# speechbrain/speechbrain

Hardware: NVIDIA B200
Metric: audio-sec/sec (RTFx) Conformer-L ASR, batch=32x10s@16kHz (higher is better)
Workload: dtype fp16 operands, fp32 accumulate/residual/softmax

## Files before the change

### include/sbk.h

```cpp
#ifndef SBK_H_
#define SBK_H_
#include <stdint.h>
#ifdef __cplusplus
extern "C" {
#endif

typedef struct sbk_fbank sbk_fbank;
typedef struct sbk_asr sbk_asr;

enum { SBK_ATT_ROPE = 0, SBK_ATT_RELPOS = 1 };
enum { SBK_ACT_RELU = 0, SBK_ACT_GELU = 1 };
enum { SBK_PART_FBANK = 1, SBK_PART_CNN = 2, SBK_PART_ENCODER = 4, SBK_PART_DECODER = 8, SBK_PART_ALL = 15, SBK_PART_LM = 16 };

typedef struct {
    const char* name;
    const float* data;
    int64_t numel;
} sbk_tensor;

typedef struct {
    int n_fft, hop, n_mels;
    int cnn_c1, cnn_c2;
    int input_size, d_model, nhead, num_encoder_layers, num_decoder_layers, d_ffn, vocab, kernel_size;
    int attention_type;
    int decoder_activation;
    int max_len;
    int parts;
    int lm_d_model, lm_nhead, lm_layers, lm_d_ffn, lm_activation;
    float fbank_amin, fbank_top_db, norm_eps;
} sbk_asr_config;

typedef struct {
    int beam_size, max_steps, min_steps, bos, eos;
    float temperature;
    int using_eos_threshold;
    float eos_threshold;
    int length_normalization;
    float minus_inf;
    float lm_weight, lm_temperature;
    float ctc_weight;
    int blank_index;
    float length_weight;
    float coverage_weight, coverage_threshold;
} sbk_beam_params;

const char* sbk_last_error(void);
int sbk_version(void);
long long sbk_launch_count(void);
void sbk_gemm_profile_enable(int on);
int sbk_gemm_profile_read(int* n_launches, double* total_ms, double* total_flops);

int sbk_fbank_create(int n_fft, int hop, int n_mels, const float* window_host, const float* mel_matrix_host,
                     float amin, float top_db, sbk_fbank** out);
void sbk_fbank_destroy(sbk_fbank* fb);
int sbk_fbank_num_frames(const sbk_fbank* fb, int n_samples);
int sbk_fbank_forward(const sbk_fbank* fb, const float* wav_dev, int B, int L, float* out_dev,
                      int* utt_max_scratch_dev, void* stream);

int sbk_input_norm_global(const float* x_dev, float* out_dev, int B, int T, int F, const float* mean_dev,
                          const float* std_dev, float eps, void* stream);
int sbk_input_norm_sentence(const float* x_dev, float* out_dev, const float* rel_len_dev, int B, int T, int F,
                            int std_norm, int avoid_padding_norm, float eps, void* stream);

int sbk_gemm_f16_test(const void* A_dev, const void* W_dev, const float* bias_dev, void* out_dev, int out_is_f32,
                      int act, int M, int N, int K, void* stream);
int sbk_gemm_f16_resid_test(const void* A_dev, const void* W_dev, const float* bias_dev, float* x_dev, float alpha,
                            int M, int N, int K, void* stream);

int sbk_asr_create(const sbk_asr_config* cfg, const sbk_tensor* weights, int n_weights, sbk_asr** out);
void sbk_asr_destroy(sbk_asr* m);
int sbk_asr_clone(sbk_asr* src, sbk_asr** out);
int sbk_asr_set_dynchunk(sbk_asr* m, int chunk_size, int left_context_chunks);
int sbk_asr_set_poll_interval(sbk_asr* m, int every_n_steps);
int sbk_asr_set_decoder_ln_fusion(sbk_asr* m, int on);
int sbk_asr_set_decoder_tc_min_rows(sbk_asr* m, int rows);
int sbk_asr_lm_rescore(sbk_asr* m, const int* tokens_dev, const int* lens_dev, int n, int L, float temperature, int pad_index,
                       float* scores_dev, void* stream);
int sbk_asr_num_frames(const sbk_asr* m, int n_samples, int* T_feat, int* T_enc);

int sbk_asr_cnn_forward(sbk_asr* m, const float* feats_dev, int B, int T0, float* out_dev, void* stream);
int sbk_asr_encode_from_cnn(sbk_asr* m, const float* src_dev, const float* rel_len_dev, int B, int T,
                            float* enc_out_dev, void* stream);
int sbk_asr_encode_feats(sbk_asr* m, const float* feats_dev, const float* rel_len_dev, int B, int T0,
                         float* cnn_out_dev, float* enc_out_dev, void* stream);
int sbk_asr_greedy_from_enc(sbk_asr* m, const float* enc_dev, const float* rel_len_dev, int B, int T, int max_steps,
                            int bos, int eos, int* pred_dev, float* score_dev, float* log_probs_dev, int* steps_done,
                            void* stream);
int sbk_rows_argmax_f32(const float* x_dev, int rows, int V, int* idx_dev, void* stream);
int sbk_asr_ctc_head(sbk_asr* m, const float* enc_dev, int B, int T, float* log_probs_dev, int* argmax_dev, void* stream);
int sbk_asr_decode_teacher_forced(sbk_asr* m, const int* tgt_dev, const float* enc_dev, const int* enc_len_dev, int n, int S,
                                  int T, float* out_dev, void* stream);
int sbk_asr_beam_from_enc(sbk_asr* m, const float* enc_dev, const float* rel_len_dev, int B, int T,
                          const sbk_beam_params* params, int* hist_tok_dev, int* hist_pred_dev, float* hist_score_dev,
                          float* hist_lp_dev, int* steps_done, void* stream);
int sbk_asr_transcribe_greedy_dev(sbk_asr* m, const float* wav_dev, const float* rel_len_dev, int B, int L,
                                  int max_steps, int bos, int eos, float* enc_out_dev, int* pred_dev,
                                  float* score_dev, float* log_probs_dev, int* steps_done, void* stream);
int sbk_asr_transcribe_greedy_group_dev(sbk_asr* m, int G, const float* const* wav_dev, const float* const* rel_len_dev,
                                        int B, int L, int max_steps, int bos, int eos, int* const* pred_dev,
                                        int* steps_done, void* stream);
int sbk_asr_transcribe_greedy_host(sbk_asr* m, const float* wav_host, const float* rel_len_host, int B, int L,
                                   int max_steps, int bos, int eos, int* pred_host, float* score_host,
                                   int* steps_done, void* stream);

int sbk_asr_transcribe_greedy_group_host_async(sbk_asr* m, int G, const float* const* wav_host,
                                               const float* const* rel_len_host, int B, int L, int max_steps, int bos, int eos,
                                               int* const* pred_host, int* const* pred_dev, int* steps_done, void* stream);

int sbk_asr_transcribe_greedy_host_async(sbk_asr* m, const float* wav_host, const float* rel_len_host, int B, int L,
                                         int max_steps, int bos, int eos, int* pred_host, float* score_host,
                                         int* steps_done, void* stream);

#ifdef __cplusplus
}
#endif
#endif
```

### speechbrain_b200/_lib.py

```python
import ctypes
import os

import torch

_HERE = os.path.dirname(os.path.abspath(__file__))
LIB_PATH = os.path.join(_HERE, "libsbk.so")

_lib = None


class sbk_tensor(ctypes.Structure):
    _fields_ = [("name", ctypes.c_char_p), ("data", ctypes.c_void_p), ("numel", ctypes.c_int64)]


class sbk_asr_config(ctypes.Structure):
    _fields_ = [(k, ctypes.c_int) for k in (
        "n_fft", "hop", "n_mels", "cnn_c1", "cnn_c2", "input_size", "d_model", "nhead", "num_encoder_layers",
        "num_decoder_layers", "d_ffn", "vocab", "kernel_size", "attention_type", "decoder_activation", "max_len",
        "parts", "lm_d_model", "lm_nhead", "lm_layers", "lm_d_ffn", "lm_activation")] + [
        (k, ctypes.c_float) for k in ("fbank_amin", "fbank_top_db", "norm_eps")]


class sbk_beam_params(ctypes.Structure):
    _fields_ = [("beam_size", ctypes.c_int), ("max_steps", ctypes.c_int), ("min_steps", ctypes.c_int),
                ("bos", ctypes.c_int), ("eos", ctypes.c_int), ("temperature", ctypes.c_float),
                ("using_eos_threshold", ctypes.c_int), ("eos_threshold", ctypes.c_float),
                ("length_normalization", ctypes.c_int), ("minus_inf", ctypes.c_float),
                ("lm_weight", ctypes.c_float), ("lm_temperature", ctypes.c_float),
                ("ctc_weight", ctypes.c_float), ("blank_index", ctypes.c_int), ("length_weight", ctypes.c_float),
                ("coverage_weight", ctypes.c_float), ("coverage_threshold", ctypes.c_float)]


SBK_ATT_ROPE, SBK_ATT_RELPOS = 0, 1
SBK_ACT_RELU, SBK_ACT_GELU = 0, 1
SBK_PARTS = {"fbank": 1, "cnn": 2, "encoder": 4, "decoder": 8, "lm": 16}

EXPORTS = [
    "sbk_last_error", "sbk_version", "sbk_launch_count", "sbk_gemm_profile_enable", "sbk_gemm_profile_read", "sbk_fbank_create", "sbk_fbank_destroy", "sbk_fbank_num_frames",
    "sbk_fbank_forward", "sbk_input_norm_global", "sbk_input_norm_sentence", "sbk_gemm_f16_test", "sbk_gemm_f16_resid_test",
    "sbk_asr_create", "sbk_asr_destroy", "sbk_asr_num_frames", "sbk_asr_cnn_forward", "sbk_asr_encode_from_cnn",
    "sbk_asr_encode_feats", "sbk_asr_greedy_from_enc", "sbk_asr_transcribe_greedy_dev",
    "sbk_asr_transcribe_greedy_host", "sbk_asr_transcribe_greedy_host_async", "sbk_asr_clone",
    "sbk_asr_set_poll_interval", "sbk_asr_beam_from_enc", "sbk_asr_set_decoder_ln_fusion", "sbk_asr_transcribe_greedy_group_dev",
    "sbk_asr_set_decoder_tc_min_rows", "sbk_asr_lm_rescore", "sbk_asr_transcribe_greedy_group_host_async", "sbk_asr_decode_teacher_forced", "sbk_asr_ctc_head", "sbk_rows_argmax_f32", "sbk_asr_set_dynchunk",
]


def lib():
    global _lib
    if _lib is None:
        if not os.path.exists(LIB_PATH):
            raise RuntimeError(
                f"{LIB_PATH} not found: the sm_100a CUDA library is required (no CPU fallback). "
                "Build it with `make -C speechbrain_b200/csrc` or `__graft_entry__.build()`.")
        L = ctypes.CDLL(LIB_PATH)
        L.sbk_last_error.restype = ctypes.c_char_p
        for name in EXPORTS:
            getattr(L, name)
        for name in EXPORTS:
            if name not in ("sbk_last_error", "sbk_fbank_destroy", "sbk_asr_destroy", "sbk_launch_count",
                            "sbk_gemm_profile_enable"):
                getattr(L, name).restype = ctypes.c_int
        L.sbk_launch_count.restype = ctypes.c_longlong
        L.sbk_gemm_profile_enable.restype = None
        _lib = L
    return _lib


def check(rc, what):
    if rc != 0:
        raise RuntimeError(f"libsbk: {what} failed ({rc}): {lib().sbk_last_error().decode()}")


def ptr(t):
    if t is None:
        return ctypes.c_void_p(0)
    assert t.is_contiguous(), "libsbk needs contiguous tensors"
    return ctypes.c_void_p(t.data_ptr())


def stream_ptr(device=None):
    return ctypes.c_void_p(torch.cuda.current_stream(device).cuda_stream)


def require_cuda(t, what):
    if not t.is_cuda:
        raise RuntimeError(f"{what}: expected a CUDA tensor (speechbrain_b200 has no CPU path)")
```

### speechbrain_b200/csrc/common.cuh

```cuda
#pragma once
#include <cuda.h>
#include <cuda_fp16.h>
#include <cuda_runtime.h>
#include <stdint.h>

#define SBK_OK 0
#define SBK_ERR_CUDA -1
#define SBK_ERR_ARG -2
#define SBK_ERR_UNSUPPORTED -3
#define SBK_ERR_NOMEM -4

namespace sbk {

void set_error(const char* fmt, ...);

#define SBK_CUDA_CHECK(expr)                                                              \
    do {                                                                                  \
        cudaError_t _e = (expr);                                                          \
        if (_e != cudaSuccess) {                                                          \
            sbk::set_error("%s:%d: %s -> %s", __FILE__, __LINE__, #expr, cudaGetErrorString(_e)); \
            return SBK_ERR_CUDA;                                                          \
        }                                                                                 \
    } while (0)

void count_launch();
#define SBK_LAUNCH_CHECK()                   \
    do {                                     \
        sbk::count_launch();                 \
        SBK_CUDA_CHECK(cudaGetLastError());  \
    } while (0)

#define SBK_REQUIRE(cond, ...)            \
    do {                                  \
        if (!(cond)) {                    \
            sbk::set_error(__VA_ARGS__);  \
            return SBK_ERR_ARG;           \
        }                                 \
    } while (0)

__host__ __device__ inline int ceil_div(int a, int b) { return (a + b - 1) / b; }

__device__ __forceinline__ float warp_sum(float v) {
#pragma unroll
    for (int o = 16; o > 0; o >>= 1) v += __shfl_xor_sync(0xffffffffu, v, o);
    return v;
}
__device__ __forceinline__ float warp_max(float v) {
#pragma unroll
    for (int o = 16; o > 0; o >>= 1) v = fmaxf(v, __shfl_xor_sync(0xffffffffu, v, o));
    return v;
}

__device__ __forceinline__ uint32_t smem_u32(const void* p) {
    return static_cast<uint32_t>(__cvta_generic_to_shared(p));
}

__device__ __forceinline__ void mbar_init(uint64_t* bar, uint32_t count) {
    asm volatile("mbarrier.init.shared::cta.b64 [%0], %1;" ::"r"(smem_u32(bar)), "r"(count));
}
__device__ __forceinline__ void mbar_fence_init() {
    asm volatile("fence.mbarrier_init.release.cluster;" ::: "memory");
}
__device__ __forceinline__ void mbar_arrive_expect_tx(uint64_t* bar, uint32_t bytes) {
    asm volatile("mbarrier.arrive.expect_tx.shared::cta.b64 _, [%0], %1;" ::"r"(smem_u32(bar)), "r"(bytes)
                 : "memory");
}
__device__ __forceinline__ void mbar_arrive(uint64_t* bar) {
    asm volatile("mbarrier.arrive.shared::cta.b64 _, [%0];" ::"r"(smem_u32(bar)) : "memory");
}
__device__ __forceinline__ bool mbar_try_wait(uint64_t* bar, uint32_t parity) {
    uint32_t ok;
    asm volatile(
        "{\n\t.reg .pred p;\n\t"
        "mbarrier.try_wait.parity.shared::cta.b64 p, [%1], %2;\n\t"
        "selp.u32 %0, 1, 0, p;\n\t}"
        : "=r"(ok)
        : "r"(smem_u32(bar)), "r"(parity)
        : "memory");
    return ok != 0;
}
__device__ __forceinline__ void mbar_wait(uint64_t* bar, uint32_t parity) {
    while (!mbar_try_wait(bar, parity)) {
    }
}

__device__ __forceinline__ void tma_prefetch_desc(const CUtensorMap* m) {
    asm volatile("prefetch.tensormap [%0];" ::"l"(reinterpret_cast<uint64_t>(m)) : "memory");
}
__device__ __forceinline__ void tma_load_2d(void* smem_dst, const CUtensorMap* m, uint64_t* bar, int c0, int c1) {
    asm volatile(
        "cp.async.bulk.tensor.2d.shared::cluster.global.mbarrier::complete_tx::bytes [%0], [%1, {%3, %4}], [%2];"
        ::"r"(smem_u32(smem_dst)), "l"(reinterpret_cast<uint64_t>(m)), "r"(smem_u32(bar)), "r"(c0), "r"(c1)
        : "memory");
}
__device__ __forceinline__ void tma_load_4d(void* smem_dst, const CUtensorMap* m, uint64_t* bar, int c0, int c1, int c2, int c3) {
    asm volatile(
        "cp.async.bulk.tensor.4d.shared::cluster.global.mbarrier::complete_tx::bytes [%0], [%1, {%3, %4, %5, %6}], [%2];"
        ::"r"(smem_u32(smem_dst)), "l"(reinterpret_cast<uint64_t>(m)), "r"(smem_u32(bar)), "r"(c0), "r"(c1), "r"(c2), "r"(c3)
        : "memory");
}
__device__ __forceinline__ void bulk_load_1d(void* smem_dst, const void* gsrc, uint32_t bytes, uint64_t* bar) {
    asm volatile(
        "cp.async.bulk.shared::cluster.global.mbarrier::complete_tx::bytes [%0], [%1], %2, [%3];"
        ::"r"(smem_u32(smem_dst)), "l"(reinterpret_cast<uint64_t>(gsrc)), "r"(bytes), "r"(smem_u32(bar))
        : "memory");
}

__device__ __forceinline__ void tmem_alloc(uint32_t* smem_result, uint32_t ncols) {
    asm volatile("tcgen05.alloc.cta_group::1.sync.aligned.shared::cta.b32 [%0], %1;" ::"r"(smem_u32(smem_result)),
                 "r"(ncols)
                 : "memory");
    asm volatile("tcgen05.relinquish_alloc_permit.cta_group::1.sync.aligned;" ::: "memory");
}
__device__ __forceinline__ void tmem_dealloc(uint32_t taddr, uint32_t ncols) {
    asm volatile("tcgen05.dealloc.cta_group::1.sync.aligned.b32 %0, %1;" ::"r"(taddr), "r"(ncols) : "memory");
}
__device__ __forceinline__ void tc_fence_before() { asm volatile("tcgen05.fence::before_thread_sync;" ::: "memory"); }
__device__ __forceinline__ void tc_fence_after() { asm volatile("tcgen05.fence::after_thread_sync;" ::: "memory"); }

__device__ __forceinline__ void umma_f16(uint32_t tmem_d, uint64_t desc_a, uint64_t desc_b, uint32_t idesc,
                                         uint32_t accumulate) {
    asm volatile(
        "{\n\t.reg .pred p;\n\t"
        "setp.ne.b32 p, %4, 0;\n\t"
        "tcgen05.mma.cta_group::1.kind::f16 [%0], %1, %2, %3, p;\n\t}"
        ::"r"(tmem_d), "l"(desc_a), "l"(desc_b), "r"(idesc), "r"(accumulate)
        : "memory");
}
__device__ __forceinline__ void umma_commit(uint64_t* bar) {
    asm volatile("tcgen05.commit.cta_group::1.mbarrier::arrive::one.shared::cluster.b64 [%0];" ::"r"(smem_u32(bar))
                 : "memory");
}
__device__ __forceinline__ void tmem_ld_32x32(uint32_t taddr, uint32_t (&r)[32]) {
    asm volatile(
        "tcgen05.ld.sync.aligned.32x32b.x32.b32 "
        "{%0, %1, %2, %3, %4, %5, %6, %7, %8, %9, %10, %11, %12, %13, %14, %15, "
        "%16, %17, %18, %19, %20, %21, %22, %23, %24, %25, %26, %27, %28, %29, %30, %31}, [%32];"
        : "=r"(r[0]), "=r"(r[1]), "=r"(r[2]), "=r"(r[3]), "=r"(r[4]), "=r"(r[5]), "=r"(r[6]), "=r"(r[7]), "=r"(r[8]),
          "=r"(r[9]), "=r"(r[10]), "=r"(r[11]), "=r"(r[12]), "=r"(r[13]), "=r"(r[14]), "=r"(r[15]), "=r"(r[16]),
          "=r"(r[17]), "=r"(r[18]), "=r"(r[19]), "=r"(r[20]), "=r"(r[21]), "=r"(r[22]), "=r"(r[23]), "=r"(r[24]),
          "=r"(r[25]), "=r"(r[26]), "=r"(r[27]), "=r"(r[28]), "=r"(r[29]), "=r"(r[30]), "=r"(r[31])
        : "r"(taddr)
        : "memory");
}
__device__ __forceinline__ void tmem_ld_wait() { asm volatile("tcgen05.wait::ld.sync.aligned;" ::: "memory"); }

__device__ __forceinline__ uint64_t make_kmajor_sw128_desc(uint32_t smem_addr) {
    uint64_t d = 0;
    d |= static_cast<uint64_t>((smem_addr & 0x3FFFFu) >> 4);
    d |= static_cast<uint64_t>(1) << 16;
    d |= static_cast<uint64_t>(1024 >> 4) << 32;
    d |= static_cast<uint64_t>(1) << 46;
    d |= static_cast<uint64_t>(2) << 61;
    return d;
}
__host__ __device__ constexpr uint32_t make_idesc_f16(int M, int N, int ab_format) {
    return (1u << 4) | (static_cast<uint32_t>(ab_format) << 7) | (static_cast<uint32_t>(ab_format) << 10) |
           (static_cast<uint32_t>(N >> 3) << 17) | (static_cast<uint32_t>(M >> 4) << 24);
}

__device__ __forceinline__ __half2 floats2half2_sat(float lo, float hi) {
    uint32_t r;
    asm("cvt.rn.satfinite.f16x2.f32 %0, %1, %2;" : "=r"(r) : "f"(hi), "f"(lo));
    return *reinterpret_cast<__half2*>(&r);
}
__device__ __forceinline__ __half float2half_sat(float x) {
    const __half2 h = floats2half2_sat(x, 0.0f);
    return __low2half(h);
}

__device__ __forceinline__ float rcp_approx(float x) {
    float y;
    asm("rcp.approx.ftz.f32 %0, %1;" : "=f"(y) : "f"(x));
    return y;
}
__device__ __forceinline__ float exp_ftz(float x) {
    float y;
    asm("ex2.approx.ftz.f32 %0, %1;" : "=f"(y) : "f"(x * 1.4426950408889634f));
    return y;
}
__device__ __forceinline__ float sigmoid_f(float x) { return rcp_approx(1.0f + exp_ftz(-x)); }
__device__ __forceinline__ float tanh_approx(float x) {
    float y;
    asm("tanh.approx.f32 %0, %1;" : "=f"(y) : "f"(x));
    return y;
}
__device__ __forceinline__ float sigmoid_fast(float x) { return fmaf(0.5f, tanh_approx(0.5f * x), 0.5f); }
__device__ __forceinline__ float silu_fast(float x) {
    const float h = 0.5f * x;
    return fmaf(h, tanh_approx(h), h);
}
__device__ __forceinline__ void sts128(uint32_t addr, uint4 v) {
    asm volatile("st.shared.v4.b32 [%0], {%1, %2, %3, %4};" ::"r"(addr), "r"(v.x), "r"(v.y), "r"(v.z), "r"(v.w) : "memory");
}
__device__ __forceinline__ uint4 lds128(uint32_t addr) {
    uint4 v;
    asm volatile("ld.shared.v4.b32 {%0, %1, %2, %3}, [%4];" : "=r"(v.x), "=r"(v.y), "=r"(v.z), "=r"(v.w) : "r"(addr) : "memory");
    return v;
}
__device__ __forceinline__ uint4 f4_as_u4(float4 f) {
    return make_uint4(__float_as_uint(f.x), __float_as_uint(f.y), __float_as_uint(f.z), __float_as_uint(f.w));
}
__device__ __forceinline__ float4 u4_as_f4(uint4 u) {
    return make_float4(__uint_as_float(u.x), __uint_as_float(u.y), __uint_as_float(u.z), __uint_as_float(u.w));
}
__device__ __forceinline__ float silu_f(float x) { return x * sigmoid_f(x); }
__device__ __forceinline__ float gelu_erf_f(float x) { return 0.5f * x * (1.0f + erff(x * 0.70710678118654752f)); }

__device__ __forceinline__ int float_to_ordered(float f) {
    int i = __float_as_int(f);
    return i >= 0 ? i : i ^ 0x7FFFFFFF;
}
__device__ __forceinline__ float ordered_to_float(int i) { return __int_as_float(i >= 0 ? i : i ^ 0x7FFFFFFF); }

int make_tmap_2d_f16(CUtensorMap* out, const void* base, uint64_t rows, uint64_t cols, uint64_t row_stride_elems,
                     uint32_t box_rows, uint32_t box_cols);

}
```

### speechbrain_b200/csrc/engine.cu

```cuda
#include <math.h>
#include <stdio.h>
#include <stdlib.h>
#include <string.h>

#include <algorithm>
#include <map>
#include <string>
#include <vector>

#include "common.cuh"
#include "sbk_internal.h"
#include "../../include/sbk.h"

namespace sbk {

struct EncLayerW {
    const float *ffn1_ln_g, *ffn1_ln_b, *ffn1_b1, *ffn1_b2;
    const __half *ffn1_w1, *ffn1_w2;
    const float *norm1_g, *norm1_b;
    const __half *wqkv, *wo;
    const float* bo;
    const __half* wpos;
    const float *pos_u, *pos_v;
    const float *conv_ln_g, *conv_ln_b;
// ... 276 lines not shown
    }
    if (!p.ok) { rc = SBK_ERR_ARG; goto fail; }
    m->enc_norm_g = p.f32("Transformer.encoder.norm.norm.weight", d);
    m->enc_norm_b = p.f32("Transformer.encoder.norm.norm.bias", d);
    m->pos_len = c.max_len;
    if (c.attention_type == SBK_ATT_ROPE) {
        std::vector<float> cs((size_t)c.max_len * dh / 2), sn(cs.size());
        for (int i = 0; i < dh / 2; ++i) {
            const float ang = expf((float)(2 * i) * -(logf(10000.0f) / (float)dh));
            for (int t = 0; t < c.max_len; ++t) {
                const float ta = (float)t * ang;
                cs[(size_t)t * (dh / 2) + i] = cosf(ta);
                sn[(size_t)t * (dh / 2) + i] = sinf(ta);
            }
        }
        m->rope_cos = p.f32_raw(cs.data(), cs.size());
        m->rope_sin = p.f32_raw(sn.data(), sn.size());
    } else {
        std::vector<float> pe((size_t)c.max_len * d);
        for (int i = 0; i < d / 2; ++i) {
            const float fr = expf((float)(2 * i) * -(logf(10000.0f) / (float)d));
            for (int t = 0; t < c.max_len; ++t) {
                pe[(size_t)t * d + 2 * i] = sinf((float)t * fr);
                pe[(size_t)t * d + 2 * i + 1] = cosf((float)t * fr);
            }
        }
        m->relpos_pe = p.f16_raw(pe.data(), pe.size());
    }
    }
    if (has_dec) {
        m->emb = p.f32("Transformer.custom_tgt_module.layers.0.emb.Embedding.weight", (int64_t)c.vocab * d);
        {
            std::vector<float> pe((size_t)c.max_len * d);
            for (int i = 0; i < d / 2; ++i) {
                const float den = expf((float)(2 * i) * -(logf(10000.0f) / (float)d));
                for (int t = 0; t < c.max_len; ++t) {
                    pe[(size_t)t * d + 2 * i] = sinf((float)t * den);
                    pe[(size_t)t * d + 2 * i + 1] = cosf((float)t * den);
                }
            }
            m->dec_pe = p.f32_raw(pe.data(), pe.size());
        }
        const int L = c.num_decoder_layers;
        m->dec.resize(L);
        std::vector<float> wckv((size_t)L * 2 * d * d), bckv((size_t)L * 2 * d);
        const float qs = 1.0f / sqrtf((float)dh);
        for (int l = 0; l < L && p.ok; ++l) {
            const std::string q = "Transformer.decoder.layers." + std::to_string(l) + ".";
            DecLayerW& e = m->dec[l];
            e.n1g = p.f32(q + "norm1.norm.weight", d); e.n1b = p.f32(q + "norm1.norm.bias", d);
            e.n2g = p.f32(q + "norm2.norm.weight", d); e.n2b = p.f32(q + "norm2.norm.bias", d);
            e.n3g = p.f32(q + "norm3.norm.weight", d); e.n3b = p.f32(q + "norm3.norm.bias", d);
            const float* wi = find(w, q + "self_attn.att.in_proj_weight", (int64_t)3 * d * d);
            const float* bi = find(w, q + "self_attn.att.in_proj_bias", 3 * d);
            const float* wc = find(w, q + "multihead_attn.att.in_proj_weight", (int64_t)3 * d * d);
            const float* bc = find(w, q + "multihead_attn.att.in_proj_bias", 3 * d);
            if (!wi || !bi || !wc || !bc) { p.ok = false; break; }
            {
                std::vector<float> ws(wi, wi + (size_t)3 * d * d), bs(bi, bi + 3 * d);
                for (size_t i = 0; i < (size_t)d * d; ++i) ws[i] *= qs;
                for (int i = 0; i < d; ++i) bs[i] *= qs;
                e.w_self_in = p.f16_raw(ws.data(), ws.size());
                e.b_self_in = p.f32_raw(bs.data(), bs.size());
                std::vector<float> wq(wc, wc + (size_t)d * d), bq(bc, bc + d);
                for (auto& v : wq) v *= qs;
                for (auto& v : bq) v *= qs;
                e.w_cross_q = p.f16_raw(wq.data(), wq.size());
                e.b_cross_q = p.f32_raw(bq.data(), bq.size());
            }
            memcpy(&wckv[(size_t)l * 2 * d * d], wc + (size_t)d * d, (size_t)2 * d * d * 4);
            memcpy(&bckv[(size_t)l * 2 * d], bc + d, (size_t)2 * d * 4);
            e.w_self_out = p.f16(q + "self_attn.att.out_proj.weight", (int64_t)d * d); e.b_self_out = p.f32(q + "self_attn.att.out_proj.bias", d);
            e.w_cross_out = p.f16(q + "multihead_attn.att.out_proj.weight", (int64_t)d * d); e.b_cross_out = p.f32(q + "multihead_attn.att.out_proj.bias", d);
            e.w_ffn1 = p.f16(q + "pos_ffn.ffn.0.weight", (int64_t)F * d); e.b_ffn1 = p.f32(q + "pos_ffn.ffn.0.bias", F);
            e.w_ffn2 = p.f16(q + "pos_ffn.ffn.3.weight", (int64_t)d * F); e.b_ffn2 = p.f32(q + "pos_ffn.ffn.3.bias", d);
        }
        if (!p.ok) { rc = SBK_ERR_ARG; goto fail; }
        m->w_ckv = p.f16_raw(wckv.data(), wckv.size());
        m->b_ckv = p.f32_raw(bckv.data(), bckv.size());
        m->dec_norm_g = p.f32("Transformer.decoder.norm.norm.weight", d);
        m->dec_norm_b = p.f32("Transformer.decoder.norm.norm.bias", d);
        m->w_lin = nullptr; m->b_lin = nullptr;
        if (w.count("seq_lin.w.weight")) {
            m->w_lin = p.f16("seq_lin.w.weight", (int64_t)c.vocab * d);
            m->b_lin = p.f32("seq_lin.w.bias", c.vocab);
        }
    }
    if ((c.parts & SBK_PART_LM) && c.lm_layers > 0) {
        const int dl = c.lm_d_model, Fl = c.lm_d_ffn, dhl = dl / c.lm_nhead;
        if (dhl != 64 || dl % 128 != 0) { set_error("asr_create: LM head_dim must be 64 and d_model %% 128 == 0"); rc = SBK_ERR_UNSUPPORTED; goto fail; }
        m->has_lm = true;
        m->lm_emb = p.f32("lm.custom_src_module.emb.Embedding.weight", (int64_t)c.vocab * dl);
        {
            std::vector<float> pe((size_t)c.max_len * dl);
            for (int i = 0; i < dl / 2; ++i) {
                const float den = expf((float)(2 * i) * -(logf(10000.0f) / (float)dl));
                for (int t = 0; t < c.max_len; ++t) {
                    pe[(size_t)t * dl + 2 * i] = sinf((float)t * den);
                    pe[(size_t)t * dl + 2 * i + 1] = cosf((float)t * den);
                }
            }
            m->lm_pe = p.f32_raw(pe.data(), pe.size());
        }
        m->lm.resize(c.lm_layers);
        const float qs = 1.0f / sqrtf((float)dhl);
        for (int l = 0; l < c.lm_layers && p.ok; ++l) {
            const std::string q = "lm.encoder.layers." + std::to_string(l) + ".";
            LmLayerW& e = m->lm[l];
            const float* wi = find(w, q + "self_att.att.in_proj_weight", (int64_t)3 * dl * dl);
            const float* bi = find(w, q + "self_att.att.in_proj_bias", 3 * dl);
            if (!wi || !bi) { p.ok = false; break; }
            std::vector<float> ws(wi, wi + (size_t)3 * dl * dl), bs(bi, bi + 3 * dl);
            for (size_t i = 0; i < (size_t)dl * dl; ++i) ws[i] *= qs;
            for (int i = 0; i < dl; ++i) bs[i] *= qs;
            e.w_in = p.f16_raw(ws.data(), ws.size());
            e.b_in = p.f32_raw(bs.data(), bs.size());
            e.w_out = p.f16(q + "self_att.att.out_proj.weight", (int64_t)dl * dl); e.b_out = p.f32(q + "self_att.att.out_proj.bias", dl);
            e.w1 = p.f16(q + "pos_ffn.ffn.0.weight", (int64_t)Fl * dl); e.b1 = p.f32(q + "pos_ffn.ffn.0.bias", Fl);
            e.w2 = p.f16(q + "pos_ffn.ffn.3.weight", (int64_t)dl * Fl); e.b2 = p.f32(q + "pos_ffn.ffn.3.bias", dl);
            e.n1g = p.f32(q + "norm1.norm.weight", dl); e.n1b = p.f32(q + "norm1.norm.bias", dl);
            e.n2g = p.f32(q + "norm2.norm.weight", dl); e.n2b = p.f32(q + "norm2.norm.bias", dl);
        }
        m->lm_norm_g = p.f32("lm.encoder.norm.norm.weight", dl); m->lm_norm_b = p.f32("lm.encoder.norm.norm.bias", dl);
        m->lm_wp0 = p.f16("lm.output_proj.layers.0.w.weight", (int64_t)dl * dl); m->lm_bp0 = p.f32("lm.output_proj.layers.0.w.bias", dl);
        m->lm_lnp_g = p.f32("lm.output_proj.layers.1.norm.weight", dl); m->lm_lnp_b = p.f32("lm.output_proj.layers.1.norm.bias", dl);
        m->lm_wp2 = p.f16("lm.output_proj.layers.2.w.weight", (int64_t)c.vocab * dl); m->lm_bp2 = p.f32("lm.output_proj.layers.2.w.bias", c.vocab);
        if (!p.ok) { rc = SBK_ERR_ARG; goto fail; }
    }
    if (w.count("ctc_lin.w.weight")) {
        m->w_ctc = p.f16("ctc_lin.w.weight", (int64_t)c.vocab * d);
        m->b_ctc = p.f32("ctc_lin.w.bias", c.vocab);
    }
    if (!p.ok) { rc = SBK_ERR_ARG; goto fail; }
    if (cudaMallocHost(&m->host_flag, 64) != cudaSuccess) { set_error("cudaMallocHost failed"); rc = SBK_ERR_NOMEM; goto fail; }
    m->weight_refs = new int(1);
    if (cudaDeviceSynchronize() != cudaSuccess) { set_error("asr_create: device error after upload"); rc = SBK_ERR_CUDA; goto fail; }
    *out = m;
    return SBK_OK;
fail:
    if (m->fbank) fbank_destroy(m->fbank);
    cudaFree(m->warena.base);
    delete m;
    return rc;
}

int asr_clone(AsrModel* src, AsrModel** out) {
    SBK_REQUIRE(src && out, "asr_clone: null argument");
    AsrModel* m = new AsrModel(*src);
    m->ws = Arena();
    m->wsB = m->wsL = m->ws_rows = m->ws_steps = 0;
    m->b = AsrModel::Buf();
    m->ctc = AsrModel::CtcBuf();
    m->cov = AsrModel::CovBuf();
    m->step_graph = nullptr;
    m->pipe_graph = nullptr;
    m->group_graph = nullptr;
    m->hgroup_graph = nullptr;
    m->beam_graph = nullptr;
    m->gwav = m->grel = nullptr; m->gwav_cap = 0;
    m->copy_stream = nullptr; m->ev_fork = nullptr;
    for (auto& e : m->ev_ready) e = nullptr;
    m->graph_rows = m->graph_T = m->graph_B = -1;
    m->cap_stream = nullptr;
    m->host_flag = nullptr;
    if (cudaMallocHost(&m->host_flag, 64) != cudaSuccess) {
        delete m;
        set_error("asr_clone: cudaMallocHost failed");
        return SBK_ERR_NOMEM;
    }
    ++*m->weight_refs;
    *out = m;
    return SBK_OK;
}

void asr_destroy(AsrModel* m) {
    if (!m) return;
    if (m->step_graph) cudaGraphExecDestroy(m->step_graph);
    if (m->pipe_graph) cudaGraphExecDestroy(m->pipe_graph);
    if (m->group_graph) cudaGraphExecDestroy(m->group_graph);
    if (m->hgroup_graph) cudaGraphExecDestroy(m->hgroup_graph);
    if (m->beam_graph) cudaGraphExecDestroy(m->beam_graph);
    cudaFree(m->gwav);
    if (m->copy_stream) cudaStreamDestroy(m->copy_stream);
    if (m->ev_fork) cudaEventDestroy(m->ev_fork);
    for (auto e : m->ev_ready) if (e) cudaEventDestroy(e);
    if (m->weight_refs && --*m->weight_refs == 0) {
        if (m->fbank) fbank_destroy(m->fbank);
        cudaFree(m->warena.base);
        delete m->weight_refs;
    }
    cudaFree(m->ws.base);
    cudaFree(m->ctc.base);
    cudaFree(m->cov.base);
    if (m->host_flag) cudaFreeHost(m->host_flag);
    if (m->cap_stream) cudaStreamDestroy(m->cap_stream);
    if (m->side_stream) cudaStreamDestroy(m->side_stream);
    if (m->dec_stream) cudaStreamDestroy(m->dec_stream);
    if (m->ev_dfork) cudaEventDestroy(m->ev_dfork);
    if (m->ev_djoin) cudaEventDestroy(m->ev_djoin);
    if (m->ev_bfork) cudaEventDestroy(m->ev_bfork);
    if (m->ev_bjoin) cudaEventDestroy(m->ev_bjoin);
    delete m;
}

static void drop_graphs(AsrModel* m) {
    if (m->step_graph) { cudaGraphExecDestroy(m->step_graph); m->step_graph = nullptr; m->graph_rows = -1; }
    if (m->pipe_graph) { cudaGraphExecDestroy(m->pipe_graph); m->pipe_graph = nullptr; }
    if (m->group_graph) { cudaGraphExecDestroy(m->group_graph); m->group_graph = nullptr; }
    if (m->hgroup_graph) { cudaGraphExecDestroy(m->hgroup_graph); m->hgroup_graph = nullptr; }
    if (m->beam_graph) { cudaGraphExecDestroy(m->beam_graph); m->beam_graph = nullptr; }
}

static void frames(const sbk_asr_config& c, int L, int* T0, int* T1, int* T2) {
    *T0 = 1 + L / c.hop;
    *T1 = (*T0 - 1) / 2 + 1;
    *T2 = (*T1 - 1) / 2 + 1;
}

static int ensure_workspace(AsrModel* m, int B, int L, int rows, int steps) {
    if (m->ws.base && B <= m->wsB && L <= m->wsL && rows <= m->ws_rows && steps <= m->ws_steps) return SBK_OK;
    B = std::max(B, m->wsB); L = std::max(L, m->wsL); rows = std::max(rows, m->ws_rows); steps = std::max(steps, m->ws_steps);
    const sbk_asr_config& c = m->cfg;
    int T0, T1, T2;
    frames(c, L, &T0, &T1, &T2);
    const int F1 = (c.n_mels - 1) / 2 + 1;
    const size_t M = (size_t)B * T2, d = c.d_model, F = c.d_ffn, Ld = c.num_decoder_layers, S = steps + 1;
    const size_t Md = (size_t)std::max(B, rows) * T2;
    size_t need = 0;
    auto sz = [&](size_t bytes) { need += (bytes + 255) & ~size_t(255); };
    sz((size_t)B * L * 4); sz((size_t)B * T0 * c.n_mels * 4); sz(M * d * 4); sz(M * d * 4); sz(Md * d * 4);
    sz((size_t)B * T1 * F1 * c.cnn_c1 * 4); sz(M * c.input_size * 4); sz((size_t)rows * d * 4);
    sz((size_t)rows * c.vocab * 4); sz((size_t)rows * S * 4);
    sz(B * 4); sz((size_t)std::max(B, rows) * 4); sz((size_t)rows * (S + 1) * 4); sz(rows * 4 + 64); sz(rows * 4); sz(64); sz((size_t)rows * S * 4); sz(B * 4);
    sz((size_t)B * T1 * F1 * c.cnn_c1 * 2); sz(M * c.input_size * 2); sz(M * d * 2); sz(M * F * 2); sz(M * 3 * d * 2);
    sz(M * d * 2); sz((size_t)T2 * d * 2); sz(Md * d * 2); sz(Md * Ld * 2 * d * 2);
    sz((size_t)Ld * rows * S * d * 2); sz((size_t)Ld * rows * S * d * 2);
    sz((size_t)rows * d * 2); sz((size_t)rows * d * 2); sz((size_t)rows * d * 2); sz((size_t)rows * F * 2);
    sz((size_t)2 * rows * S * 4); sz(B * 4 + 64); sz((size_t)2 * rows * 4); sz((size_t)rows * d * 4); sz((size_t)rows * 33 * 4);
    sz((size_t)rows * S * 4); sz((size_t)rows * S * 4); sz((size_t)rows * S * 4); sz((size_t)rows * S * 4);
    const size_t dl = m->has_lm ? c.lm_d_model : 0, Fl = m->has_lm ? c.lm_d_ffn : 0, Ll = m->has_lm ? c.lm_layers : 0;
    if (m->has_lm) {
        sz(rows * dl * 4); sz(rows * dl * 4); sz((size_t)rows * c.vocab * 4); sz((size_t)rows * c.vocab * 4);
        sz(rows * dl * 2); sz(rows * dl * 2); sz(rows * dl * 2); sz(rows * Fl * 2); sz(rows * dl * 2);
        sz(Ll * rows * S * dl * 2); sz(Ll * rows * S * dl * 2); sz((size_t)rows * S * 4);
    }
    need += 1 << 20;
    if (need > m->ws.cap) {
        if (m->ws.base) { cudaDeviceSynchronize(); cudaFree(m->ws.base); m->ws.base = nullptr; }
        if (cudaMalloc(&m->ws.base, need) != cudaSuccess) {
            m->ws.cap = 0;
            set_error("workspace cudaMalloc(%zu) failed", need);
            return SBK_ERR_NOMEM;
        }
        m->ws.cap = need;
    }
    drop_graphs(m);
    m->ws.used = 0;
    AsrModel::Buf& b = m->b;
#define TAKE(field, type, bytes) b.field = reinterpret_cast<type*>(m->ws.take(bytes))
    TAKE(wav, float, (size_t)B * L * 4); TAKE(feats, float, (size_t)B * T0 * c.n_mels * 4); TAKE(x, float, M * d * 4);
    TAKE(glu, float, M * d * 4); TAKE(enc_out, float, Md * d * 4); TAKE(act1_f, float, (size_t)B * T1 * F1 * c.cnn_c1 * 4);
    TAKE(cnn_f, float, M * c.input_size * 4); TAKE(dx, float, (size_t)rows * d * 4); TAKE(logits, float, (size_t)rows * c.vocab * 4);
    TAKE(score, float, (size_t)rows * S * 4);
    TAKE(utt_max, int, B * 4); TAKE(enc_len, int, (size_t)std::max(B, rows) * 4); TAKE(tokens, int, (size_t)rows * (S + 1) * 4); TAKE(step, int, rows * 4 + 64);
    TAKE(has_ended, int, rows * 4); TAKE(ended_count, int, 64); TAKE(pred, int, (size_t)rows * S * 4); TAKE(rel_len, float, B * 4);
    TAKE(act1, __half, (size_t)B * T1 * F1 * c.cnn_c1 * 2); TAKE(a_in, __half, M * c.input_size * 2); TAKE(h16, __half, M * d * 2);
    TAKE(f16, __half, M * F * 2); TAKE(qkv16, __half, M * 3 * d * 2); TAKE(att16, __half, M * d * 2);
    TAKE(P16, __half, (size_t)T2 * d * 2); TAKE(enc16, __half, Md * d * 2); TAKE(ckv16, __half, Md * Ld * 2 * d * 2);
    TAKE(kcache, __half, (size_t)Ld * rows * S * d * 2); TAKE(vcache, __half, (size_t)Ld * rows * S * d * 2);
    TAKE(dh16, __half, (size_t)rows * d * 2); TAKE(dq16, __half, (size_t)rows * d * 2); TAKE(datt16, __half, (size_t)rows * d * 2);
    TAKE(df16, __half, (size_t)rows * F * 2);
    TAKE(lineage, int, (size_t)2 * rows * S * 4); TAKE(finished, int, B * 4 + 64); TAKE(seq_scores, float, (size_t)2 * rows * 4);
    TAKE(lnout, float, (size_t)rows * d * 4); TAKE(beam_scr, float, (size_t)rows * 33 * 4);
    TAKE(hist_tok, int, (size_t)rows * S * 4); TAKE(hist_pred, int, (size_t)rows * S * 4);
    TAKE(hist_score, float, (size_t)rows * S * 4); TAKE(hist_lp, float, (size_t)rows * S * 4);
    if (m->has_lm) {
        TAKE(lx, float, rows * dl * 4); TAKE(lh32, float, rows * dl * 4); TAKE(lm_logits, float, (size_t)rows * c.vocab * 4);
        TAKE(lm_extra, float, (size_t)rows * c.vocab * 4);
        TAKE(lx16, __half, rows * dl * 2); TAKE(lq16, __half, rows * dl * 2); TAKE(latt16, __half, rows * dl * 2);
        TAKE(lf16, __half, rows * Fl * 2); TAKE(lh16, __half, rows * dl * 2);
        TAKE(lkc, __half, Ll * rows * S * dl * 2); TAKE(lvc, __half, Ll * rows * S * dl * 2); TAKE(tok_cache, int, (size_t)rows * S * 4);
        if (!b.tok_cache) { set_error("workspace carve failed (LM)"); return SBK_ERR_NOMEM; }
    }
    if (!b.df16 || !b.seq_scores || !b.lnout || !b.hist_lp) { set_error("workspace carve failed"); return SBK_ERR_NOMEM; }
#undef TAKE
    m->wsB = B; m->wsL = L; m->ws_rows = rows; m->ws_steps = steps;
    return SBK_OK;
}

#define RC(expr) do { int _rc = (expr); if (_rc) return _rc; } while (0)

static int run_encoder(AsrModel* m, const float* feats, int B, int T0, const int* enc_len, float* cnn_out_f,
                       float* enc_out, cudaStream_t st) {
    const sbk_asr_config& c = m->cfg;
    AsrModel::Buf& b = m->b;
    const int T1 = (T0 - 1) / 2 + 1, T = feats ? (T1 - 1) / 2 + 1 : T0;
    const int M = B * T, d = c.d_model, F = c.d_ffn, H = c.nhead, dh = d / H;
    SBK_REQUIRE(m->has_enc, "encode: this handle was created without encoder weights");
    SBK_REQUIRE(feats == nullptr || m->has_cnn, "encode: this handle was created without CNN weights");
    SBK_REQUIRE(T <= m->pos_len, "encode: %d frames exceed max_len=%d", T, m->pos_len);
    if (feats != nullptr)
        RC(cnn_frontend_forward(feats, B, T0, c.n_mels, m->c1_w, m->c1_b, m->c1_g, m->c1_be, c.cnn_c1, m->c2_w, m->c2_b,
                                m->c2_g, m->c2_be, c.cnn_c2, b.act1, nullptr, b.a_in, cnn_out_f, st));
    GemmEpilogue e;
    e.mode = EPI_F32; e.bias = m->b_in; e.out = b.x; e.ldo = d;
    RC(gemm_f16(b.a_in, c.input_size, m->w_in, c.input_size, e, M, d, c.input_size, st));
    const float att_scale = 1.0f / sqrtf((float)d);
    for (int l = 0; l < c.num_encoder_layers; ++l) {
        const EncLayerW& w = m->enc[l];
        if (l == 0) RC(layernorm_rows(b.x, b.h16, true, w.ffn1_ln_g, w.ffn1_ln_b, M, d, 1e-5f, false, st));
        e = GemmEpilogue(); e.mode = EPI_F16; e.act = ACT_SILU; e.bias = w.ffn1_b1; e.out = b.f16; e.ldo = F;
        RC(gemm_f16(b.h16, d, w.ffn1_w1, d, e, M, F, d, st));
        e = GemmEpilogue(); e.mode = EPI_RESID; e.bias = w.ffn1_b2; e.out = b.x; e.resid = b.x; e.ldo = d; e.alpha = 0.5f;
        RC(gemm_f16(b.f16, F, w.ffn1_w2, F, e, M, d, F, st));
        RC(layernorm_rows(b.x, b.h16, true, w.norm1_g, w.norm1_b, M, d, 1e-5f, false, st));
        e = GemmEpilogue(); e.out = b.qkv16; e.ldo = 3 * d;
        if (c.attention_type == SBK_ATT_ROPE) {
            e.mode = EPI_ROPE; e.alpha = att_scale; e.T = T; e.rope_cos = m->rope_cos; e.rope_sin = m->rope_sin; e.head_dim = dh;
        } else {
            e.mode = EPI_F16;
        }
        RC(gemm_f16(b.h16, d, w.wqkv, d, e, M, 3 * d, d, st));
        if (c.attention_type == SBK_ATT_RELPOS) {
            e = GemmEpilogue(); e.mode = EPI_F16; e.out = b.P16; e.ldo = d;
            RC(gemm_f16(m->relpos_pe, d, w.wpos, d, e, T, d, d, st));
        }
        RC(encoder_attention(b.qkv16, 3 * d, B, T, H, dh, enc_len, c.attention_type == SBK_ATT_RELPOS, w.pos_u, w.pos_v,
                             b.P16, d, att_scale, b.att16, d, st, m->dyn_chunk, m->dyn_left));
        e = GemmEpilogue(); e.mode = EPI_RESID; e.bias = w.bo; e.out = b.x; e.resid = b.x; e.ldo = d; e.alpha = 1.0f;
        RC(gemm_f16(b.att16, d, w.wo, d, e, M, d, d, st));
        RC(layernorm_rows(b.x, b.h16, true, w.conv_ln_g, w.conv_ln_b, M, d, 1e-5f, false, st));
        e = GemmEpilogue(); e.mode = EPI_GLU; e.bias = w.bpw1; e.out = b.glu; e.ldo = d;
        RC(gemm_f16(b.h16, d, w.wpw1, d, e, M, 2 * d, d, st));
        RC(dwconv_ln_swish(b.glu, B, T, d, c.kernel_size, w.wdw, w.bdw, w.aconv_ln_g, w.aconv_ln_b, 1e-5f, b.h16, st, m->dyn_chunk));
        e = GemmEpilogue(); e.mode = EPI_RESID; e.bias = w.bpw2; e.out = b.x; e.resid = b.x; e.ldo = d; e.alpha = 1.0f;
        e.row_lens = enc_len; e.T = T;
        RC(gemm_f16(b.h16, d, w.wpw2, d, e, M, d, d, st));
        RC(layernorm_rows(b.x, b.h16, true, w.ffn2_ln_g, w.ffn2_ln_b, M, d, 1e-5f, false, st));
        e = GemmEpilogue(); e.mode = EPI_F16; e.act = ACT_SILU; e.bias = w.ffn2_b1; e.out = b.f16; e.ldo = F;
        RC(gemm_f16(b.h16, d, w.ffn2_w1, d, e, M, F, d, st));
        e = GemmEpilogue(); e.mode = EPI_RESID; e.bias = w.ffn2_b2; e.out = b.x; e.resid = b.x; e.ldo = d; e.alpha = 0.5f;
        RC(gemm_f16(b.f16, F, w.ffn2_w2, F, e, M, d, F, st));
        if (l + 1 < c.num_encoder_layers) {
            const EncLayerW& nx = m->enc[l + 1];
            RC(layernorm2_rows(b.x, b.x, b.h16, true, w.norm2_g, w.norm2_b, 1e-5f, nx.ffn1_ln_g, nx.ffn1_ln_b, 1e-5f, M, d, st));
        } else {
            RC(layernorm2_rows(b.x, nullptr, enc_out, false, w.norm2_g, w.norm2_b, 1e-5f, m->enc_norm_g, m->enc_norm_b, 1e-6f, M,
                               d, st));
        }
    }
    if (c.num_encoder_layers == 0)
        RC(layernorm_rows(b.x, enc_out, false, m->enc_norm_g, m->enc_norm_b, M, d, 1e-6f, false, st));
    return SBK_OK;
}

__global__ void abs_len_kernel(const float* rel, int B, int T, int* out) {
    const int i = blockIdx.x * blockDim.x + threadIdx.x;
    if (i < B) out[i] = min(T, max(0, __float2int_rn(rel[i] * static_cast<float>(T))));
}

static int dec_ln(AsrModel* m, SkinnyArgs& a, const float* g, const float* bta, int rows, cudaStream_t st) {
    AsrModel::Buf& b = m->b;
    const int d = m->cfg.d_model;
    if (m->fuse_dec_ln && (d == 256 || d == 512 || d == 768 || d == 1024)) {
        a.X = b.dx; a.ln_g = g; a.ln_b = bta; a.ln_eps = 1e-6f;
        return SBK_OK;
    }
    a.A = b.dh16; a.lda = d;
    return layernorm_rows(b.dx, b.dh16, true, g, bta, rows, d, 1e-6f, false, st);
}

static bool xatt_headmajor(const AsrModel* m) {
    static const bool legacy = getenv("SBK_XATT_ROWMAJOR") != nullptr || getenv("SBK_GEMM_V1") != nullptr;
    return !legacy && m->cfg.d_model / m->cfg.nhead == 64 && m->cfg.d_model % 256 == 0;
}
static int project_cross_kv(AsrModel* m, int M, int T, cudaStream_t st) {
    const sbk_asr_config& c = m->cfg;
    AsrModel::Buf& b = m->b;
    const int d = c.d_model, Ld = c.num_decoder_layers;
    RC(cast_f32_f16(b.enc_out, b.enc16, (size_t)M * d, st));
    for (int l = 0; l < Ld; ++l) {
        GemmEpilogue e;
        e.mode = EPI_F16; e.bias = m->b_ckv + (size_t)l * 2 * d; e.out = b.ckv16 + (size_t)l * M * 2 * d; e.ldo = 2 * d;
        if (xatt_headmajor(m)) { e.kv_heads = c.nhead; e.kv_part_stride = (size_t)M * d; e.T = T; }
        RC(gemm_f16(b.enc16, d, m->w_ckv + (size_t)l * 2 * d * d, d, e, M, 2 * d, d, st));
    }
    return SBK_OK;
}
static void cross_kv_args(const AsrModel* m, DecAttnArgs& t, int l, int n_utt, int T) {
    const int d = m->cfg.d_model;
    const size_t M = (size_t)n_utt * T;
    t.kbase = m->b.ckv16 + (size_t)l * M * 2 * d;
    if (xatt_headmajor(m)) {
        t.vbase = t.kbase + M * d; t.row_stride = (size_t)T * d; t.head_stride = T * 64; t.key_stride = 64;
    } else {
        t.vbase = t.kbase + d; t.row_stride = (size_t)T * 2 * d; t.head_stride = 0; t.key_stride = 2 * d;
    }
}

static int enqueue_decode_layers_tc(AsrModel* m, int rows, int rows_per_utt, int T, int S_max, const int* lineage,
                                    cudaStream_t st, bool with_head) {
    const sbk_asr_config& c = m->cfg;
    AsrModel::Buf& b = m->b;
    const int d = c.d_model, F = c.d_ffn, H = c.nhead, dh = d / H, Ld = c.num_decoder_layers;
    const int n_utt = rows / rows_per_utt;
    for (int l = 0; l < Ld; ++l) {
        const DecLayerW& w = m->dec[l];
        __half* kc = b.kcache + (size_t)l * rows * S_max * d;
        __half* vc = b.vcache + (size_t)l * rows * S_max * d;
        RC(layernorm_rows(b.dx, b.dh16, true, w.n1g, w.n1b, rows, d, 1e-6f, false, st));
        GemmEpilogue e;
        e.mode = EPI_QKV_CACHE; e.bias = w.b_self_in; e.out = b.dq16; e.ldo = d; e.kcache = kc; e.vcache = vc;
        e.step_ptr = b.step; e.S_max = S_max; e.qkv_d = d;
        RC(gemm_f16_small(b.dh16, d, w.w_self_in, d, e, rows, 3 * d, d, st));
        DecAttnArgs t{};
        t.q = b.dq16; t.ldq = d; t.kbase = kc; t.vbase = vc; t.row_stride = (size_t)S_max * d; t.key_stride = d;
        t.rows_per_block = 1; t.n_keys_ptr = b.step; t.enc_len = nullptr; t.H = H; t.dh = dh; t.out = b.datt16; t.ldo = d;
        t.lineage = lineage; t.lin_stride = S_max;
        RC(dec_attention(t, rows, S_max, st));
        e = GemmEpilogue(); e.mode = EPI_RESID; e.bias = w.b_self_out; e.out = b.dx; e.resid = b.dx; e.ldo = d;
        RC(gemm_f16_small(b.datt16, d, w.w_self_out, d, e, rows, d, d, st));
        RC(layernorm_rows(b.dx, b.dh16, true, w.n2g, w.n2b, rows, d, 1e-6f, false, st));
        e = GemmEpilogue(); e.mode = EPI_F16; e.bias = w.b_cross_q; e.out = b.dq16; e.ldo = d;
        RC(gemm_f16_small(b.dh16, d, w.w_cross_q, d, e, rows, d, d, st));
        t = DecAttnArgs{};
        t.q = b.dq16; t.ldq = d; cross_kv_args(m, t, l, n_utt, T); t.rows_per_block = rows_per_utt;
        t.n_keys_ptr = nullptr; t.enc_len = b.enc_len; t.H = H; t.dh = dh; t.out = b.datt16; t.ldo = d;
        RC(dec_attention(t, rows, T, st));
        e = GemmEpilogue(); e.mode = EPI_RESID; e.bias = w.b_cross_out; e.out = b.dx; e.resid = b.dx; e.ldo = d;
        RC(gemm_f16_small(b.datt16, d, w.w_cross_out, d, e, rows, d, d, st));
        RC(layernorm_rows(b.dx, b.dh16, true, w.n3g, w.n3b, rows, d, 1e-6f, false, st));
        e = GemmEpilogue(); e.mode = EPI_F16; e.act = c.decoder_activation == SBK_ACT_GELU ? ACT_GELU : ACT_RELU;
        e.bias = w.b_ffn1; e.out = b.df16; e.ldo = F;
        RC(gemm_f16_small(b.dh16, d, w.w_ffn1, d, e, rows, F, d, st));
        e = GemmEpilogue(); e.mode = EPI_RESID; e.bias = w.b_ffn2; e.out = b.dx; e.resid = b.dx; e.ldo = d;
        RC(gemm_f16_small(b.df16, F, w.w_ffn2, F, e, rows, d, F, st));
    }
    if (!with_head) return SBK_OK;
    SBK_REQUIRE(m->w_lin != nullptr, "decode step: this handle was created without the output head (seq_lin.w.*)");
    RC(layernorm_rows(b.dx, b.dh16, true, m->dec_norm_g, m->dec_norm_b, rows, d, 1e-6f, false, st));
    GemmEpilogue e;
    e.mode = EPI_F32; e.bias = m->b_lin; e.out = b.logits; e.ldo = c.vocab;
    RC(gemm_f16_small(b.dh16, d, m->w_lin, d, e, rows, c.vocab, d, st));
    return SBK_OK;
}

static int enqueue_decode_layers(AsrModel* m, int rows, int rows_per_utt, int T, int S_max, const int* lineage,
                                 cudaStream_t st, bool with_head = true) {
    if (rows >= m->dec_tc_rows && m->cfg.d_model % 32 == 0)
        return enqueue_decode_layers_tc(m, rows, rows_per_utt, T, S_max, lineage, st, with_head);
    const sbk_asr_config& c = m->cfg;
    AsrModel::Buf& b = m->b;
    const int d = c.d_model, F = c.d_ffn, H = c.nhead, dh = d / H, Ld = c.num_decoder_layers;
    const int ffn_epi = c.decoder_activation == SBK_ACT_GELU ? SK_F16_GELU : SK_F16_RELU;
    const int n_utt = rows / rows_per_utt;
    for (int l = 0; l < Ld; ++l) {
        const DecLayerW& w = m->dec[l];
        __half* kc = b.kcache + (size_t)l * rows * S_max * d;
        __half* vc = b.vcache + (size_t)l * rows * S_max * d;
        SkinnyArgs a{};
        RC(dec_ln(m, a, w.n1g, w.n1b, rows, st));
        a.W = w.w_self_in; a.ldw = d; a.bias = w.b_self_in; a.n_rows = rows; a.N = 3 * d; a.K = d;
        a.epi = SK_QKV_CACHE; a.out = b.dq16; a.ldo = d; a.kcache = kc; a.vcache = vc; a.step_ptr = b.step; a.S_max = S_max;
        a.d = d; a.q_scale = 1.0f;
        RC(skinny_gemm(a, st));
        DecAttnArgs t{};
        t.q = b.dq16; t.ldq = d; t.kbase = kc; t.vbase = vc; t.row_stride = (size_t)S_max * d; t.key_stride = d;
        t.rows_per_block = 1; t.n_keys_ptr = b.step; t.enc_len = nullptr; t.H = H; t.dh = dh; t.out = b.datt16; t.ldo = d;
        t.lineage = lineage; t.lin_stride = S_max;
        RC(dec_attention(t, rows, S_max, st));
        a = SkinnyArgs{}; a.A = b.datt16; a.lda = d; a.W = w.w_self_out; a.ldw = d; a.bias = w.b_self_out; a.n_rows = rows;
        a.N = d; a.K = d; a.epi = SK_RESID; a.out = b.dx; a.ldo = d;
        RC(skinny_gemm(a, st));
        a = SkinnyArgs{};
        RC(dec_ln(m, a, w.n2g, w.n2b, rows, st));
        a.W = w.w_cross_q; a.ldw = d; a.bias = w.b_cross_q; a.n_rows = rows;
        a.N = d; a.K = d; a.epi = SK_F16; a.out = b.dq16; a.ldo = d;
        RC(skinny_gemm(a, st));
        t = DecAttnArgs{};
        t.q = b.dq16; t.ldq = d; cross_kv_args(m, t, l, n_utt, T); t.rows_per_block = rows_per_utt;
        t.n_keys_ptr = nullptr; t.enc_len = b.enc_len; t.H = H; t.dh = dh; t.out = b.datt16; t.ldo = d;
        RC(dec_attention(t, rows, T, st));
        a = SkinnyArgs{}; a.A = b.datt16; a.lda = d; a.W = w.w_cross_out; a.ldw = d; a.bias = w.b_cross_out; a.n_rows = rows;
        a.N = d; a.K = d; a.epi = SK_RESID; a.out = b.dx; a.ldo = d;
        RC(skinny_gemm(a, st));
        a = SkinnyArgs{};
        RC(dec_ln(m, a, w.n3g, w.n3b, rows, st));
        a.W = w.w_ffn1; a.ldw = d; a.bias = w.b_ffn1; a.n_rows = rows;
        a.N = F; a.K = d; a.epi = ffn_epi; a.out = b.df16; a.ldo = F;
        RC(skinny_gemm(a, st));
        a = SkinnyArgs{}; a.A = b.df16; a.lda = F; a.W = w.w_ffn2; a.ldw = F; a.bias = w.b_ffn2; a.n_rows = rows;
        a.N = d; a.K = F; a.epi = SK_RESID; a.out = b.dx; a.ldo = d;
        RC(skinny_gemm(a, st));
    }
    if (!with_head) return SBK_OK;
    SBK_REQUIRE(m->w_lin != nullptr, "decode step: this handle was created without the output head (seq_lin.w.*)");
    SkinnyArgs a{};
    RC(dec_ln(m, a, m->dec_norm_g, m->dec_norm_b, rows, st));
    a.W = m->w_lin; a.ldw = d; a.bias = m->b_lin; a.n_rows = rows; a.N = c.vocab; a.K = d;
    a.epi = SK_F32; a.out = b.logits; a.ldo = c.vocab;
    RC(skinny_gemm(a, st));
    return SBK_OK;
}

static int enqueue_decode_step(AsrModel* m, int rows, int rows_per_utt, int T, int S_max, int eos, float* log_probs,
                               int L_lp, cudaStream_t st) {
    AsrModel::Buf& b = m->b;
    RC(enqueue_decode_layers(m, rows, rows_per_utt, T, S_max, nullptr, st));
    RC(greedy_select(b.logits, rows, m->cfg.vocab, b.step, eos, b.tokens, S_max + 1, b.has_ended, b.ended_count, b.pred,
                     b.score, S_max, log_probs, L_lp, m->emb, m->dec_pe, m->cfg.d_model, b.dx, st));
    return SBK_OK;
}

static int enqueue_lm_step_tc(AsrModel* m, int rows, int S_max, float temperature, float weight, cudaStream_t st) {
    const sbk_asr_config& c = m->cfg;
    AsrModel::Buf& b = m->b;
    const int dl = c.lm_d_model, Fl = c.lm_d_ffn, H = c.lm_nhead;
    for (int l = 0; l < c.lm_layers; ++l) {
        const LmLayerW& w = m->lm[l];
        __half* kc = b.lkc + (size_t)l * rows * S_max * dl;
        __half* vc = b.lvc + (size_t)l * rows * S_max * dl;
        GemmEpilogue e;
        e.mode = EPI_QKV_CACHE; e.bias = w.b_in; e.out = b.lq16; e.ldo = dl; e.kcache = kc; e.vcache = vc;
        e.step_ptr = b.step; e.S_max = S_max; e.qkv_d = dl;
        RC(gemm_f16_small(b.lx16, dl, w.w_in, dl, e, rows, 3 * dl, dl, st));
        DecAttnArgs t{};
        t.q = b.lq16; t.ldq = dl; t.kbase = kc; t.vbase = vc; t.row_stride = (size_t)S_max * dl; t.key_stride = dl;
        t.rows_per_block = 1; t.n_keys_ptr = b.step; t.H = H; t.dh = 64; t.out = b.latt16; t.ldo = dl;
        t.lineage = b.lineage; t.lin_stride = S_max; t.tok_cache = b.tok_cache; t.pad_tok = 0;
        RC(dec_attention(t, rows, S_max, st));
        e = GemmEpilogue(); e.mode = EPI_RESID; e.bias = w.b_out; e.out = b.lx; e.resid = b.lx; e.ldo = dl;
        RC(gemm_f16_small(b.latt16, dl, w.w_out, dl, e, rows, dl, dl, st));
        RC(layernorm_dual(b.lx, b.lx16, w.n1g, w.n1b, rows, dl, 1e-6f, true, st));
        e = GemmEpilogue(); e.mode = EPI_F16; e.act = c.lm_activation == SBK_ACT_GELU ? ACT_GELU : ACT_RELU;
        e.bias = w.b1; e.out = b.lf16; e.ldo = Fl;
        RC(gemm_f16_small(b.lx16, dl, w.w1, dl, e, rows, Fl, dl, st));
        e = GemmEpilogue(); e.mode = EPI_RESID; e.bias = w.b2; e.out = b.lx; e.resid = b.lx; e.ldo = dl;
        RC(gemm_f16_small(b.lf16, Fl, w.w2, Fl, e, rows, dl, Fl, st));
        RC(layernorm_dual(b.lx, b.lx16, w.n2g, w.n2b, rows, dl, 1e-6f, true, st));
    }
    RC(layernorm_dual(b.lx, b.lx16, m->lm_norm_g, m->lm_norm_b, rows, dl, 1e-6f, false, st));
    GemmEpilogue e;
    e.mode = EPI_F32; e.bias = m->lm_bp0; e.out = b.lh32; e.ldo = dl;
    RC(gemm_f16_small(b.lx16, dl, m->lm_wp0, dl, e, rows, dl, dl, st));
    RC(layernorm_dual(b.lh32, b.lh16, m->lm_lnp_g, m->lm_lnp_b, rows, dl, 1e-6f, false, st));
    e = GemmEpilogue(); e.mode = EPI_F32; e.bias = m->lm_bp2; e.out = b.lm_logits; e.ldo = c.vocab;
    RC(gemm_f16_small(b.lh16, dl, m->lm_wp2, dl, e, rows, c.vocab, dl, st));
    RC(weighted_log_softmax(b.lm_logits, b.lm_extra, rows, c.vocab, temperature, weight, st));
    return SBK_OK;
}

static int enqueue_lm_step(AsrModel* m, int rows, int S_max, float temperature, float weight, cudaStream_t st) {
    if (rows >= m->dec_tc_rows) return enqueue_lm_step_tc(m, rows, S_max, temperature, weight, st);
    const sbk_asr_config& c = m->cfg;
    AsrModel::Buf& b = m->b;
    const int dl = c.lm_d_model, Fl = c.lm_d_ffn, H = c.lm_nhead;
    for (int l = 0; l < c.lm_layers; ++l) {
        const LmLayerW& w = m->lm[l];
        __half* kc = b.lkc + (size_t)l * rows * S_max * dl;
        __half* vc = b.lvc + (size_t)l * rows * S_max * dl;
        SkinnyArgs a{};
        a.A = b.lx16; a.lda = dl; a.W = w.w_in; a.ldw = dl; a.bias = w.b_in; a.n_rows = rows; a.N = 3 * dl; a.K = dl;
        a.epi = SK_QKV_CACHE; a.out = b.lq16; a.ldo = dl; a.kcache = kc; a.vcache = vc; a.step_ptr = b.step; a.S_max = S_max;
        a.d = dl; a.q_scale = 1.0f;
        RC(skinny_gemm(a, st));
        DecAttnArgs t{};
        t.q = b.lq16; t.ldq = dl; t.kbase = kc; t.vbase = vc; t.row_stride = (size_t)S_max * dl; t.key_stride = dl;
        t.rows_per_block = 1; t.n_keys_ptr = b.step; t.H = H; t.dh = 64; t.out = b.latt16; t.ldo = dl;
        t.lineage = b.lineage; t.lin_stride = S_max; t.tok_cache = b.tok_cache; t.pad_tok = 0;
        RC(dec_attention(t, rows, S_max, st));
        a = SkinnyArgs{}; a.A = b.latt16; a.lda = dl; a.W = w.w_out; a.ldw = dl; a.bias = w.b_out; a.n_rows = rows;
        a.N = dl; a.K = dl; a.epi = SK_RESID; a.out = b.lx; a.ldo = dl;
        RC(skinny_gemm(a, st));
        RC(layernorm_dual(b.lx, b.lx16, w.n1g, w.n1b, rows, dl, 1e-6f, true, st));
        a = SkinnyArgs{}; a.A = b.lx16; a.lda = dl; a.W = w.w1; a.ldw = dl; a.bias = w.b1; a.n_rows = rows;
        a.N = Fl; a.K = dl; a.epi = c.lm_activation == SBK_ACT_GELU ? SK_F16_GELU : SK_F16_RELU; a.out = b.lf16; a.ldo = Fl;
        RC(skinny_gemm(a, st));
        a = SkinnyArgs{}; a.A = b.lf16; a.lda = Fl; a.W = w.w2; a.ldw = Fl; a.bias = w.b2; a.n_rows = rows;
        a.N = dl; a.K = Fl; a.epi = SK_RESID; a.out = b.lx; a.ldo = dl;
        RC(skinny_gemm(a, st));
        RC(layernorm_dual(b.lx, b.lx16, w.n2g, w.n2b, rows, dl, 1e-6f, true, st));
    }
    RC(layernorm_dual(b.lx, b.lx16, m->lm_norm_g, m->lm_norm_b, rows, dl, 1e-6f, false, st));
    SkinnyArgs a{};
    a.A = b.lx16; a.lda = dl; a.W = m->lm_wp0; a.ldw = dl; a.bias = m->lm_bp0; a.n_rows = rows; a.N = dl; a.K = dl;
    a.epi = SK_F32; a.out = b.lh32; a.ldo = dl;
    RC(skinny_gemm(a, st));
    RC(layernorm_dual(b.lh32, b.lh16, m->lm_lnp_g, m->lm_lnp_b, rows, dl, 1e-6f, false, st));
    a = SkinnyArgs{}; a.A = b.lh16; a.lda = dl; a.W = m->lm_wp2; a.ldw = dl; a.bias = m->lm_bp2; a.n_rows = rows;
    a.N = c.vocab; a.K = dl; a.epi = SK_F32; a.out = b.lm_logits; a.ldo = c.vocab;
    RC(skinny_gemm(a, st));
    RC(weighted_log_softmax(b.lm_logits, b.lm_extra, rows, c.vocab, temperature, weight, st));
    return SBK_OK;
}

static int run_beam(AsrModel* m, int B, int T, const sbk_beam_params& p, int* hist_tok_out, int* hist_pred_out,
                    float* hist_score_out, float* hist_lp_out, int* steps_done, cudaStream_t st) {
    const sbk_asr_config& c = m->cfg;
    AsrModel::Buf& b = m->b;
    const int d = c.d_model, Ld = c.num_decoder_layers, M = B * T, beam = p.beam_size, rows = B * beam, S_max = m->ws_steps + 1;
    SBK_REQUIRE(m->has_dec, "beam: this handle was created without decoder weights");
    SBK_REQUIRE(p.max_steps <= m->ws_steps && p.max_steps + 1 <= c.max_len, "beam: max_steps=%d too large", p.max_steps);
    *steps_done = 0;
    if (p.max_steps <= 0) return SBK_OK;
    RC(project_cross_kv(m, M, T, st));
    set_pdl(getenv("SBK_PDL") != nullptr);
    const bool use_lm = p.lm_weight != 0.0f;
    SBK_REQUIRE(!use_lm || m->has_lm, "beam: lm_weight != 0 but this handle has no TransformerLM weights");
    const bool use_ctc = p.ctc_weight != 0.0f;
    int* hist_tok = b.hist_tok; int* hist_pred = b.hist_pred; float* hist_score = b.hist_score; float* hist_lp = b.hist_lp;
    CtcStep cs{};
    if (use_ctc) {
        SBK_REQUIRE(m->w_ctc, "beam: ctc_weight != 0 but this handle has no ctc_lin weights");
        SBK_REQUIRE(p.blank_index >= 0 && p.blank_index < c.vocab && p.blank_index != p.bos && p.blank_index != p.eos &&
                    p.bos != p.eos, "Set blank, eos and bos to different indexes for joint ATT/CTC or CTC decoding");
        const size_t V = c.vocab;
        auto al = [](size_t n) { return (n * 4 + 255) & ~size_t(255); };
        const size_t need = 2 * al((size_t)M * V) + al(M) + 2 * al((size_t)2 * rows * T) + al(2 * rows) + (use_lm ? 0 : al(rows * V)) +
                            al((size_t)2 * rows * (T + 4)) + al(2 * rows);
        AsrModel::CtcBuf& cb = m->ctc;
        if (need > cb.cap) {
            if (cb.base) { SBK_CUDA_CHECK(cudaStreamSynchronize(st)); cudaFree(cb.base); cb.base = nullptr; cb.cap = 0; }
            if (m->beam_graph) { cudaGraphExecDestroy(m->beam_graph); m->beam_graph = nullptr; }
            if (cudaMalloc(&cb.base, need) != cudaSuccess) { set_error("beam: CTC scorer cudaMalloc(%zu) failed", need); return SBK_ERR_NOMEM; }
            cb.cap = need;
        }
        char* q = reinterpret_cast<char*>(cb.base);
        cb.x = reinterpret_cast<float*>(q); q += al((size_t)M * V);
        cb.xlin = reinterpret_cast<float*>(q); q += al((size_t)M * V);
        cb.xb = reinterpret_cast<float*>(q); q += al(M);
        cb.rsum = reinterpret_cast<float*>(q); q += al((size_t)2 * rows * T);
        cb.rb = reinterpret_cast<float*>(q); q += al((size_t)2 * rows * T);
        cb.psi = reinterpret_cast<float*>(q); q += al(2 * rows);
        cb.tab = reinterpret_cast<float*>(q); q += al((size_t)2 * rows * (T + 4));
        cb.tabM = reinterpret_cast<float*>(q); q += al(2 * rows);
        cb.add = use_lm ? b.lm_extra : reinterpret_cast<float*>(q);
        GemmEpilogue e;
        e.mode = EPI_F32; e.bias = m->b_ctc; e.out = cb.x; e.ldo = c.vocab;
        RC(gemm_f16(b.enc16, d, m->w_ctc, d, e, M, c.vocab, d, st));
        RC(ctc_prefix_reset(cb.x, cb.xlin, cb.xb, b.enc_len, B, T, c.vocab, p.blank_index, beam, cb.rsum, cb.rb, cb.psi, cb.tab, cb.tabM, st));
        cs.x = cb.x; cs.xlin = cb.xlin; cs.xb = cb.xb; cs.enc_len = b.enc_len; cs.hist_tok = hist_tok; cs.hist_pred = hist_pred; cs.n_bh = rows;
        cs.rsum_base = cb.rsum; cs.rb_base = cb.rb; cs.psi_base = cb.psi; cs.step_ptr = b.step; cs.tab = cb.tab; cs.tabM = cb.tabM;
        cs.bos = p.bos; cs.T = T; cs.V = c.vocab; cs.beam = beam; cs.blank = p.blank_index; cs.eos = p.eos;
        cs.weight = p.ctc_weight; cs.out = cb.add; cs.accumulate = use_lm ? 1 : 0;
// ... 17 lines not shown
        cv.threshold = p.coverage_threshold; cv.weight = p.coverage_weight; cv.out = m->cov.base + (size_t)2 * rows * T;
    }
    BeamLm lm;
    if (use_lm) { lm.emb = m->lm_emb; lm.pe = m->lm_pe; lm.d = c.lm_d_model; lm.x = b.lx; lm.x16 = b.lx16; lm.tok_cache = b.tok_cache; }
    RC(beam_reset(rows, beam, S_max, p.bos, b.step, b.seq_scores, b.lineage, b.finished, b.ended_count, m->emb, m->dec_pe, d,
                  b.dx, use_lm ? &lm : nullptr, st));
    BeamStepArgs a{};
    a.add_scores = use_lm ? b.lm_extra : (use_ctc ? m->ctc.add : nullptr);
    a.lm = lm;
    if (use_ctc) { a.attn_weight = 1.0f - p.ctc_weight; a.blank = p.blank_index; }
    a.add_const = p.length_weight;
    a.add_row = use_cov ? cv.out : nullptr;
    a.logits = b.logits; a.V = c.vocab; a.beam = beam; a.S_max = S_max; a.seq_scores = b.seq_scores; a.lineage = b.lineage;
    a.step_arr = b.step; a.finished = b.finished; a.n_full = b.ended_count;
    a.hist_tok = hist_tok; a.hist_pred = hist_pred; a.hist_score = hist_score; a.hist_lp = hist_lp;
    a.temperature = p.temperature; a.eos_threshold = p.eos_threshold; a.minus_inf = p.minus_inf; a.min_steps = p.min_steps;
    a.eos = p.eos; a.use_eos_threshold = p.using_eos_threshold; a.length_norm = p.length_normalization;
    a.emb = m->emb; a.pe = m->dec_pe; a.d = d; a.x_next = b.dx; a.scratch = b.beam_scr;
    const bool fork = (use_lm || use_ctc) && getenv("SBK_BEAM_SERIAL") == nullptr;
    if (fork && !m->side_stream) {
        SBK_CUDA_CHECK(cudaStreamCreateWithFlags(&m->side_stream, cudaStreamNonBlocking));
        SBK_CUDA_CHECK(cudaEventCreateWithFlags(&m->ev_bfork, cudaEventDisableTiming));
        SBK_CUDA_CHECK(cudaEventCreateWithFlags(&m->ev_bjoin, cudaEventDisableTiming));
    }
    auto enqueue_step = [&](cudaStream_t s_) -> int {
        cudaStream_t s2 = s_;
        if (fork) {
            s2 = m->side_stream;
            SBK_CUDA_CHECK(cudaEventRecord(m->ev_bfork, s_));
            SBK_CUDA_CHECK(cudaStreamWaitEvent(s2, m->ev_bfork, 0));
        }
        if (use_ctc) RC(ctc_prefix_update(cs, s2));
        if (use_lm) RC(enqueue_lm_step(m, rows, S_max, p.lm_temperature, p.lm_weight, s2));
        RC(enqueue_decode_layers(m, rows, beam, T, S_max, b.lineage, s_));
        if (use_cov) RC(coverage_score(cv, s_));
        if (fork) {
            SBK_CUDA_CHECK(cudaEventRecord(m->ev_bjoin, s2));
            SBK_CUDA_CHECK(cudaStreamWaitEvent(s_, m->ev_bjoin, 0));
        }
        if (use_ctc) RC(ctc_prefix_score(cs, s_));
        RC(beam_step(a, B, s_));
        return SBK_OK;
    };
    const bool use_graph = getenv("SBK_NO_GRAPH") == nullptr;
    if (use_graph) {
        AsrModel::BeamKey key;
        memset(&key, 0, sizeof(key));
        key.p = p; key.B = B; key.T = T; key.rows = rows; key.S_max = S_max; key.fuse_ln = m->fuse_dec_ln; key.tc_rows = m->dec_tc_rows; key.fork = fork ? 1 : 0;
        if (m->beam_graph == nullptr || memcmp(&key, &m->beam_key, sizeof(key)) != 0) {
            if (m->beam_graph) { cudaGraphExecDestroy(m->beam_graph); m->beam_graph = nullptr; }
            if (!m->cap_stream) SBK_CUDA_CHECK(cudaStreamCreateWithFlags(&m->cap_stream, cudaStreamNonBlocking));
            cudaGraph_t g;
            SBK_CUDA_CHECK(cudaStreamBeginCapture(m->cap_stream, cudaStreamCaptureModeThreadLocal));
            launch_count_begin_capture();
            int rc = enqueue_step(m->cap_stream);
            m->beam_nodes = launch_count_end_capture();
            cudaError_t ce = cudaStreamEndCapture(m->cap_stream, &g);
            if (rc) return rc;
            SBK_CUDA_CHECK(ce);
            SBK_CUDA_CHECK(cudaGraphInstantiate(&m->beam_graph, g, 0));
            cudaGraphDestroy(g);
            m->beam_key = key;
        }
    }
    const int check_every = m->poll_every > 0 ? m->poll_every : p.max_steps;
    int s = 0;
    while (s < p.max_steps) {
        const int chunk = std::min(check_every, p.max_steps - s);
        for (int i = 0; i < chunk; ++i) {
            if (use_graph) { SBK_CUDA_CHECK(cudaGraphLaunch(m->beam_graph, st)); launch_count_add(m->beam_nodes); }
            else RC(enqueue_step(st));
        }
        s += chunk;
        if (s < p.max_steps && m->poll_every > 0) {
            SBK_CUDA_CHECK(cudaMemcpyAsync(m->host_flag, b.ended_count, 4, cudaMemcpyDeviceToHost, st));
            SBK_CUDA_CHECK(cudaStreamSynchronize(st));
            if (*m->host_flag >= B) break;
        }
    }
    const size_t hb = (size_t)s * rows * 4;
    if (hist_tok_out) SBK_CUDA_CHECK(cudaMemcpyAsync(hist_tok_out, hist_tok, hb, cudaMemcpyDeviceToDevice, st));
    if (hist_pred_out) SBK_CUDA_CHECK(cudaMemcpyAsync(hist_pred_out, hist_pred, hb, cudaMemcpyDeviceToDevice, st));
    if (hist_score_out) SBK_CUDA_CHECK(cudaMemcpyAsync(hist_score_out, hist_score, hb, cudaMemcpyDeviceToDevice, st));
    if (hist_lp_out) SBK_CUDA_CHECK(cudaMemcpyAsync(hist_lp_out, hist_lp, hb, cudaMemcpyDeviceToDevice, st));
    *steps_done = s;
    return SBK_OK;
}

static int run_greedy(AsrModel* m, int B, int T, int max_steps, int bos, int eos, float* log_probs, int* steps_done,
                      cudaStream_t st, bool in_capture = false) {
    const sbk_asr_config& c = m->cfg;
    AsrModel::Buf& b = m->b;
    const int d = c.d_model, M = B * T, rows = B, S_max = m->ws_steps + 1;
    SBK_REQUIRE(m->has_dec, "greedy: this handle was created without decoder weights");
    SBK_REQUIRE(max_steps <= m->ws_steps && max_steps + 1 <= c.max_len, "greedy: max_steps=%d too large", max_steps);
    *steps_done = 0;
    if (max_steps <= 0) return SBK_OK;
    RC(project_cross_kv(m, M, T, st));
    RC(greedy_reset(b.tokens, S_max + 1, rows, bos, b.step, b.has_ended, b.ended_count, m->emb, m->dec_pe, d, b.dx, st));
    set_pdl(getenv("SBK_PDL") != nullptr);
    const bool use_graph = !in_capture && getenv("SBK_NO_GRAPH") == nullptr && log_probs == nullptr;
    if (in_capture) {
        for (int i = 0; i < max_steps; ++i) RC(enqueue_decode_step(m, rows, 1, T, S_max, eos, log_probs, max_steps, st));
        *steps_done = max_steps;
        return SBK_OK;
    }
    if (use_graph && (m->step_graph == nullptr || m->graph_rows != rows || m->graph_T != T || m->graph_B != B ||
                      m->graph_eos != eos || m->graph_S != S_max)) {
        if (m->step_graph) { cudaGraphExecDestroy(m->step_graph); m->step_graph = nullptr; }
        cudaGraph_t g;
        if (!m->cap_stream) SBK_CUDA_CHECK(cudaStreamCreateWithFlags(&m->cap_stream, cudaStreamNonBlocking));
        SBK_CUDA_CHECK(cudaStreamBeginCapture(m->cap_stream, cudaStreamCaptureModeThreadLocal));
        launch_count_begin_capture();
        int rc = enqueue_decode_step(m, rows, 1, T, S_max, eos, nullptr, 0, m->cap_stream);
        m->graph_nodes = launch_count_end_capture();
        cudaError_t ce = cudaStreamEndCapture(m->cap_stream, &g);
        if (rc) return rc;
        SBK_CUDA_CHECK(ce);
        SBK_CUDA_CHECK(cudaGraphInstantiate(&m->step_graph, g, 0));
        cudaGraphDestroy(g);
        m->graph_rows = rows; m->graph_T = T; m->graph_B = B; m->graph_eos = eos; m->graph_S = S_max;
    }
    const int check_every = m->poll_every > 0 ? m->poll_every : max_steps;
    int s = 0;
    while (s < max_steps) {
        const int chunk = std::min(check_every, max_steps - s);
        for (int i = 0; i < chunk; ++i) {
            if (use_graph) { SBK_CUDA_CHECK(cudaGraphLaunch(m->step_graph, st)); launch_count_add(m->graph_nodes); }
            else RC(enqueue_decode_step(m, rows, 1, T, S_max, eos, log_probs, max_steps, st));
        }
        s += chunk;
        if (s < max_steps && m->poll_every > 0) {
            SBK_CUDA_CHECK(cudaMemcpyAsync(m->host_flag, b.ended_count, 4, cudaMemcpyDeviceToHost, st));
            SBK_CUDA_CHECK(cudaStreamSynchronize(st));
            if (*m->host_flag >= rows) break;
        }
    }
    *steps_done = s;
    return SBK_OK;
}

__global__ void lm_teacher_reset_kernel(const int* __restrict__ tokens, int n, int L, int S_max, int pad, int* __restrict__ lineage,
                                        int* __restrict__ tok_cache, float* __restrict__ scores) {
    const int r = blockIdx.x;
    for (int p = threadIdx.x; p < S_max; p += blockDim.x) {
        lineage[static_cast<size_t>(r) * S_max + p] = r;
        lineage[static_cast<size_t>(n) * S_max + static_cast<size_t>(r) * S_max + p] = r;
        tok_cache[static_cast<size_t>(r) * S_max + p] = p < L ? tokens[static_cast<size_t>(r) * L + p] : pad;
    }
    if (threadIdx.x == 0) scores[r] = 0.0f;
}
__global__ void lm_teacher_embed_kernel(const int* __restrict__ tokens, int L, int s, const float* __restrict__ emb,
                                        const float* __restrict__ pe, int d, float sqrt_d, float* __restrict__ x,
                                        __half* __restrict__ x16, int* __restrict__ step_arr) {
    const int r = blockIdx.x;
    const int tok = tokens[static_cast<size_t>(r) * L + s];
    for (int i = threadIdx.x; i < d; i += blockDim.x) {
        const float v = emb[static_cast<size_t>(tok) * d + i] * sqrt_d + pe[static_cast<size_t>(s) * d + i];
        x[static_cast<size_t>(r) * d + i] = v;
        x16[static_cast<size_t>(r) * d + i] = float2half_sat(v);
    }
    if (threadIdx.x == 0) step_arr[r] = s;
}
__global__ void lm_teacher_score_kernel(const float* __restrict__ log_probs, int V, const int* __restrict__ tokens, int L, int s,
                                        const int* __restrict__ lens, int pad, float* __restrict__ scores, int n) {
    const int r = blockIdx.x * blockDim.x + threadIdx.x;
    if (r >= n || s + 1 >= lens[r]) return;
    const float* lp = log_probs + static_cast<size_t>(r) * V;
    const int tgt = tokens[static_cast<size_t>(r) * L + s + 1];
    const float v = (tgt == pad ? -INFINITY : lp[tgt]) - log1pf(-expf(lp[pad]));
    if (v == v) scores[r] += v;
}

__global__ void dec_teacher_embed_kernel(const int* __restrict__ tokens, int S, int s, const float* __restrict__ emb,
                                         const float* __restrict__ pe, int d, float sqrt_d, float* __restrict__ x,
                                         int* __restrict__ step_arr) {
    const int r = blockIdx.x;
    const int tok = tokens[static_cast<size_t>(r) * S + s];
    for (int i = threadIdx.x; i < d; i += blockDim.x)
        x[static_cast<size_t>(r) * d + i] = emb[static_cast<size_t>(tok) * d + i] * sqrt_d + pe[static_cast<size_t>(s) * d + i];
    if (threadIdx.x == 0) step_arr[r] = s;
}

static int run_decode_teacher(AsrModel* m, const int* tokens, int n, int S, int T, float* out, cudaStream_t st) {
    const sbk_asr_config& c = m->cfg;
    AsrModel::Buf& b = m->b;
    const int d = c.d_model, M = n * T, S_max = m->ws_steps + 1;
    SBK_REQUIRE(m->has_dec, "decode: this handle was created without decoder weights");
    SBK_REQUIRE(S <= m->ws_steps && S <= c.max_len, "decode: %d target positions exceed the workspace / max_len", S);
    RC(project_cross_kv(m, M, T, st));
    for (int s = 0; s < S; ++s) {
        dec_teacher_embed_kernel<<<n, 128, 0, st>>>(tokens, S, s, m->emb, m->dec_pe, d, sqrtf((float)d), b.dx, b.step);
        SBK_LAUNCH_CHECK();
        RC(enqueue_decode_layers(m, n, 1, T, S_max, nullptr, st, false));
        RC(layernorm_rows(b.dx, b.lnout, false, m->dec_norm_g, m->dec_norm_b, n, d, 1e-6f, false, st));
        SBK_CUDA_CHECK(cudaMemcpy2DAsync(out + (size_t)s * d, (size_t)S * d * 4, b.lnout, (size_t)d * 4, (size_t)d * 4, n,
                                         cudaMemcpyDeviceToDevice, st));
    }
    return SBK_OK;
}

static int run_lm_rescore(AsrModel* m, const int* tokens, const int* lens, int n, int L, float temperature, int pad,
                          float* scores, cudaStream_t st) {
    const sbk_asr_config& c = m->cfg;
    AsrModel::Buf& b = m->b;
    const int S_max = m->ws_steps + 1, dl = c.lm_d_model;
    lm_teacher_reset_kernel<<<n, 128, 0, st>>>(tokens, n, L, S_max, pad, b.lineage, b.tok_cache, scores);
    SBK_LAUNCH_CHECK();
    for (int s = 0; s + 1 < L; ++s) {
        lm_teacher_embed_kernel<<<n, 128, 0, st>>>(tokens, L, s, m->lm_emb, m->lm_pe, dl, sqrtf((float)dl), b.lx, b.lx16, b.step);
        SBK_LAUNCH_CHECK();
        RC(enqueue_lm_step(m, n, S_max, temperature, 1.0f, st));
        lm_teacher_score_kernel<<<ceil_div(n, 128), 128, 0, st>>>(b.lm_extra, c.vocab, tokens, L, s, lens, pad, scores, n);
        SBK_LAUNCH_CHECK();
    }
    return SBK_OK;
}

}

using namespace sbk;

extern "C" {

const char* sbk_last_error(void) { return sbk::last_error(); }

int sbk_version(void) { return 100; }

long long sbk_launch_count(void) { return sbk::launch_count(); }

void sbk_gemm_profile_enable(int on) {
    GemmProfile* p = gemm_profile();
    for (cudaEvent_t e : p->ev) cudaEventDestroy(e);
    p->ev.clear();
    p->flops.clear();
    p->shape.clear();
    p->enabled = on != 0;
}
int sbk_gemm_profile_read(int* n_launches, double* total_ms, double* total_flops) {
    GemmProfile* p = gemm_profile();
    double ms = 0.0, fl = 0.0;
    for (size_t i = 0; i < p->flops.size(); ++i) {
        float t = 0.0f;
        if (cudaEventElapsedTime(&t, p->ev[2 * i], p->ev[2 * i + 1]) != cudaSuccess) {
            set_error("sbk_gemm_profile_read: events not complete (synchronize first)");
            return SBK_ERR_CUDA;
        }
        ms += t;
        fl += p->flops[i];
        if (getenv("SBK_GEMM_TRACE"))
            fprintf(stderr, "gemm M=%d N=%d K=%d epi=%d : %.1f us  %.0f TFLOP/s\n", p->shape[4 * i], p->shape[4 * i + 1],
                    p->shape[4 * i + 2], p->shape[4 * i + 3], t * 1e3, p->flops[i] / (t * 1e-3) / 1e12);
    }
    if (n_launches) *n_launches = (int)p->flops.size();
    if (total_ms) *total_ms = ms;
    if (total_flops) *total_flops = fl;
    return SBK_OK;
}

int sbk_fbank_create(int n_fft, int hop, int n_mels, const float* window_host, const float* mel_matrix_host, float amin,
                     float top_db, sbk_fbank** out) {
    return fbank_create(reinterpret_cast<Fbank**>(out), n_fft, hop, n_mels, window_host, mel_matrix_host, amin, top_db);
}
void sbk_fbank_destroy(sbk_fbank* fb) { fbank_destroy(reinterpret_cast<Fbank*>(fb)); }
int sbk_fbank_num_frames(const sbk_fbank* fb, int n_samples) { return fbank_num_frames(reinterpret_cast<const Fbank*>(fb), n_samples); }
int sbk_fbank_forward(const sbk_fbank* fb, const float* wav_dev, int B, int L, float* out_dev, int* utt_max_scratch_dev,
                      void* stream) {
    return fbank_forward(reinterpret_cast<const Fbank*>(fb), wav_dev, B, L, out_dev, utt_max_scratch_dev, nullptr, nullptr,
                         0.0f, static_cast<cudaStream_t>(stream));
}
int sbk_input_norm_global(const float* x_dev, float* out_dev, int B, int T, int F, const float* mean_dev,
                          const float* std_dev, float eps, void* stream) {
    return global_norm_forward(x_dev, out_dev, B, T, F, mean_dev, std_dev, eps, static_cast<cudaStream_t>(stream));
}
int sbk_input_norm_sentence(const float* x_dev, float* out_dev, const float* rel_len_dev, int B, int T, int F,
                            int std_norm, int avoid_padding_norm, float eps, void* stream) {
    return sentence_norm_forward(x_dev, out_dev, rel_len_dev, B, T, F, std_norm, avoid_padding_norm, eps,
                                 static_cast<cudaStream_t>(stream));
}

int sbk_gemm_f16_test(const void* A_dev, const void* W_dev, const float* bias_dev, void* out_dev, int out_is_f32, int act,
                      int M, int N, int K, void* stream) {
    GemmEpilogue e;
    e.mode = out_is_f32 ? EPI_F32 : EPI_F16;
    e.act = act;
    e.bias = bias_dev;
    e.out = out_dev;
    e.ldo = N;
    return gemm_f16(A_dev, K, W_dev, K, e, M, N, K, static_cast<cudaStream_t>(stream));
}

int sbk_gemm_f16_resid_test(const void* A_dev, const void* W_dev, const float* bias_dev, float* x_dev, float alpha, int M,
                            int N, int K, void* stream) {
    GemmEpilogue e;
    e.mode = EPI_RESID;
    e.bias = bias_dev;
    e.out = x_dev;
    e.resid = x_dev;
    e.alpha = alpha;
    e.ldo = N;
    return gemm_f16(A_dev, K, W_dev, K, e, M, N, K, static_cast<cudaStream_t>(stream));
}

int sbk_asr_create(const sbk_asr_config* cfg, const sbk_tensor* weights, int n_weights, sbk_asr** out) {
    return asr_create(cfg, weights, n_weights, reinterpret_cast<AsrModel**>(out));
}
void sbk_asr_destroy(sbk_asr* m) { asr_destroy(reinterpret_cast<AsrModel*>(m)); }
int sbk_asr_clone(sbk_asr* src, sbk_asr** out) {
    return asr_clone(reinterpret_cast<AsrModel*>(src), reinterpret_cast<AsrModel**>(out));
}
int sbk_asr_set_decoder_ln_fusion(sbk_asr* m, int on) {
    AsrModel* mm = reinterpret_cast<AsrModel*>(m);
    if (mm->fuse_dec_ln != (on != 0)) drop_graphs(mm);
    mm->fuse_dec_ln = on != 0;
    return SBK_OK;
}
int sbk_asr_set_decoder_tc_min_rows(sbk_asr* m, int rows) {
    AsrModel* mm = reinterpret_cast<AsrModel*>(m);
    if (mm->dec_tc_rows != rows) drop_graphs(mm);
    mm->dec_tc_rows = rows;
    return SBK_OK;
}
int sbk_asr_set_dynchunk(sbk_asr* m, int chunk_size, int left_context_chunks) {
    AsrModel* mm = reinterpret_cast<AsrModel*>(m);
    SBK_REQUIRE(chunk_size >= 0, "set_dynchunk: chunk_size must be >= 0 (0 = full-context attention)");
    const int left = left_context_chunks < 0 ? -1 : left_context_chunks;
    if (mm->dyn_chunk != chunk_size || mm->dyn_left != left) drop_graphs(mm);
    mm->dyn_chunk = chunk_size;
    mm->dyn_left = left;
    return SBK_OK;
}
int sbk_asr_set_poll_interval(sbk_asr* m, int every_n_steps) {
    reinterpret_cast<AsrModel*>(m)->poll_every = every_n_steps;
    return SBK_OK;
}

int sbk_asr_num_frames(const sbk_asr* mm, int n_samples, int* T_feat, int* T_enc) {
    const AsrModel* m = reinterpret_cast<const AsrModel*>(mm);
    int T0, T1, T2;
    frames(m->cfg, n_samples, &T0, &T1, &T2);
    if (T_feat) *T_feat = T0;
    if (T_enc) *T_enc = T2;
    return SBK_OK;
}

int sbk_asr_cnn_forward(sbk_asr* mm, const float* feats_dev, int B, int T0, float* out_dev, void* stream) {
    AsrModel* m = reinterpret_cast<AsrModel*>(mm);
    const sbk_asr_config& c = m->cfg;
    SBK_REQUIRE(m->has_cnn, "cnn_forward: this handle was created without CNN weights");
    const int L = (T0 - 1) * c.hop;
    RC(ensure_workspace(m, B, L, std::max(B, m->ws_rows), std::max(1, m->ws_steps)));
    return cnn_frontend_forward(feats_dev, B, T0, c.n_mels, m->c1_w, m->c1_b, m->c1_g, m->c1_be, c.cnn_c1, m->c2_w, m->c2_b,
                                m->c2_g, m->c2_be, c.cnn_c2, m->b.act1, nullptr, m->b.a_in, out_dev,
                                static_cast<cudaStream_t>(stream));
}

int sbk_asr_encode_feats(sbk_asr* mm, const float* feats_dev, const float* rel_len_dev, int B, int T0,
                         float* cnn_out_dev, float* enc_out_dev, void* stream) {
    AsrModel* m = reinterpret_cast<AsrModel*>(mm);
    cudaStream_t st = static_cast<cudaStream_t>(stream);
    const sbk_asr_config& c = m->cfg;
    const int L = (T0 - 1) * c.hop;
    RC(ensure_workspace(m, B, L, std::max(B, m->ws_rows), std::max(1, m->ws_steps)));
    const int T1 = (T0 - 1) / 2 + 1, T = (T1 - 1) / 2 + 1;
    const int* enc_len = nullptr;
    if (rel_len_dev) {
        abs_len_kernel<<<ceil_div(B, 128), 128, 0, st>>>(rel_len_dev, B, T, m->b.enc_len);
        SBK_LAUNCH_CHECK();
        enc_len = m->b.enc_len;
    }
    return run_encoder(m, feats_dev, B, T0, enc_len, cnn_out_dev, enc_out_dev ? enc_out_dev : m->b.enc_out, st);
}

int sbk_asr_encode_from_cnn(sbk_asr* mm, const float* src_dev, const float* rel_len_dev, int B, int T,
                            float* enc_out_dev, void* stream) {
    AsrModel* m = reinterpret_cast<AsrModel*>(mm);
    cudaStream_t st = static_cast<cudaStream_t>(stream);
    const sbk_asr_config& c = m->cfg;
    const int L = ((T - 1) * 4) * c.hop;
    RC(ensure_workspace(m, B, L, std::max(B, m->ws_rows), std::max(1, m->ws_steps)));
    RC(cast_f32_f16(src_dev, m->b.a_in, (size_t)B * T * c.input_size, st));
    const int* enc_len = nullptr;
    if (rel_len_dev) {
        abs_len_kernel<<<ceil_div(B, 128), 128, 0, st>>>(rel_len_dev, B, T, m->b.enc_len);
        SBK_LAUNCH_CHECK();
        enc_len = m->b.enc_len;
    }
    return run_encoder(m, nullptr, B, T, enc_len, nullptr, enc_out_dev ? enc_out_dev : m->b.enc_out, st);
}

static int transcribe_enqueue(AsrModel* m, const float* wav_dev, const float* rel_len_dev, int B, int L, int max_steps,
                              int bos, int eos, float* enc_out_dev, int* pred_dev, float* score_dev, float* log_probs_dev,
                              int* steps_done, cudaStream_t st, bool in_capture) {
    const sbk_asr_config& c = m->cfg;
    int T0, T1, T;
    frames(c, L, &T0, &T1, &T);
    AsrModel::Buf& b = m->b;
    RC(fbank_forward(m->fbank, wav_dev, B, L, b.feats, b.utt_max, m->glob_mean, m->glob_std, c.norm_eps > 0.0f ? c.norm_eps : 1e-10f, st));
    const int* enc_len = nullptr;
    if (rel_len_dev) {
        abs_len_kernel<<<ceil_div(B, 128), 128, 0, st>>>(rel_len_dev, B, T, b.enc_len);
        SBK_LAUNCH_CHECK();
        enc_len = b.enc_len;
    } else {
        std::vector<int> full(B, T);
        SBK_CUDA_CHECK(cudaMemcpyAsync(b.enc_len, full.data(), B * 4, cudaMemcpyHostToDevice, st));
        SBK_CUDA_CHECK(cudaStreamSynchronize(st));
        enc_len = b.enc_len;
    }
    RC(run_encoder(m, b.feats, B, T0, enc_len, nullptr, b.enc_out, st));
    if (enc_out_dev)
        SBK_CUDA_CHECK(cudaMemcpyAsync(enc_out_dev, b.enc_out, (size_t)B * T * c.d_model * 4, cudaMemcpyDeviceToDevice, st));
    int done = 0;
    if (max_steps > 0 && m->has_dec) {
        RC(run_greedy(m, B, T, max_steps, bos, eos, log_probs_dev, &done, st, in_capture));
        const int S_max = m->ws_steps + 1;
        if (pred_dev)
            SBK_CUDA_CHECK(cudaMemcpy2DAsync(pred_dev, (size_t)max_steps * 4, b.pred, (size_t)S_max * 4, (size_t)done * 4, B,
                                             cudaMemcpyDeviceToDevice, st));
        if (score_dev)
            SBK_CUDA_CHECK(cudaMemcpy2DAsync(score_dev, (size_t)max_steps * 4, b.score, (size_t)S_max * 4, (size_t)done * 4, B,
                                             cudaMemcpyDeviceToDevice, st));
    }
    if (steps_done) *steps_done = done;
    return SBK_OK;
}

static int transcribe_group_enqueue(AsrModel* m, int G, const float* const* wav_dev, const float* const* rel_dev, int B, int L,
                                    int max_steps, int bos, int eos, int* const* pred_dev, int* steps_done, cudaStream_t st,
                                    bool in_capture, const cudaEvent_t* ready = nullptr, int* const* pred_host = nullptr) {
    const sbk_asr_config& c = m->cfg;
    int T0, T1, T;
    frames(c, L, &T0, &T1, &T);
    AsrModel::Buf& b = m->b;
    for (int g = 0; g < G; ++g) {
        if (ready) SBK_CUDA_CHECK(cudaStreamWaitEvent(st, ready[g], 0));
        RC(fbank_forward(m->fbank, wav_dev[g], B, L, b.feats, b.utt_max, m->glob_mean, m->glob_std, c.norm_eps > 0.0f ? c.norm_eps : 1e-10f, st));
        int* enc_len = b.enc_len + (size_t)g * B;
        abs_len_kernel<<<ceil_div(B, 128), 128, 0, st>>>(rel_dev[g], B, T, enc_len);
        SBK_LAUNCH_CHECK();
        RC(run_encoder(m, b.feats, B, T0, enc_len, nullptr, b.enc_out + (size_t)g * B * T * c.d_model, st));
    }
    static const bool prio = getenv("SBK_DEC_PRIORITY") == nullptr || atoi(getenv("SBK_DEC_PRIORITY")) != 0;
    cudaStream_t ds = st;
    if (prio) {
        if (!m->dec_stream) {
            int lo = 0, hi = 0;
            SBK_CUDA_CHECK(cudaDeviceGetStreamPriorityRange(&lo, &hi));
            SBK_CUDA_CHECK(cudaStreamCreateWithPriority(&m->dec_stream, cudaStreamNonBlocking, hi));
            SBK_CUDA_CHECK(cudaEventCreateWithFlags(&m->ev_dfork, cudaEventDisableTiming));
            SBK_CUDA_CHECK(cudaEventCreateWithFlags(&m->ev_djoin, cudaEventDisableTiming));
        }
        ds = m->dec_stream;
        SBK_CUDA_CHECK(cudaEventRecord(m->ev_dfork, st));
        SBK_CUDA_CHECK(cudaStreamWaitEvent(ds, m->ev_dfork, 0));
    }
    int done = 0;
    RC(run_greedy(m, G * B, T, max_steps, bos, eos, nullptr, &done, ds, in_capture));
    const int S_max = m->ws_steps + 1;
    for (int g = 0; g < G; ++g) {
        if (pred_dev && pred_dev[g])
            SBK_CUDA_CHECK(cudaMemcpy2DAsync(pred_dev[g], (size_t)max_steps * 4, b.pred + (size_t)g * B * S_max, (size_t)S_max * 4,
                                             (size_t)done * 4, B, cudaMemcpyDeviceToDevice, ds));
        if (pred_host && pred_host[g])
            SBK_CUDA_CHECK(cudaMemcpy2DAsync(pred_host[g], (size_t)max_steps * 4, b.pred + (size_t)g * B * S_max, (size_t)S_max * 4,
                                             (size_t)done * 4, B, cudaMemcpyDeviceToHost, ds));
    }
    if (prio) {
        SBK_CUDA_CHECK(cudaEventRecord(m->ev_djoin, ds));
        SBK_CUDA_CHECK(cudaStreamWaitEvent(st, m->ev_djoin, 0));
    }
    if (steps_done) *steps_done = done;
    return SBK_OK;
}

static int transcribe_group_host_enqueue(AsrModel* m, int G, const float* const* wav_host, const float* const* rel_host, int B,
                                         int L, int max_steps, int bos, int eos, int* const* pred_host, int* const* pred_dev,
                                         int* steps_done, cudaStream_t st, bool in_capture) {
    SBK_CUDA_CHECK(cudaEventRecord(m->ev_fork, st));
    SBK_CUDA_CHECK(cudaStreamWaitEvent(m->copy_stream, m->ev_fork, 0));
    const float* wav_dev[16];
    const float* rel_dev[16];
    for (int g = 0; g < G; ++g) {
        float* w = m->gwav + (size_t)g * B * L;
        float* r = m->grel + (size_t)g * B;
        SBK_CUDA_CHECK(cudaMemcpyAsync(w, wav_host[g], (size_t)B * L * 4, cudaMemcpyHostToDevice, m->copy_stream));
        SBK_CUDA_CHECK(cudaMemcpyAsync(r, rel_host[g], (size_t)B * 4, cudaMemcpyHostToDevice, m->copy_stream));
        SBK_CUDA_CHECK(cudaEventRecord(m->ev_ready[g], m->copy_stream));
        wav_dev[g] = w; rel_dev[g] = r;
    }
    return transcribe_group_enqueue(m, G, wav_dev, rel_dev, B, L, max_steps, bos, eos, pred_dev, steps_done, st, in_capture,
                                    m->ev_ready, pred_host);
}

int sbk_asr_transcribe_greedy_group_dev(sbk_asr* mm, int G, const float* const* wav_dev, const float* const* rel_len_dev,
                                        int B, int L, int max_steps, int bos, int eos, int* const* pred_dev, int* steps_done,
                                        void* stream) {
    AsrModel* m = reinterpret_cast<AsrModel*>(mm);
    cudaStream_t st = static_cast<cudaStream_t>(stream);
    SBK_REQUIRE(G >= 1 && G <= 16, "transcribe_group: G=%d not in [1, 16]", G);
    SBK_REQUIRE(m->has_fbank && m->has_cnn && m->has_enc && m->has_dec, "transcribe_group: handle lacks model parts");
    SBK_REQUIRE(m->glob_mean != nullptr, "transcribe_group: model has no normalize.glob_mean/std weights");
    for (int g = 0; g < G; ++g) SBK_REQUIRE(wav_dev[g] && rel_len_dev[g], "transcribe_group: null batch pointer");
    RC(ensure_workspace(m, B, L, std::max(G * B, m->ws_rows), std::max(max_steps, m->ws_steps)));
    const bool whole_graph = m->poll_every == 0 && getenv("SBK_NO_GRAPH") == nullptr && max_steps > 0;
    if (!whole_graph) return transcribe_group_enqueue(m, G, wav_dev, rel_len_dev, B, L, max_steps, bos, eos, pred_dev, steps_done, st, false);
    AsrModel::GroupKey key;
    memset(&key, 0, sizeof(key));
    key.G = G; key.B = B; key.L = L; key.steps = max_steps; key.bos = bos; key.eos = eos;
    for (int g = 0; g < G; ++g) { key.wav[g] = wav_dev[g]; key.rel[g] = rel_len_dev[g]; key.pred[g] = pred_dev[g]; }
    if (m->group_graph == nullptr || memcmp(&key, &m->group_key, sizeof(key)) != 0) {
        if (m->group_graph) { cudaGraphExecDestroy(m->group_graph); m->group_graph = nullptr; }
        if (!m->cap_stream) SBK_CUDA_CHECK(cudaStreamCreateWithFlags(&m->cap_stream, cudaStreamNonBlocking));
        cudaGraph_t gr;
        SBK_CUDA_CHECK(cudaStreamBeginCapture(m->cap_stream, cudaStreamCaptureModeThreadLocal));
        launch_count_begin_capture();
        int done = 0;
        int rc = transcribe_group_enqueue(m, G, wav_dev, rel_len_dev, B, L, max_steps, bos, eos, pred_dev, &done, m->cap_stream, true);
        m->group_nodes = launch_count_end_capture();
        cudaError_t ce = cudaStreamEndCapture(m->cap_stream, &gr);
        if (rc) return rc;
        SBK_CUDA_CHECK(ce);
        SBK_CUDA_CHECK(cudaGraphInstantiate(&m->group_graph, gr, 0));
        cudaGraphDestroy(gr);
        m->group_key = key;
    }
    SBK_CUDA_CHECK(cudaGraphLaunch(m->group_graph, st));
    launch_count_add(m->group_nodes);
    if (steps_done) *steps_done = max_steps;
    return SBK_OK;
}

int sbk_asr_transcribe_greedy_group_host_async(sbk_asr* mm, int G, const float* const* wav_host,
                                               const float* const* rel_len_host, int B, int L, int max_steps, int bos, int eos,
                                               int* const* pred_host, int* const* pred_dev, int* steps_done, void* stream) {
    AsrModel* m = reinterpret_cast<AsrModel*>(mm);
    cudaStream_t st = static_cast<cudaStream_t>(stream);
    SBK_REQUIRE(G >= 1 && G <= 16, "transcribe_group_host: G=%d not in [1, 16]", G);
    SBK_REQUIRE(m->has_fbank && m->has_cnn && m->has_enc && m->has_dec, "transcribe_group_host: handle lacks model parts");
    SBK_REQUIRE(m->glob_mean != nullptr, "transcribe_group_host: model has no normalize.glob_mean/std weights");
    SBK_REQUIRE(wav_host && rel_len_host && pred_host, "transcribe_group_host: null argument");
    for (int g = 0; g < G; ++g) SBK_REQUIRE(wav_host[g] && rel_len_host[g] && pred_host[g], "transcribe_group_host: null batch pointer");
    RC(ensure_workspace(m, B, L, std::max(G * B, m->ws_rows), std::max(max_steps, m->ws_steps)));
    const size_t need = (size_t)G * B * L * 4 + (size_t)G * B * 4 + 256;
    if (need > m->gwav_cap) {
        if (m->gwav) { SBK_CUDA_CHECK(cudaDeviceSynchronize()); cudaFree(m->gwav); m->gwav = nullptr; m->gwav_cap = 0; }
        if (m->hgroup_graph) { cudaGraphExecDestroy(m->hgroup_graph); m->hgroup_graph = nullptr; }
        if (cudaMalloc(&m->gwav, need) != cudaSuccess) { set_error("transcribe_group_host: cudaMalloc(%zu) failed", need); return SBK_ERR_NOMEM; }
        m->gwav_cap = need;
    }
    m->grel = m->gwav + (size_t)G * B * L;
    if (!m->copy_stream) {
        SBK_CUDA_CHECK(cudaStreamCreateWithFlags(&m->copy_stream, cudaStreamNonBlocking));
        SBK_CUDA_CHECK(cudaEventCreateWithFlags(&m->ev_fork, cudaEventDisableTiming));
        for (auto& e : m->ev_ready) SBK_CUDA_CHECK(cudaEventCreateWithFlags(&e, cudaEventDisableTiming));
    }
    const bool whole_graph = m->poll_every == 0 && getenv("SBK_NO_GRAPH") == nullptr && max_steps > 0;
    if (!whole_graph)
        return transcribe_group_host_enqueue(m, G, wav_host, rel_len_host, B, L, max_steps, bos, eos, pred_host, pred_dev,
                                             steps_done, st, false);
    AsrModel::HostGroupKey key;
    memset(&key, 0, sizeof(key));
    key.G = G; key.B = B; key.L = L; key.steps = max_steps; key.bos = bos; key.eos = eos;
    for (int g = 0; g < G; ++g) {
        key.wav[g] = wav_host[g]; key.rel[g] = rel_len_host[g]; key.pred[g] = pred_host[g];
        key.pred_dev[g] = pred_dev ? pred_dev[g] : nullptr;
    }
    if (m->hgroup_graph == nullptr || memcmp(&key, &m->hgroup_key, sizeof(key)) != 0) {
        if (m->hgroup_graph) { cudaGraphExecDestroy(m->hgroup_graph); m->hgroup_graph = nullptr; }
        if (!m->cap_stream) SBK_CUDA_CHECK(cudaStreamCreateWithFlags(&m->cap_stream, cudaStreamNonBlocking));
        cudaGraph_t gr;
        SBK_CUDA_CHECK(cudaStreamBeginCapture(m->cap_stream, cudaStreamCaptureModeThreadLocal));
        launch_count_begin_capture();
        int done = 0;
        int rc = transcribe_group_host_enqueue(m, G, wav_host, rel_len_host, B, L, max_steps, bos, eos, pred_host, pred_dev, &done,
                                               m->cap_stream, true);
        m->hgroup_nodes = launch_count_end_capture();
        cudaError_t ce = cudaStreamEndCapture(m->cap_stream, &gr);
        if (rc) return rc;
        SBK_CUDA_CHECK(ce);
        SBK_CUDA_CHECK(cudaGraphInstantiate(&m->hgroup_graph, gr, 0));
        cudaGraphDestroy(gr);
        m->hgroup_key = key;
    }
    SBK_CUDA_CHECK(cudaGraphLaunch(m->hgroup_graph, st));
    launch_count_add(m->hgroup_nodes);
    if (steps_done) *steps_done = max_steps;
    return SBK_OK;
}

int sbk_asr_transcribe_greedy_dev(sbk_asr* mm, const float* wav_dev, const float* rel_len_dev, int B, int L,
                                  int max_steps, int bos, int eos, float* enc_out_dev, int* pred_dev, float* score_dev,
                                  float* log_probs_dev, int* steps_done, void* stream) {
    AsrModel* m = reinterpret_cast<AsrModel*>(mm);
    cudaStream_t st = static_cast<cudaStream_t>(stream);
    SBK_REQUIRE(m->has_fbank && m->has_cnn && m->has_enc, "transcribe: handle lacks fbank/CNN/encoder weights");
    SBK_REQUIRE(m->glob_mean != nullptr, "transcribe: model has no normalize.glob_mean/std (global CMVN) weights");
    RC(ensure_workspace(m, B, L, std::max(B, m->ws_rows), std::max(max_steps, m->ws_steps)));
    const bool whole_graph = m->poll_every == 0 && rel_len_dev != nullptr && log_probs_dev == nullptr &&
                             getenv("SBK_NO_GRAPH") == nullptr && (max_steps == 0 || m->has_dec);
    if (!whole_graph)
        return transcribe_enqueue(m, wav_dev, rel_len_dev, B, L, max_steps, bos, eos, enc_out_dev, pred_dev, score_dev,
                                  log_probs_dev, steps_done, st, false);
    AsrModel::PipeKey key;
    memset(&key, 0, sizeof(key));
    key.wav = wav_dev; key.rel = rel_len_dev; key.enc = enc_out_dev; key.pred = pred_dev; key.score = score_dev;
// ... 192 lines not shown
```

### speechbrain_b200/csrc/gemm_epilogue.cuh

```cuda
#pragma once
#include "common.cuh"
#include "sbk_internal.h"

namespace sbk {

struct EpiPrefetch {
    float4 bias[8];
    float4 res[8];
    bool on = false;
};
__device__ __forceinline__ void epilogue_prefetch(const GemmEpilogue& e, EpiPrefetch& p, int row, int col0, int M, int N) {
    p.on = row < M && col0 + 32 <= N;
    if (!p.on) return;
#pragma unroll
    for (int j = 0; j < 8; ++j)
        p.bias[j] = e.bias != nullptr ? __ldg(reinterpret_cast<const float4*>(e.bias + col0) + j) : make_float4(0.f, 0.f, 0.f, 0.f);
    if (e.mode == EPI_RESID) {
        const float4* r = reinterpret_cast<const float4*>(e.resid + static_cast<size_t>(row) * e.ldo + col0);
#pragma unroll
        for (int j = 0; j < 8; ++j) p.res[j] = __ldcg(r + j);
    }
}

__device__ __forceinline__ void epilogue_chunk(const GemmEpilogue& e, const uint32_t (&acc)[32], int row, int col0,
                                               int M, int N, const EpiPrefetch& pre) {
    if (row >= M || col0 >= N) return;
    const bool full = (col0 + 32 <= N);
    float v[32];
#pragma unroll
    for (int j = 0; j < 32; ++j) v[j] = __uint_as_float(acc[j]);
    if (pre.on) {
#pragma unroll
        for (int j = 0; j < 32; j += 4) {
            const float4 b = pre.bias[j >> 2];
            v[j] += b.x; v[j + 1] += b.y; v[j + 2] += b.z; v[j + 3] += b.w;
        }
    } else if (e.bias != nullptr) {
        if (full) {
#pragma unroll
            for (int j = 0; j < 32; j += 4) {
                const float4 b = __ldg(reinterpret_cast<const float4*>(e.bias + col0 + j));
                v[j] += b.x; v[j + 1] += b.y; v[j + 2] += b.z; v[j + 3] += b.w;
            }
        } else {
#pragma unroll
            for (int j = 0; j < 32; ++j)
                if (col0 + j < N) v[j] += __ldg(e.bias + col0 + j);
        }
    }
    switch (e.mode) {
        case EPI_F16: {
            if (e.act == ACT_SILU) {
#pragma unroll
                for (int j = 0; j < 32; ++j) v[j] = silu_f(v[j]);
            } else if (e.act == ACT_GELU) {
#pragma unroll
                for (int j = 0; j < 32; ++j) v[j] = gelu_erf_f(v[j]);
            } else if (e.act == ACT_RELU) {
#pragma unroll
                for (int j = 0; j < 32; ++j) v[j] = fmaxf(v[j], 0.0f);
            }
            __half* o = reinterpret_cast<__half*>(e.out) + static_cast<size_t>(row) * e.ldo + col0;
            if (full) {
#pragma unroll
                for (int j = 0; j < 32; j += 8) {
                    __half2 h0 = floats2half2_sat(v[j], v[j + 1]), h1 = floats2half2_sat(v[j + 2], v[j + 3]);
                    __half2 h2 = floats2half2_sat(v[j + 4], v[j + 5]), h3 = floats2half2_sat(v[j + 6], v[j + 7]);
                    uint4 u;
                    u.x = *reinterpret_cast<uint32_t*>(&h0); u.y = *reinterpret_cast<uint32_t*>(&h1);
                    u.z = *reinterpret_cast<uint32_t*>(&h2); u.w = *reinterpret_cast<uint32_t*>(&h3);
                    *reinterpret_cast<uint4*>(o + j) = u;
                }
            } else {
#pragma unroll
                for (int j = 0; j < 32; ++j)
                    if (col0 + j < N) o[j] = float2half_sat(v[j]);
            }
            break;
        }
        case EPI_F32: {
            float* o = reinterpret_cast<float*>(e.out) + static_cast<size_t>(row) * e.ldo + col0;
            if (full) {
#pragma unroll
                for (int j = 0; j < 32; j += 4)
                    *reinterpret_cast<float4*>(o + j) = make_float4(v[j], v[j + 1], v[j + 2], v[j + 3]);
            } else {
#pragma unroll
                for (int j = 0; j < 32; ++j)
                    if (col0 + j < N) o[j] = v[j];
            }
            break;
        }
        case EPI_RESID: {
            float alpha = e.alpha;
            if (e.row_lens != nullptr) {
                const int b = row / e.T, t = row - b * e.T;
                if (t >= e.row_lens[b]) alpha = 0.0f;
            }
            const float* r = e.resid + static_cast<size_t>(row) * e.ldo + col0;
            float* o = reinterpret_cast<float*>(e.out) + static_cast<size_t>(row) * e.ldo + col0;
            if (full) {
#pragma unroll
                for (int j = 0; j < 32; j += 4) {
                    const float4 x = pre.on ? pre.res[j >> 2] : *reinterpret_cast<const float4*>(r + j);
                    *reinterpret_cast<float4*>(o + j) = make_float4(fmaf(alpha, v[j], x.x), fmaf(alpha, v[j + 1], x.y),
                                                                    fmaf(alpha, v[j + 2], x.z), fmaf(alpha, v[j + 3], x.w));
                }
            } else {
#pragma unroll
                for (int j = 0; j < 32; ++j)
                    if (col0 + j < N) o[j] = fmaf(alpha, v[j], r[j]);
            }
            break;
        }
        case EPI_QKV_CACHE: {
            const int sect = col0 / e.qkv_d, c = col0 - sect * e.qkv_d;
            __half* o;
            if (sect == 0) o = reinterpret_cast<__half*>(e.out) + static_cast<size_t>(row) * e.ldo + c;
            else o = (sect == 1 ? e.kcache : e.vcache) +
                     (static_cast<size_t>(row) * e.S_max + __ldg(e.step_ptr + row)) * e.qkv_d + c;
#pragma unroll
            for (int j = 0; j < 32; j += 8) {
                __half2 h0 = floats2half2_sat(v[j], v[j + 1]), h1 = floats2half2_sat(v[j + 2], v[j + 3]);
                __half2 h2 = floats2half2_sat(v[j + 4], v[j + 5]), h3 = floats2half2_sat(v[j + 6], v[j + 7]);
                uint4 u;
                u.x = *reinterpret_cast<uint32_t*>(&h0); u.y = *reinterpret_cast<uint32_t*>(&h1);
                u.z = *reinterpret_cast<uint32_t*>(&h2); u.w = *reinterpret_cast<uint32_t*>(&h3);
                *reinterpret_cast<uint4*>(o + j) = u;
            }
            break;
        }
        case EPI_GLU: {
            float* o = reinterpret_cast<float*>(e.out) + static_cast<size_t>(row) * e.ldo + (col0 >> 1);
#pragma unroll
            for (int j = 0; j < 16; j += 4)
                *reinterpret_cast<float4*>(o + j) =
                    make_float4(v[j] * sigmoid_f(v[j + 16]), v[j + 1] * sigmoid_f(v[j + 17]),
                                v[j + 2] * sigmoid_f(v[j + 18]), v[j + 3] * sigmoid_f(v[j + 19]));
            break;
        }
        case EPI_ROPE: {
            const int dh = e.head_dim;
            const int within = col0 % (3 * dh);
            const int sect = within / dh;
            if (sect < 2) {
                const int t = row % e.T;
                const int p0 = (within - sect * dh) >> 1;
                const float* cs = e.rope_cos + static_cast<size_t>(t) * (dh >> 1) + p0;
                const float* sn = e.rope_sin + static_cast<size_t>(t) * (dh >> 1) + p0;
                const float sc = sect == 0 ? e.alpha : 1.0f;
#pragma unroll
                for (int j = 0; j < 32; j += 2) {
                    const float c = __ldg(cs + (j >> 1)), s = __ldg(sn + (j >> 1));
                    const float x0 = v[j], x1 = v[j + 1];
                    v[j] = (x0 * c - x1 * s) * sc;
                    v[j + 1] = (x1 * c + x0 * s) * sc;
                }
            }
            __half* o = reinterpret_cast<__half*>(e.out) + static_cast<size_t>(row) * e.ldo + col0;
#pragma unroll
            for (int j = 0; j < 32; j += 8) {
                __half2 h0 = floats2half2_sat(v[j], v[j + 1]), h1 = floats2half2_sat(v[j + 2], v[j + 3]);
                __half2 h2 = floats2half2_sat(v[j + 4], v[j + 5]), h3 = floats2half2_sat(v[j + 6], v[j + 7]);
                uint4 u;
                u.x = *reinterpret_cast<uint32_t*>(&h0); u.y = *reinterpret_cast<uint32_t*>(&h1);
                u.z = *reinterpret_cast<uint32_t*>(&h2); u.w = *reinterpret_cast<uint32_t*>(&h3);
                *reinterpret_cast<uint4*>(o + j) = u;
            }
            break;
        }
    }
}


constexpr int EPI_STG_PITCH = 144;
constexpr int EPI_STG_BYTES = 32 * EPI_STG_PITCH;

template <int MODE>
__host__ __device__ constexpr int epi_stg_pitch() { return (MODE == EPI_F32 || MODE == EPI_RESID || MODE == EPI_ROPE) ? EPI_STG_PITCH : 80; }

__device__ __forceinline__ void epilogue_resid_prefetch(const GemmEpilogue& e, float4 (&res)[8], int row_base, int col0, int M,
                                                        int lane) {
    const int seg = lane & 7, rsub = lane >> 3;
#pragma unroll
    for (int i = 0; i < 8; ++i) {
        const int row = row_base + i * 4 + rsub;
        res[i] = row < M ? __ldcg(reinterpret_cast<const float4*>(e.resid + static_cast<size_t>(row) * e.ldo + col0 + seg * 4))
                         : make_float4(0.f, 0.f, 0.f, 0.f);
    }
}

__device__ __forceinline__ void epilogue_rope_prefetch(const GemmEpilogue& e, float4 (&rc)[4], float4 (&rs)[4], int row_base,
                                                       int col0, int lane) {
    const int dh = e.head_dim;
    const int within = col0 % (3 * dh);
    const int sect = within / dh;
    if (sect < 2) {
        const int p = ((within - sect * dh) >> 1) + (lane & 3) * 4;
#pragma unroll
        for (int i = 0; i < 4; ++i) {
            const int t = (row_base + i * 8 + (lane >> 2)) % e.T;
            rc[i] = __ldg(reinterpret_cast<const float4*>(e.rope_cos + static_cast<size_t>(t) * (dh >> 1) + p));
            rs[i] = __ldg(reinterpret_cast<const float4*>(e.rope_sin + static_cast<size_t>(t) * (dh >> 1) + p));
        }
    }
}

template <int MODE, int ACT, int PITCH = EPI_STG_PITCH>
__device__ __forceinline__ void epilogue_chunk_coalesced(const GemmEpilogue& e, const uint32_t (&acc)[32], uint8_t* stg,
                                                         int row_base, int col0, int M, int lane, float4 (&res)[8],
                                                         int next_col0, float4 (&rc)[4], float4 (&rs)[4],
                                                         const float* sbias = nullptr) {
    float v[32];
#pragma unroll
    for (int j = 0; j < 32; ++j) v[j] = __uint_as_float(acc[j]);
    if (sbias != nullptr) {
#pragma unroll
        for (int j = 0; j < 32; j += 4) {
            const float4 b = *reinterpret_cast<const float4*>(sbias + j);
            v[j] += b.x; v[j + 1] += b.y; v[j + 2] += b.z; v[j + 3] += b.w;
        }
    } else if (e.bias != nullptr) {
#pragma unroll
        for (int j = 0; j < 32; j += 4) {
            const float4 b = __ldg(reinterpret_cast<const float4*>(e.bias + col0 + j));
            v[j] += b.x; v[j + 1] += b.y; v[j + 2] += b.z; v[j + 3] += b.w;
        }
    }
    const int my_row = row_base + lane;
    const uint32_t stg_s = smem_u32(stg);
    const uint32_t my = stg_s + lane * PITCH;
    constexpr int out_bytes_per_row = (MODE == EPI_F32 || MODE == EPI_RESID) ? 128 : 64;
    {
        if constexpr (MODE == EPI_F32 || MODE == EPI_RESID || MODE == EPI_ROPE) {
            if constexpr (MODE == EPI_RESID) {
                float alpha = e.alpha;
                if (e.row_lens != nullptr && my_row < M) {
                    const int b = my_row / e.T, t = my_row - b * e.T;
                    if (t >= e.row_lens[b]) alpha = 0.0f;
                }
#pragma unroll
                for (int j = 0; j < 32; ++j) v[j] *= alpha;
            }
#pragma unroll
            for (int j = 0; j < 32; j += 4)
                sts128(my + j * 4, f4_as_u4(make_float4(v[j], v[j + 1], v[j + 2], v[j + 3])));
        } else if constexpr (MODE == EPI_GLU) {
            if constexpr (ACT == ACT_SILU_FAST) {
#pragma unroll
                for (int j = 0; j < 16; j += 4)
                    sts128(my + j * 4, f4_as_u4(make_float4(v[j] * sigmoid_fast(v[j + 16]), v[j + 1] * sigmoid_fast(v[j + 17]),
                                                            v[j + 2] * sigmoid_fast(v[j + 18]), v[j + 3] * sigmoid_fast(v[j + 19]))));
            } else {
#pragma unroll
                for (int j = 0; j < 16; j += 4)
                    sts128(my + j * 4, f4_as_u4(make_float4(v[j] * sigmoid_f(v[j + 16]), v[j + 1] * sigmoid_f(v[j + 17]),
                                                            v[j + 2] * sigmoid_f(v[j + 18]), v[j + 3] * sigmoid_f(v[j + 19]))));
            }
        } else {
            if constexpr (ACT == ACT_SILU) {
#pragma unroll
                for (int j = 0; j < 32; ++j) v[j] = silu_f(v[j]);
            } else if constexpr (ACT == ACT_SILU_FAST) {
#pragma unroll
                for (int j = 0; j < 32; ++j) v[j] = silu_fast(v[j]);
            } else if constexpr (ACT == ACT_GELU) {
#pragma unroll
                for (int j = 0; j < 32; ++j) v[j] = gelu_erf_f(v[j]);
            }
#pragma unroll
            for (int j = 0; j < 32; j += 8) {
                __half2 h0 = floats2half2_sat(v[j], v[j + 1]), h1 = floats2half2_sat(v[j + 2], v[j + 3]);
                __half2 h2 = floats2half2_sat(v[j + 4], v[j + 5]), h3 = floats2half2_sat(v[j + 6], v[j + 7]);
                uint4 u;
                u.x = *reinterpret_cast<uint32_t*>(&h0); u.y = *reinterpret_cast<uint32_t*>(&h1);
                u.z = *reinterpret_cast<uint32_t*>(&h2); u.w = *reinterpret_cast<uint32_t*>(&h3);
                sts128(my + j * 2, u);
            }
        }
    }
    __syncwarp();
    if constexpr (out_bytes_per_row == 128) {
        const int seg = lane & 7, rsub = lane >> 3;
        float* outp = reinterpret_cast<float*>(e.out);
#pragma unroll
        for (int i = 0; i < 8; ++i) {
            const int r = i * 4 + rsub;
            const int row = row_base + r;
            if (row < M) {
                float4 val = u4_as_f4(lds128(stg_s + r * PITCH + seg * 16));
                if constexpr (MODE == EPI_RESID) {
                    val.x += res[i].x; val.y += res[i].y; val.z += res[i].z; val.w += res[i].w;
                }
                *reinterpret_cast<float4*>(outp + static_cast<size_t>(row) * e.ldo + col0 + seg * 4) = val;
            }
        }
        if constexpr (MODE == EPI_RESID)
            if (next_col0 >= 0) epilogue_resid_prefetch(e, res, row_base, next_col0, M, lane);
    } else if constexpr (MODE == EPI_ROPE) {
        const int seg = lane & 3, rsub = lane >> 2;
        const int dh = e.head_dim;
        const int sect = (col0 % (3 * dh)) / dh;
        const float sc = sect == 0 ? e.alpha : 1.0f;
        __half* outp = reinterpret_cast<__half*>(e.out);
#pragma unroll
        for (int i = 0; i < 4; ++i) {
            const int r = i * 8 + rsub;
            const int row = row_base + r;
            float4 x0 = u4_as_f4(lds128(stg_s + r * PITCH + seg * 32));
            float4 x1 = u4_as_f4(lds128(stg_s + r * PITCH + seg * 32 + 16));
            if (sect < 2) {
                const float4 c = rc[i], s4 = rs[i];
                const float a0 = (x0.x * c.x - x0.y * s4.x) * sc, a1 = (x0.y * c.x + x0.x * s4.x) * sc;
                const float a2 = (x0.z * c.y - x0.w * s4.y) * sc, a3 = (x0.w * c.y + x0.z * s4.y) * sc;
                const float b0 = (x1.x * c.z - x1.y * s4.z) * sc, b1 = (x1.y * c.z + x1.x * s4.z) * sc;
                const float b2 = (x1.z * c.w - x1.w * s4.w) * sc, b3 = (x1.w * c.w + x1.z * s4.w) * sc;
                x0 = make_float4(a0, a1, a2, a3);
                x1 = make_float4(b0, b1, b2, b3);
            }
            if (row < M) {
                __half2 h0 = floats2half2_sat(x0.x, x0.y), h1 = floats2half2_sat(x0.z, x0.w);
                __half2 h2 = floats2half2_sat(x1.x, x1.y), h3 = floats2half2_sat(x1.z, x1.w);
                uint4 u;
                u.x = *reinterpret_cast<uint32_t*>(&h0); u.y = *reinterpret_cast<uint32_t*>(&h1);
                u.z = *reinterpret_cast<uint32_t*>(&h2); u.w = *reinterpret_cast<uint32_t*>(&h3);
                *reinterpret_cast<uint4*>(outp + static_cast<size_t>(row) * e.ldo + col0 + seg * 8) = u;
            }
        }
        if (next_col0 >= 0) epilogue_rope_prefetch(e, rc, rs, row_base, next_col0, lane);
    } else {
        const int seg = lane & 3, rsub = lane >> 2;
        uint8_t* outp = reinterpret_cast<uint8_t*>(e.out);
        const size_t row_pitch = MODE == EPI_GLU ? static_cast<size_t>(e.ldo) * 4 : static_cast<size_t>(e.ldo) * 2;
        const size_t col_off = static_cast<size_t>(col0) * 2;
        if (MODE == EPI_F16 && e.kv_heads > 0) {
            const int d = e.kv_heads * 64;
            const int part = col0 / d, cc = col0 - part * d, head = cc >> 6, dcol = cc & 63;
            __half* pbase = reinterpret_cast<__half*>(e.out) + static_cast<size_t>(part) * e.kv_part_stride;
#pragma unroll
            for (int i = 0; i < 4; ++i) {
                const int r = i * 8 + rsub;
                const int row = row_base + r;
                if (row < M) {
                    const int b = row / e.T, t = row - b * e.T;
                    __half* dst = pbase + ((static_cast<size_t>(b) * e.kv_heads + head) * e.T + t) * 64 + dcol + seg * 8;
                    *reinterpret_cast<uint4*>(dst) = lds128(stg_s + r * PITCH + seg * 16);
                }
            }
        } else {
#pragma unroll
            for (int i = 0; i < 4; ++i) {
                const int r = i * 8 + rsub;
                const int row = row_base + r;
                if (row < M)
                    *reinterpret_cast<uint4*>(outp + static_cast<size_t>(row) * row_pitch + col_off + seg * 16) =
                        lds128(stg_s + r * PITCH + seg * 16);
            }
        }
    }
    __syncwarp();
}

}
```

### speechbrain_b200/csrc/gemm_tc.cu

```cuda
#include <stdlib.h>

#include "common.cuh"
#include "gemm_epilogue.cuh"
#include "sbk_internal.h"

namespace sbk {

constexpr int GEMM_BM = 128;
constexpr int GEMM_BK = 64;
constexpr int GEMM_THREADS = 192;

template <int BN, int STAGES, int SPLIT = 1>
struct GemmSmem {
    static constexpr int A_BYTES = GEMM_BM * GEMM_BK * 2;
    static constexpr int B_BYTES = BN * GEMM_BK * 2;
    static constexpr int STAGE_BYTES = A_BYTES + B_BYTES;
    static constexpr int BAR_OFFSET = STAGES * STAGE_BYTES;
    static constexpr int PART_OFFSET = BAR_OFFSET + 256;
    static constexpr int PART_BYTES = (SPLIT - 1) * GEMM_BM * BN * 4;
    static constexpr int TOTAL = PART_OFFSET + PART_BYTES + 1024;
};

__device__ __forceinline__ uint32_t gemm_cluster_rank() {
    uint32_t r;
    asm volatile("mov.u32 %0, %%cluster_ctarank;" : "=r"(r));
    return r;
}
__device__ __forceinline__ void gemm_cluster_sync() {
    asm volatile("barrier.cluster.arrive.release.aligned;" ::: "memory");
    asm volatile("barrier.cluster.wait.acquire.aligned;" ::: "memory");
}
__device__ __forceinline__ void st_cluster_f4(const void* local_ptr, uint32_t cta, float a, float b, float c, float d) {
    uint32_t raddr;
    asm volatile("mapa.shared::cluster.u32 %0, %1, %2;" : "=r"(raddr) : "r"(smem_u32(local_ptr)), "r"(cta));
    asm volatile("st.shared::cluster.v4.f32 [%0], {%1, %2, %3, %4};" ::"r"(raddr), "f"(a), "f"(b), "f"(c), "f"(d) : "memory");
}

template <int BN, int STAGES, int SPLIT = 1>
__global__ void __launch_bounds__(GEMM_THREADS, (BN <= 128 ? 2 : 1))
gemm_tc_kernel(const __grid_constant__ CUtensorMap tmap_a, const __grid_constant__ CUtensorMap tmap_b,
               const GemmEpilogue epi, int M, int N, int K) {
    using S = GemmSmem<BN, STAGES, SPLIT>;
    extern __shared__ uint8_t smem_raw[];
    uint8_t* smem = reinterpret_cast<uint8_t*>((reinterpret_cast<uintptr_t>(smem_raw) + 1023) & ~uintptr_t(1023));
    uint64_t* full_bar = reinterpret_cast<uint64_t*>(smem + S::BAR_OFFSET);
    uint64_t* empty_bar = full_bar + STAGES;
    uint64_t* tmem_full_bar = empty_bar + STAGES;
    uint32_t* tmem_base_ptr = reinterpret_cast<uint32_t*>(tmem_full_bar + 1);

    const int warp = threadIdx.x >> 5, lane = threadIdx.x & 31;
    const int n0 = blockIdx.x * BN, m0 = blockIdx.y * GEMM_BM;
    const uint32_t rank = SPLIT > 1 ? gemm_cluster_rank() : 0u;
    const int num_kb = (K + GEMM_BK - 1) / GEMM_BK / SPLIT;
    const int kb0 = static_cast<int>(rank) * num_kb;

    if (warp == 0 && lane == 0) {
        tma_prefetch_desc(&tmap_a);
        tma_prefetch_desc(&tmap_b);
        for (int s = 0; s < STAGES; ++s) {
            mbar_init(&full_bar[s], 1);
            mbar_init(&empty_bar[s], 1);
        }
        mbar_init(tmem_full_bar, 1);
        mbar_fence_init();
    }
    if (warp == 1) tmem_alloc(tmem_base_ptr, BN);
    tc_fence_before();
    __syncthreads();
    if constexpr (SPLIT > 1) gemm_cluster_sync();
    tc_fence_after();
    const uint32_t tmem_base = *tmem_base_ptr;

    if (warp == 0) {
        if (lane == 0) {
            for (int kb = 0; kb < num_kb; ++kb) {
                const int s = kb % STAGES;
                const uint32_t ph = (kb / STAGES) & 1;
                mbar_wait(&empty_bar[s], ph ^ 1);
                mbar_arrive_expect_tx(&full_bar[s], S::STAGE_BYTES);
                uint8_t* a_dst = smem + s * S::STAGE_BYTES;
                tma_load_2d(a_dst, &tmap_a, &full_bar[s], (kb0 + kb) * GEMM_BK, m0);
                tma_load_2d(a_dst + S::A_BYTES, &tmap_b, &full_bar[s], (kb0 + kb) * GEMM_BK, n0);
            }
        }
    } else if (warp == 1) {
        if (lane == 0) {
            const uint32_t idesc = make_idesc_f16(GEMM_BM, BN, 0);
            for (int kb = 0; kb < num_kb; ++kb) {
                const int s = kb % STAGES;
                const uint32_t ph = (kb / STAGES) & 1;
                mbar_wait(&full_bar[s], ph);
                tc_fence_after();
                const uint32_t a_addr = smem_u32(smem + s * S::STAGE_BYTES);
                const uint64_t da = make_kmajor_sw128_desc(a_addr);
                const uint64_t db = make_kmajor_sw128_desc(a_addr + S::A_BYTES);
#pragma unroll
                for (int k = 0; k < GEMM_BK / 16; ++k)
                    umma_f16(tmem_base, da + 2 * k, db + 2 * k, idesc, (kb | k) != 0 ? 1u : 0u);
                umma_commit(&empty_bar[s]);
            }
            umma_commit(tmem_full_bar);
        }
    } else {
        const int q = warp & 3;
        const int row = m0 + q * 32 + lane;
        EpiPrefetch pre;
        if constexpr (BN == 32 && SPLIT == 1) epilogue_prefetch(epi, pre, row, n0, M, N);
        mbar_wait(tmem_full_bar, 0);
        tc_fence_after();
        if constexpr (SPLIT == 1) {
#pragma unroll 1
            for (int c = 0; c < BN / 32; ++c) {
                uint32_t acc[32];
                tmem_ld_32x32(tmem_base + (static_cast<uint32_t>(q * 32) << 16) + c * 32, acc);
                tmem_ld_wait();
                epilogue_chunk(epi, acc, row, n0 + c * 32, M, N, pre);
            }
        } else if (rank != 0) {
            float* part = reinterpret_cast<float*>(smem + S::PART_OFFSET) +
                          (static_cast<size_t>(rank - 1) * GEMM_BM + q * 32 + lane) * BN;
#pragma unroll 1
            for (int c = 0; c < BN / 32; ++c) {
                uint32_t acc[32];
                tmem_ld_32x32(tmem_base + (static_cast<uint32_t>(q * 32) << 16) + c * 32, acc);
                tmem_ld_wait();
#pragma unroll
                for (int j = 0; j < 32; j += 4)
                    st_cluster_f4(part + c * 32 + j, 0, __uint_as_float(acc[j]), __uint_as_float(acc[j + 1]),
                                  __uint_as_float(acc[j + 2]), __uint_as_float(acc[j + 3]));
            }
        }
    }
    if constexpr (SPLIT > 1) {
        tc_fence_before();
        gemm_cluster_sync();
        if (rank == 0 && warp >= 2) {
            tc_fence_after();
            const int q = warp & 3;
            const int row = m0 + q * 32 + lane;
#pragma unroll 1
            for (int c = 0; c < BN / 32; ++c) {
                uint32_t acc[32];
                tmem_ld_32x32(tmem_base + (static_cast<uint32_t>(q * 32) << 16) + c * 32, acc);
                tmem_ld_wait();
#pragma unroll 1
                for (int r = 0; r < SPLIT - 1; ++r) {
                    const float* part = reinterpret_cast<const float*>(smem + S::PART_OFFSET) +
                                        (static_cast<size_t>(r) * GEMM_BM + q * 32 + lane) * BN + c * 32;
#pragma unroll
                    for (int j = 0; j < 32; j += 4) {
                        const float4 p4 = *reinterpret_cast<const float4*>(part + j);
                        acc[j] = __float_as_uint(__uint_as_float(acc[j]) + p4.x);
                        acc[j + 1] = __float_as_uint(__uint_as_float(acc[j + 1]) + p4.y);
                        acc[j + 2] = __float_as_uint(__uint_as_float(acc[j + 2]) + p4.z);
                        acc[j + 3] = __float_as_uint(__uint_as_float(acc[j + 3]) + p4.w);
                    }
                }
                epilogue_chunk(epi, acc, row, n0 + c * 32, M, N, EpiPrefetch());
            }
        }
    }
    tc_fence_before();
    __syncthreads();
    if (warp == 1) tmem_dealloc(tmem_base, BN);
}

template <int BN, int STAGES, int SPLIT = 1>
static int launch_gemm(const void* A, int lda, const void* W, int ldw, const GemmEpilogue& epi, int M, int N, int K,
                       cudaStream_t stream) {
    using S = GemmSmem<BN, STAGES, SPLIT>;
    CUtensorMap ta, tb;
    int rc = make_tmap_2d_f16(&ta, A, M, K, lda, GEMM_BM, GEMM_BK);
    if (rc) return rc;
    rc = make_tmap_2d_f16(&tb, W, N, K, ldw, BN, GEMM_BK);
    if (rc) return rc;
    auto kern = gemm_tc_kernel<BN, STAGES, SPLIT>;
    SBK_CUDA_CHECK(cudaFuncSetAttribute(kern, cudaFuncAttributeMaxDynamicSharedMemorySize, S::TOTAL));
    dim3 grid(ceil_div(N, BN), ceil_div(M, GEMM_BM), SPLIT);
    GemmProfile* prof = gemm_profile();
    cudaEvent_t e0 = nullptr, e1 = nullptr;
    if (prof->enabled) {
        cudaEventCreate(&e0);
        cudaEventCreate(&e1);
        cudaEventRecord(e0, stream);
    }
    if constexpr (SPLIT == 1) {
        kern<<<grid, GEMM_THREADS, S::TOTAL, stream>>>(ta, tb, epi, M, N, K);
    } else {
        cudaLaunchConfig_t cfg = {};
        cfg.gridDim = grid;
        cfg.blockDim = dim3(GEMM_THREADS);
        cfg.dynamicSmemBytes = S::TOTAL;
        cfg.stream = stream;
        cudaLaunchAttribute attr[1];
        attr[0].id = cudaLaunchAttributeClusterDimension;
        attr[0].val.clusterDim.x = 1;
        attr[0].val.clusterDim.y = 1;
        attr[0].val.clusterDim.z = SPLIT;
        cfg.attrs = attr;
        cfg.numAttrs = 1;
        SBK_CUDA_CHECK(cudaLaunchKernelEx(&cfg, kern, ta, tb, epi, M, N, K));
    }
    if (prof->enabled) {
        cudaEventRecord(e1, stream);
        prof->ev.push_back(e0);
        prof->ev.push_back(e1);
        prof->flops.push_back(2.0 * M * N * K);
        prof->shape.insert(prof->shape.end(), {M, N, K, epi.mode});
    }
    SBK_LAUNCH_CHECK();
    return SBK_OK;
}

int gemm_f16_small(const void* A, int lda, const void* W, int ldw, const GemmEpilogue& epi, int M, int N, int K,
                   cudaStream_t stream) {
    SBK_REQUIRE(M > 0 && N > 0 && K > 0, "gemm_f16_small: empty problem M=%d N=%d K=%d", M, N, K);
    SBK_REQUIRE((K % 8) == 0 && (lda % 8) == 0 && (ldw % 8) == 0, "gemm_f16_small: K/lda/ldw must be multiples of 8");
    SBK_REQUIRE((reinterpret_cast<uintptr_t>(A) & 15) == 0 && (reinterpret_cast<uintptr_t>(W) & 15) == 0,
                "gemm_f16_small: operands must be 16-byte aligned");
    SBK_REQUIRE(epi.mode == EPI_F16 || epi.mode == EPI_F32 || epi.mode == EPI_RESID || epi.mode == EPI_QKV_CACHE,
                "gemm_f16_small: epilogue mode %d not supported", epi.mode);
    if (epi.mode == EPI_QKV_CACHE)
        SBK_REQUIRE(epi.qkv_d % 32 == 0 && N == 3 * epi.qkv_d && epi.kcache && epi.vcache && epi.step_ptr,
                    "gemm_f16_small: bad EPI_QKV_CACHE arguments");
    if (N > 2048) return launch_gemm<64, 6>(A, lda, W, ldw, epi, M, N, K, stream);
    static const bool split = getenv("SBK_DEC_SPLITK") != nullptr;
    if (K >= 2048 && K % (4 * GEMM_BK) == 0 && split)
        return launch_gemm<32, 8, 4>(A, lda, W, ldw, epi, M, N, K, stream);
    return launch_gemm<32, 8>(A, lda, W, ldw, epi, M, N, K, stream);
}

int gemm_f16(const void* A, int lda, const void* W, int ldw, const GemmEpilogue& epi, int M, int N, int K,
             cudaStream_t stream) {
    SBK_REQUIRE(M > 0 && N > 0 && K > 0, "gemm_f16: empty problem M=%d N=%d K=%d", M, N, K);
    SBK_REQUIRE((K % 8) == 0 && (lda % 8) == 0 && (ldw % 8) == 0, "gemm_f16: K/lda/ldw must be multiples of 8");
    SBK_REQUIRE((reinterpret_cast<uintptr_t>(A) & 15) == 0 && (reinterpret_cast<uintptr_t>(W) & 15) == 0,
                "gemm_f16: operands must be 16-byte aligned");
    if (epi.mode == EPI_GLU || epi.mode == EPI_ROPE)
        SBK_REQUIRE(N % 32 == 0, "gemm_f16: GLU/RoPE epilogues need N %% 32 == 0");
    if (epi.mode == EPI_ROPE) SBK_REQUIRE(epi.head_dim % 32 == 0, "gemm_f16: RoPE epilogue needs head_dim %% 32 == 0");
    if (N % 256 == 0 && getenv("SBK_GEMM_V1") == nullptr) return gemm_f16_2cta(A, lda, W, ldw, epi, M, N, K, stream);
    return launch_gemm<128, 3>(A, lda, W, ldw, epi, M, N, K, stream);
}

}
```

### speechbrain_b200/csrc/gemm_tc2.cu

```cuda
#include <stdio.h>
#include <stdlib.h>

#include <algorithm>

#include "common.cuh"
#include "gemm_epilogue.cuh"
#include "sbk_internal.h"

namespace sbk {

constexpr int G2_BM = 128;
constexpr int G2_BN = 256;
constexpr int G2_BK = 64;
constexpr int G2_STAGES = 5;
template <int MODE>
constexpr int g2_epi_warps() { return (MODE == EPI_F32 || MODE == EPI_RESID || MODE == EPI_ROPE) ? 8 : 16; }
constexpr int G2_A_BYTES = G2_BM * G2_BK * 2;
template <int BN, int ST>
struct G2Cfg {
    static constexpr int B_BYTES = (BN / 2) * G2_BK * 2;
    static constexpr int STAGE_BYTES = G2_A_BYTES + B_BYTES;
    static constexpr int BAR_OFFSET = ST * STAGE_BYTES;
    static constexpr int STG_OFFSET = BAR_OFFSET + 256;
    static_assert(STAGE_BYTES % 1024 == 0, "128B-swizzled stages must stay 1 KB aligned");
    static_assert((2 * ST + 4) * 8 + 4 <= 256, "barrier block");
};
template <int MODE, int EW, int BN, int ST>
constexpr int g2_bias_offset() { return G2Cfg<BN, ST>::STG_OFFSET + EW * 32 * epi_stg_pitch<MODE>(); }
template <int MODE, int EW, int BN, int ST>
constexpr int g2_smem() { return g2_bias_offset<MODE, EW, BN, ST>() + BN * 4 + 1024; }

__device__ __forceinline__ uint32_t cluster_ctarank() {
    uint32_t r;
    asm volatile("mov.u32 %0, %%cluster_ctarank;" : "=r"(r));
    return r;
}
__device__ __forceinline__ void cluster_sync_all() {
    asm volatile("barrier.cluster.arrive.release.aligned;" ::: "memory");
    asm volatile("barrier.cluster.wait.acquire.aligned;" ::: "memory");
}
__device__ __forceinline__ void mbar_wait_b(uint64_t* bar, uint32_t parity, int tag) {
    for (uint32_t spins = 0; !mbar_try_wait(bar, parity); ++spins) {
        if (spins > (1u << 26)) {
            printf("gemm2: barrier timeout tag=%d block=%d thread=%d\n", tag, blockIdx.x, threadIdx.x);
            __trap();
        }
    }
}
__device__ __forceinline__ void mbar_arrive_remote(uint64_t* bar, uint32_t cta) {
    uint32_t raddr;
    asm volatile("mapa.shared::cluster.u32 %0, %1, %2;" : "=r"(raddr) : "r"(smem_u32(bar)), "r"(cta));
    asm volatile("mbarrier.arrive.shared::cluster.b64 _, [%0];" ::"r"(raddr) : "memory");
}
__device__ __forceinline__ void tma_load_2d_2sm(void* smem_dst, const CUtensorMap* m, uint64_t* bar, int c0, int c1) {
    const uint32_t bar_leader = smem_u32(bar) & 0xFEFFFFFFu;
    asm volatile(
        "cp.async.bulk.tensor.2d.cta_group::2.shared::cluster.global.mbarrier::complete_tx::bytes [%0], [%1, {%3, %4}], [%2];"
        ::"r"(smem_u32(smem_dst)), "l"(reinterpret_cast<uint64_t>(m)), "r"(bar_leader), "r"(c0), "r"(c1)
        : "memory");
}
__device__ __forceinline__ void umma_f16_2sm(uint32_t tmem_d, uint64_t desc_a, uint64_t desc_b, uint32_t idesc,
                                             uint32_t accumulate) {
    asm volatile(
        "{\n\t.reg .pred p;\n\t"
        "setp.ne.b32 p, %4, 0;\n\t"
        "tcgen05.mma.cta_group::2.kind::f16 [%0], %1, %2, %3, p;\n\t}"
        ::"r"(tmem_d), "l"(desc_a), "l"(desc_b), "r"(idesc), "r"(accumulate)
        : "memory");
}
__device__ __forceinline__ void umma_commit_2sm(uint64_t* bar, uint32_t lead_rank) {
    const uint16_t mask = static_cast<uint16_t>(3u << lead_rank);
    asm volatile("tcgen05.commit.cta_group::2.mbarrier::arrive::one.shared::cluster.multicast::cluster.b64 [%0], %1;"
                 ::"r"(smem_u32(bar)), "h"(mask)
                 : "memory");
}
__device__ __forceinline__ void umma_commit_mask(uint64_t* bar, uint16_t mask) {
    asm volatile("tcgen05.commit.cta_group::2.mbarrier::arrive::one.shared::cluster.multicast::cluster.b64 [%0], %1;"
                 ::"r"(smem_u32(bar)), "h"(mask)
                 : "memory");
}
__device__ __forceinline__ void tma_load_2d_2sm_mc(void* smem_dst, const CUtensorMap* m, uint64_t* bar, int c0, int c1,
                                                   uint16_t mask) {
    const uint32_t bar_leader = smem_u32(bar) & 0xFEFFFFFFu;
    asm volatile(
        "cp.async.bulk.tensor.2d.cta_group::2.shared::cluster.global.mbarrier::complete_tx::bytes.multicast::cluster"
        " [%0], [%1, {%3, %4}], [%2], %5;"
        ::"r"(smem_u32(smem_dst)), "l"(reinterpret_cast<uint64_t>(m)), "r"(bar_leader), "r"(c0), "r"(c1), "h"(mask)
        : "memory");
}
__device__ __forceinline__ void tmem_alloc_2sm(uint32_t* smem_result, uint32_t ncols) {
    asm volatile("tcgen05.alloc.cta_group::2.sync.aligned.shared::cta.b32 [%0], %1;" ::"r"(smem_u32(smem_result)),
                 "r"(ncols)
                 : "memory");
    asm volatile("tcgen05.relinquish_alloc_permit.cta_group::2.sync.aligned;" ::: "memory");
}
__device__ __forceinline__ void tmem_dealloc_2sm(uint32_t taddr, uint32_t ncols) {
    asm volatile("tcgen05.dealloc.cta_group::2.sync.aligned.b32 %0, %1;" ::"r"(taddr), "r"(ncols) : "memory");
}

template <int MODE, int ACT, int EW, int BN = G2_BN, int ST = G2_STAGES>
__global__ void __launch_bounds__(64 + 32 * EW, 1)
gemm_tc2_kernel(const __grid_constant__ CUtensorMap tmap_a, const __grid_constant__ CUtensorMap tmap_b,
                const __grid_constant__ CUtensorMap tmap_a64, const GemmEpilogue epi, int M, int N, int K, int mc) {
    using C = G2Cfg<BN, ST>;
    extern __shared__ uint8_t smem_raw[];
    uint8_t* smem = reinterpret_cast<uint8_t*>((reinterpret_cast<uintptr_t>(smem_raw) + 1023) & ~uintptr_t(1023));
    uint64_t* full_bar = reinterpret_cast<uint64_t*>(smem + C::BAR_OFFSET);
    uint64_t* empty_bar = full_bar + ST;
    uint64_t* tmem_full_bar = empty_bar + ST;
    uint64_t* tmem_empty_bar = tmem_full_bar + 2;
    uint32_t* tmem_base_ptr = reinterpret_cast<uint32_t*>(tmem_empty_bar + 2);

    const int warp = threadIdx.x >> 5, lane = threadIdx.x & 31;
    const uint32_t crank = cluster_ctarank();
    const uint32_t rank = crank & 1u;
    const uint32_t lead_rank = crank & ~1u;
    const bool leader = rank == 0;
    const int pair = blockIdx.x >> 1, num_pairs = gridDim.x >> 1;
    const int n_tiles = (N + BN - 1) / BN, m_tiles = (M + 2 * G2_BM - 1) / (2 * G2_BM);
    const int total_tiles = n_tiles * m_tiles;
    const int num_kb = (K + G2_BK - 1) / G2_BK;

    if (warp == 0 && lane == 0) {
        tma_prefetch_desc(&tmap_a);
        tma_prefetch_desc(&tmap_b);
        for (int s = 0; s < ST; ++s) {
            mbar_init(&full_bar[s], 2);
            mbar_init(&empty_bar[s], mc ? 2 : 1);
        }
        for (int i = 0; i < 2; ++i) {
            mbar_init(&tmem_full_bar[i], 1);
            mbar_init(&tmem_empty_bar[i], 2);
        }
        mbar_fence_init();
    }
    cluster_sync_all();
    if (warp == 1) tmem_alloc_2sm(tmem_base_ptr, 512);
    tc_fence_before();
    cluster_sync_all();
    tc_fence_after();
    const uint32_t tmem_base = *tmem_base_ptr;

    if (warp == 0) {
        if (lane == 0) {
            int it = 0;
            for (int tile = pair; tile < total_tiles; tile += num_pairs) {
                const int mt = tile / n_tiles, nt = tile - mt * n_tiles;
                const int m_row = mt * 2 * G2_BM + static_cast<int>(rank) * G2_BM;
                const int n_row = nt * BN + static_cast<int>(rank) * (BN / 2);
                for (int kb = 0; kb < num_kb; ++kb, ++it) {
                    const int s = it % ST;
                    const uint32_t ph = (it / ST) & 1;
                    mbar_wait_b(&empty_bar[s], ph ^ 1, 1);
                    uint8_t* a_dst = smem + s * C::STAGE_BYTES;
                    if (mc) {
                        const int half = static_cast<int>(crank >> 1);
                        tma_load_2d_2sm_mc(a_dst + half * (G2_A_BYTES / 2), &tmap_a64, &full_bar[s], kb * G2_BK,
                                           m_row + half * (G2_BM / 2), static_cast<uint16_t>((1u << crank) | (1u << (crank ^ 2u))));
                    } else {
                        tma_load_2d_2sm(a_dst, &tmap_a, &full_bar[s], kb * G2_BK, m_row);
                    }
                    tma_load_2d_2sm(a_dst + G2_A_BYTES, &tmap_b, &full_bar[s], kb * G2_BK, n_row);
                    if (leader) mbar_arrive_expect_tx(&full_bar[s], 2 * C::STAGE_BYTES);
                    else mbar_arrive_remote(&full_bar[s], lead_rank);
                }
            }
        }
    } else if (warp == 1) {
        if (leader && lane == 0) {
            const uint32_t idesc = make_idesc_f16(2 * G2_BM, BN, 0);
            int it = 0, local_tile = 0;
            for (int tile = pair; tile < total_tiles; tile += num_pairs, ++local_tile) {
                const int buf = local_tile & 1;
                const uint32_t acc_ph = (local_tile >> 1) & 1;
                mbar_wait_b(&tmem_empty_bar[buf], acc_ph ^ 1, 2);
                tc_fence_after();
                const uint32_t d_addr = tmem_base + buf * BN;
                for (int kb = 0; kb < num_kb; ++kb, ++it) {
                    const int s = it % ST;
                    const uint32_t ph = (it / ST) & 1;
                    mbar_wait_b(&full_bar[s], ph, 3);
                    tc_fence_after();
                    const uint32_t a_addr = smem_u32(smem + s * C::STAGE_BYTES);
                    const uint64_t da = make_kmajor_sw128_desc(a_addr);
                    const uint64_t db = make_kmajor_sw128_desc(a_addr + G2_A_BYTES);
#pragma unroll
                    for (int k = 0; k < G2_BK / 16; ++k)
                        umma_f16_2sm(d_addr, da + 2 * k, db + 2 * k, idesc, (kb | k) != 0 ? 1u : 0u);
                    if (mc) umma_commit_mask(&empty_bar[s], 0xF);
                    else umma_commit_2sm(&empty_bar[s], lead_rank);
                }
                umma_commit_2sm(&tmem_full_bar[buf], lead_rank);
            }
        }
    } else {
        const int q = warp & 3;
        constexpr int PARTS = EW / 4, PART_COLS = BN / PARTS, PITCH = epi_stg_pitch<MODE>();
        const int part = (warp - 2) >> 2;
        constexpr int CHUNKS = PART_COLS / 32;
        static_assert(CHUNKS % 2 == 0, "epilogue double buffer needs an even chunk count");
        uint8_t* stg = smem + C::STG_OFFSET + (warp - 2) * 32 * PITCH;
        int local_tile = 0;
        for (int tile = pair; tile < total_tiles; tile += num_pairs, ++local_tile) {
            const int mt = tile / n_tiles, nt = tile - mt * n_tiles;
            const int buf = local_tile & 1;
            const uint32_t acc_ph = (local_tile >> 1) & 1;
            const int row_base = mt * 2 * G2_BM + static_cast<int>(rank) * G2_BM + q * 32;
            const int n0 = nt * BN + part * PART_COLS;
            constexpr int BIAS_OFF = C::STG_OFFSET + EW * 32 * PITCH;
            float* sbias_tile = reinterpret_cast<float*>(smem + BIAS_OFF);
            {
                const int e_tid = (warp - 2) * 32 + lane;
                for (int j = e_tid; j < BN; j += 32 * EW) sbias_tile[j] = epi.bias ? __ldg(epi.bias + nt * BN + j) : 0.0f;
                asm volatile("bar.sync 2, %0;" ::"n"(32 * EW) : "memory");
            }
            const float* sb = sbias_tile + part * PART_COLS;
            float4 res[2][8];
            float4 rcs[4], rsn[4];
            if constexpr (MODE == EPI_RESID) {
                epilogue_resid_prefetch(epi, res[0], row_base, n0, M, lane);
                epilogue_resid_prefetch(epi, res[1], row_base, n0 + 32, M, lane);
            }
            if constexpr (MODE == EPI_ROPE) epilogue_rope_prefetch(epi, rcs, rsn, row_base, n0, lane);
            mbar_wait_b(&tmem_full_bar[buf], acc_ph, 4);
            tc_fence_after();
            const uint32_t t0 = tmem_base + (static_cast<uint32_t>(q * 32) << 16) + buf * BN + part * PART_COLS;
            if constexpr (MODE == EPI_RESID) {
                uint32_t acc1[32];
#pragma unroll 1
                for (int c = 0; c < CHUNKS; c += 2) {
                    tmem_ld_32x32(t0 + c * 32, acc1);
                    tmem_ld_wait();
                    epilogue_chunk_coalesced<MODE, ACT, PITCH>(epi, acc1, stg, row_base, n0 + c * 32, M, lane, res[0],
                                                               c + 2 < CHUNKS ? n0 + (c + 2) * 32 : -1, rcs, rsn, sb + c * 32);
                    tmem_ld_32x32(t0 + (c + 1) * 32, acc1);
                    tmem_ld_wait();
                    epilogue_chunk_coalesced<MODE, ACT, PITCH>(epi, acc1, stg, row_base, n0 + (c + 1) * 32, M, lane, res[1],
                                                               c + 3 < CHUNKS ? n0 + (c + 3) * 32 : -1, rcs, rsn, sb + (c + 1) * 32);
                }
            } else {
                uint32_t acc[2][32];
                tmem_ld_32x32(t0, acc[0]);
#pragma unroll 1
                for (int c = 0; c < CHUNKS; c += 2) {
                    tmem_ld_wait();
                    tmem_ld_32x32(t0 + (c + 1) * 32, acc[1]);
                    epilogue_chunk_coalesced<MODE, ACT, PITCH>(epi, acc[0], stg, row_base, n0 + c * 32, M, lane, res[0],
                                                               n0 + (c + 1) * 32, rcs, rsn, sb + c * 32);
                    tmem_ld_wait();
                    if (c + 2 < CHUNKS) tmem_ld_32x32(t0 + (c + 2) * 32, acc[0]);
                    epilogue_chunk_coalesced<MODE, ACT, PITCH>(epi, acc[1], stg, row_base, n0 + (c + 1) * 32, M, lane, res[0],
                                                               c + 2 < CHUNKS ? n0 + (c + 2) * 32 : -1, rcs, rsn, sb + (c + 1) * 32);
                }
            }
            tc_fence_before();
            asm volatile("bar.sync 1, %0;" ::"n"(32 * EW) : "memory");
            if (warp == 2 && lane == 0) {
                if (leader) mbar_arrive(&tmem_empty_bar[buf]);
                else mbar_arrive_remote(&tmem_empty_bar[buf], lead_rank);
            }
        }
    }
    tc_fence_before();
    cluster_sync_all();
    if (warp == 1) tmem_dealloc_2sm(tmem_base, 512);
}

int gemm_f16_2cta(const void* A, int lda, const void* W, int ldw, const GemmEpilogue& epi, int M, int N, int K,
                  cudaStream_t stream) {
    CUtensorMap ta, tb;
    int rc = make_tmap_2d_f16(&ta, A, M, K, lda, G2_BM, G2_BK);
    if (rc) return rc;
    static const bool bn128_env = getenv("SBK_GEMM_BN128") != nullptr;
    const bool bn128 = bn128_env && (epi.mode == EPI_RESID || epi.mode == EPI_F32) && N % 128 == 0 && N <= 1024;
    const int bn = bn128 ? 128 : G2_BN;
    rc = make_tmap_2d_f16(&tb, W, N, K, ldw, bn / 2, G2_BK);
    if (rc) return rc;
    void (*kern)(const CUtensorMap, const CUtensorMap, const CUtensorMap, const GemmEpilogue, int, int, int, int) = nullptr;
    int smem = 0, threads = 0;
#define G2_PICK(MODE, ACT)                                                        \
    do {                                                                          \
        constexpr int EW = g2_epi_warps<MODE>();                                  \
        kern = gemm_tc2_kernel<MODE, ACT, EW>;                                    \
        smem = g2_smem<MODE, EW, G2_BN, G2_STAGES>();                             \
        threads = 64 + 32 * EW;                                                   \
    } while (0)
#define G2_PICK_BN128(MODE)                                                       \
    do {                                                                          \
        kern = gemm_tc2_kernel<MODE, ACT_NONE, 8, 128, 7>;                        \
        smem = g2_smem<MODE, 8, 128, 7>();                                        \
        threads = 64 + 32 * 8;                                                    \
    } while (0)
    static const bool fast_act = getenv("SBK_SILU_EXACT") == nullptr;
    switch (epi.mode) {
        case EPI_F16:
            if (epi.act == ACT_SILU && fast_act) G2_PICK(EPI_F16, ACT_SILU_FAST);
            else if (epi.act == ACT_SILU) G2_PICK(EPI_F16, ACT_SILU);
            else if (epi.act == ACT_GELU) G2_PICK(EPI_F16, ACT_GELU);
            else if (epi.act == ACT_NONE) G2_PICK(EPI_F16, ACT_NONE);
            else { set_error("gemm_f16_2cta: activation %d not built", epi.act); return SBK_ERR_ARG; }
            break;
        case EPI_F32:
            if (bn128) G2_PICK_BN128(EPI_F32);
            else G2_PICK(EPI_F32, ACT_NONE);
            break;
        case EPI_RESID:
            if (bn128) G2_PICK_BN128(EPI_RESID);
            else G2_PICK(EPI_RESID, ACT_NONE);
            break;
        case EPI_GLU:
            if (fast_act) G2_PICK(EPI_GLU, ACT_SILU_FAST);
            else G2_PICK(EPI_GLU, ACT_NONE);
            break;
        case EPI_ROPE: G2_PICK(EPI_ROPE, ACT_NONE); break;
        default: set_error("gemm_f16_2cta: bad epilogue mode %d", epi.mode); return SBK_ERR_ARG;
    }
#undef G2_PICK
#undef G2_PICK_BN128
    SBK_CUDA_CHECK(cudaFuncSetAttribute(kern, cudaFuncAttributeMaxDynamicSharedMemorySize, smem));
    static int num_sms = 0;
    if (num_sms == 0) {
        int dev = 0;
        cudaGetDevice(&dev);
        cudaDeviceGetAttribute(&num_sms, cudaDevAttrMultiProcessorCount, dev);
    }
    const int n_tiles = ceil_div(N, bn), m_tiles = ceil_div(M, 2 * G2_BM);
    static const int pairs_env = getenv("SBK_GEMM_PAIRS") ? atoi(getenv("SBK_GEMM_PAIRS")) : 0;
    const int max_pairs = num_sms / 2, tiles = n_tiles * m_tiles;
    int pairs = std::min(max_pairs, tiles);
    if (pairs_env > 0) pairs = std::min(pairs, pairs_env);
    else pairs = ceil_div(tiles, ceil_div(tiles, max_pairs));
    static const bool mc_env = getenv("SBK_GEMM_MC") != nullptr;
    static const bool cl4_env = getenv("SBK_GEMM_CL4") != nullptr || mc_env;
    int cluster = 2, mc = 0;
    CUtensorMap ta64 = ta;
    if (cl4_env && n_tiles % 2 == 0 && pairs >= 2) {
        if (mc_env) {
            mc = 1;
            rc = make_tmap_2d_f16(&ta64, A, M, K, lda, G2_BM / 2, G2_BK);
            if (rc) return rc;
        }
        cluster = 4;
        pairs &= ~1;
        static int max_cl4[64] = {0};
        int& cap = max_cl4[(epi.mode * 8 + epi.act) & 63];
        if (cap == 0) {
            cudaLaunchConfig_t q = {};
            q.gridDim = dim3(num_sms / 4 * 4); q.blockDim = dim3(threads); q.dynamicSmemBytes = smem;
            cudaLaunchAttribute qa[1];
            qa[0].id = cudaLaunchAttributeClusterDimension;
            qa[0].val.clusterDim.x = 4; qa[0].val.clusterDim.y = 1; qa[0].val.clusterDim.z = 1;
            q.attrs = qa; q.numAttrs = 1;
            int nc = 0;
            if (cudaOccupancyMaxActiveClusters(&nc, reinterpret_cast<const void*>(kern), &q) != cudaSuccess || nc < 1) nc = 1;
            cap = nc;
            if (getenv("SBK_GEMM_TRACE")) fprintf(stderr, "gemm2: %d resident clusters of 4 for mode %d\n", nc, epi.mode);
        }
        pairs = std::min(pairs, 2 * cap);
    }
    GemmProfile* prof = gemm_profile();
    cudaEvent_t e0 = nullptr, e1 = nullptr;
    if (prof->enabled) {
        cudaEventCreate(&e0);
        cudaEventCreate(&e1);
        cudaEventRecord(e0, stream);
    }
    {
        cudaLaunchConfig_t cfg = {};
        cfg.gridDim = dim3(2 * pairs); cfg.blockDim = dim3(threads); cfg.dynamicSmemBytes = smem; cfg.stream = stream;
        cudaLaunchAttribute at[1];
        at[0].id = cudaLaunchAttributeClusterDimension;
        at[0].val.clusterDim.x = cluster; at[0].val.clusterDim.y = 1; at[0].val.clusterDim.z = 1;
        cfg.attrs = at; cfg.numAttrs = 1;
        SBK_CUDA_CHECK(cudaLaunchKernelEx(&cfg, kern, ta, tb, ta64, epi, M, N, K, mc));
    }
    if (prof->enabled) {
        cudaEventRecord(e1, stream);
        prof->ev.push_back(e0);
        prof->ev.push_back(e1);
        prof->flops.push_back(2.0 * M * N * K);
        prof->shape.insert(prof->shape.end(), {M, N, K, epi.mode});
    }
    SBK_LAUNCH_CHECK();
    return SBK_OK;
}

}
```

### speechbrain_b200/csrc/sbk_internal.h

```cpp
#pragma once
#include <cuda_fp16.h>
#include <cuda_runtime.h>
#include <stdint.h>

#include <vector>

namespace sbk {

enum GemmEpiMode { EPI_F16 = 0, EPI_F32 = 1, EPI_RESID = 2, EPI_GLU = 3, EPI_ROPE = 4, EPI_QKV_CACHE = 5 };
enum GemmAct { ACT_NONE = 0, ACT_SILU = 1, ACT_GELU = 2, ACT_RELU = 3, ACT_SILU_FAST = 4  };

struct GemmEpilogue {
    int mode = EPI_F16;
    int act = ACT_NONE;
    const float* bias = nullptr;
    void* out = nullptr;
    int ldo = 0;
    const float* resid = nullptr;
    float alpha = 1.0f;
    const int* row_lens = nullptr;
    int T = 1;
    const float* rope_cos = nullptr;
    const float* rope_sin = nullptr;
    int head_dim = 64;
    __half* kcache = nullptr; __half* vcache = nullptr; const int* step_ptr = nullptr; int S_max = 0; int qkv_d = 0;
    int kv_heads = 0; size_t kv_part_stride = 0;
};

int gemm_f16(const void* A, int lda, const void* W, int ldw, const GemmEpilogue& epi, int M, int N, int K,
             cudaStream_t stream);
int gemm_f16_small(const void* A, int lda, const void* W, int ldw, const GemmEpilogue& epi, int M, int N, int K,
                   cudaStream_t stream);
int gemm_f16_2cta(const void* A, int lda, const void* W, int ldw, const GemmEpilogue& epi, int M, int N, int K,
                  cudaStream_t stream);


const char* last_error();
void launch_count_begin_capture();
long long launch_count_end_capture();
void launch_count_add(long long n);
long long launch_count();

struct GemmProfile {
    bool enabled = false;
    std::vector<cudaEvent_t> ev;
    std::vector<double> flops;
    std::vector<int> shape;
};
GemmProfile* gemm_profile();

struct Fbank;
int fbank_create(Fbank** out, int n_fft, int hop, int n_mels, const float* window_host, const float* mel_matrix_host,
                 float amin, float top_db);
void fbank_destroy(Fbank* fb);
int fbank_num_frames(const Fbank* fb, int L);
int fbank_forward(const Fbank* fb, const float* wav, int B, int L, float* out, int* utt_max, const float* mean,
                  const float* stdv, float eps, cudaStream_t stream);
int global_norm_forward(const float* x, float* out, int B, int T, int F, const float* mean, const float* stdv,
                        float eps, cudaStream_t stream);
int sentence_norm_forward(const float* x, float* out, const float* rel_len, int B, int T, int F, int std_norm,
                          int avoid_padding_norm, float eps, cudaStream_t stream);

int cnn_frontend_forward(const float* feats, int B, int T0, int F0, const float* w1, const float* b1, const float* g1,
                         const float* be1, int C1, const __half* w2p, const float* b2, const float* g2,
                         const float* be2, int C2, __half* act1_h, float* act1_f, __half* out_h, float* out_f,
                         cudaStream_t stream);

int layernorm_rows(const float* x, void* out, bool out_half, const float* gamma, const float* beta, int M, int D,
                   float eps, bool act_silu, cudaStream_t stream);
int layernorm2_rows(const float* x, float* y_out, void* z_out, bool z_half, const float* ga, const float* ba, float eps_a,
                    const float* gb, const float* bb, float eps_b, int M, int D, cudaStream_t stream);
int cast_f32_f16(const float* in, __half* out, size_t n, cudaStream_t stream);
int dwconv_ln_swish(const float* glu, int B, int T, int D, int K, const float* wdw, const float* bdw,
                    const float* gamma, const float* beta, float eps, __half* out, cudaStream_t stream, int chunk = 0);
int encoder_attention(const __half* qkv, int ld, int B, int T, int H, int head_dim, const int* lens, bool relpos,
                      const float* pos_u, const float* pos_v, const __half* P, int ldp, float scale, __half* out,
                      int ldo, cudaStream_t stream, int chunk = 0, int left_chunks = -1);

enum SkinnyEpi { SK_F16 = 0, SK_F16_GELU = 1, SK_F32 = 2, SK_RESID = 3, SK_QKV_CACHE = 4, SK_F16_RELU = 5 };
struct SkinnyArgs {
    const __half* A; int lda;
    const __half* W; int ldw;
    const float* bias;
    int n_rows, N, K, epi;
    void* out; int ldo;
    __half* kcache; __half* vcache;
    const int* step_ptr; int S_max; int d; float q_scale;
    const float* X; const float* ln_g; const float* ln_b; float ln_eps;
};
void set_pdl(bool on);
int skinny_gemm(const SkinnyArgs& a, cudaStream_t stream);
struct DecAttnArgs {
    const __half* q; int ldq;
    const __half* kbase; const __half* vbase;
    size_t row_stride;
    int key_stride;
    int head_stride = 0;
    int rows_per_block;
    const int* n_keys_ptr;
    const int* enc_len;
    int n_keys_fixed;
    int H, dh;
    __half* out; int ldo;
    const int* lineage; int lin_stride;
    const int* tok_cache; int pad_tok;
};
int dec_attention(const DecAttnArgs& a, int n_rows, int max_keys, cudaStream_t stream);
int make_tmap_kv_f16(CUtensorMap* out, const void* base, int n_utt, int T, int H, uint64_t key_stride_elems,
                     uint64_t utt_stride_elems, int box_T);
struct BeamLm {
    const float* emb = nullptr; const float* pe = nullptr; int d = 0;
    float* x = nullptr; __half* x16 = nullptr; int* tok_cache = nullptr;
};
struct BeamStepArgs {
    const float* logits; int V; int beam; int S_max;
    float* seq_scores; int* lineage; int* step_arr; int* finished; int* n_full;
    int* hist_tok; int* hist_pred; float* hist_score; float* hist_lp;
    float temperature, eos_threshold, minus_inf;
    int min_steps, eos, use_eos_threshold, length_norm;
    const float* emb; const float* pe; int d; float* x_next;
    const float* add_scores;
    BeamLm lm;
    float attn_weight = 1.0f;
    int blank = -1;
    float add_const = 0.0f;
    const float* add_row = nullptr;
    float* scratch = nullptr;
};
struct CoverageStep {
    const __half* q; int ldq; const __half* kbase; size_t utt_stride; int key_stride; const int* enc_len;
    int head_stride = 0;
    int rows_per_utt, T, H; float* cov_base; const int* hist_pred; const int* step_ptr; int n_bh;
    float threshold, weight; float* out;
};
int coverage_score(const CoverageStep& p, cudaStream_t stream);
struct CtcStep {
    const float* x; const float* xlin; const float* xb; const int* enc_len;
    float* rsum_base; float* rb_base; float* psi_base;
    float* tab; float* tabM;
    const int* hist_tok; const int* hist_pred;
    const int* step_ptr;
    int n_bh, bos, T, V, beam, blank, eos;
    float weight; float* out; int accumulate;
};
int ctc_prefix_reset(float* x, float* xlin, float* xb, const int* enc_len, int B, int T, int V, int blank, int beam, float* rsum,
                     float* rb, float* psi_prev, float* tab, float* tabM, cudaStream_t stream);
int ctc_prefix_score(const CtcStep& p, cudaStream_t stream);
int rows_logsoftmax_argmax(float* x, int rows, int V, bool do_logsoftmax, int* idx, cudaStream_t stream);
int ctc_prefix_update(const CtcStep& p, cudaStream_t stream);
int beam_reset(int n_bh, int beam, int S_max, int bos, int* step_arr, float* seq_scores, int* lineage, int* finished,
               int* n_full, const float* emb, const float* pe, int d, float* x, const BeamLm* lm, cudaStream_t stream);
int layernorm_dual(float* x, __half* x16, const float* gamma, const float* beta, int M, int D, float eps, bool write_f32,
                   cudaStream_t stream);
int weighted_log_softmax(const float* logits, float* out, int rows, int V, float temperature, float weight,
                         cudaStream_t stream);
int beam_step(const BeamStepArgs& p, int B, cudaStream_t stream);
int greedy_reset(int* tokens, int tok_stride, int n_rows, int bos, int* step_arr, int* has_ended, int* ended_count,
                 const float* emb, const float* pe, int d, float* x, cudaStream_t stream);
int greedy_select(const float* logits, int n_rows, int V, int* step_arr, int eos, int* tokens, int tok_stride,
                  int* has_ended, int* ended_count, int* pred, float* score, int out_stride, float* log_probs, int L,
                  const float* emb, const float* pe, int d, float* x_next, cudaStream_t stream);

}
```

Baseline: 63890.

## Fuse residual add and LayerNorm into 2-CTA GEMM epilogue for encoder

Adds an EPI_RESID_LN epilogue mode where a CTA pair covers the full row width (N=256 or 512). The residual sum is kept in tensor memory, and row mean and variance are reduced across epilogue warps so the following LayerNorm, or two chained LayerNorms at layer boundaries, is applied in place. In the Conformer encoder this replaces each separate layernorm_rows launch and the extra f32 round-trip through global memory. The cost is a full-width N tile per CTA pair, which gives fewer tiles and less parallelism, plus more shared memory and serial epilogue work that could lengthen the GEMM tail.

Measured after the change: 65300 (median of 6 runs). +2.2%, better.

```diff
diff --git a/include/sbk.h b/include/sbk.h
--- a/include/sbk.h
+++ b/include/sbk.h
@@ -66,6 +66,10 @@
                       int act, int M, int N, int K, void* stream);
 int sbk_gemm_f16_resid_test(const void* A_dev, const void* W_dev, const float* bias_dev, float* x_dev, float alpha,
                             int M, int N, int K, void* stream);
+int sbk_gemm_f16_resid_ln_test(const void* A_dev, const void* W_dev, const float* bias_dev, float* x_dev, int has_resid,
+                               float alpha, const int* row_lens_dev, int T, const float* ga, const float* ba, float eps_a,
+                               const float* gb, const float* bb, float eps_b, int store_y, void* ln_out_dev, int ln_out_f32,
+                               int M, int N, int K, void* stream);
 
 int sbk_asr_create(const sbk_asr_config* cfg, const sbk_tensor* weights, int n_weights, sbk_asr** out);
 void sbk_asr_destroy(sbk_asr* m);
diff --git a/speechbrain_b200/_lib.py b/speechbrain_b200/_lib.py
--- a/speechbrain_b200/_lib.py
+++ b/speechbrain_b200/_lib.py
@@ -38,6 +38,7 @@
 EXPORTS = [
     "sbk_last_error", "sbk_version", "sbk_launch_count", "sbk_gemm_profile_enable", "sbk_gemm_profile_read", "sbk_fbank_create", "sbk_fbank_destroy", "sbk_fbank_num_frames",
     "sbk_fbank_forward", "sbk_input_norm_global", "sbk_input_norm_sentence", "sbk_gemm_f16_test", "sbk_gemm_f16_resid_test",
+    "sbk_gemm_f16_resid_ln_test",
     "sbk_asr_create", "sbk_asr_destroy", "sbk_asr_num_frames", "sbk_asr_cnn_forward", "sbk_asr_encode_from_cnn",
     "sbk_asr_encode_feats", "sbk_asr_greedy_from_enc", "sbk_asr_transcribe_greedy_dev",
     "sbk_asr_transcribe_greedy_host", "sbk_asr_transcribe_greedy_host_async", "sbk_asr_clone",
diff --git a/speechbrain_b200/csrc/common.cuh b/speechbrain_b200/csrc/common.cuh
--- a/speechbrain_b200/csrc/common.cuh
+++ b/speechbrain_b200/csrc/common.cuh
@@ -144,6 +144,18 @@
         : "memory");
 }
 __device__ __forceinline__ void tmem_ld_wait() { asm volatile("tcgen05.wait::ld.sync.aligned;" ::: "memory"); }
+__device__ __forceinline__ void tmem_st_32x32(uint32_t taddr, const uint32_t (&r)[32]) {
+    asm volatile(
+        "tcgen05.st.sync.aligned.32x32b.x32.b32 [%0], "
+        "{%1, %2, %3, %4, %5, %6, %7, %8, %9, %10, %11, %12, %13, %14, %15, %16, "
+        "%17, %18, %19, %20, %21, %22, %23, %24, %25, %26, %27, %28, %29, %30, %31, %32};"
+        ::"r"(taddr), "r"(r[0]), "r"(r[1]), "r"(r[2]), "r"(r[3]), "r"(r[4]), "r"(r[5]), "r"(r[6]), "r"(r[7]), "r"(r[8]),
+          "r"(r[9]), "r"(r[10]), "r"(r[11]), "r"(r[12]), "r"(r[13]), "r"(r[14]), "r"(r[15]), "r"(r[16]), "r"(r[17]),
+          "r"(r[18]), "r"(r[19]), "r"(r[20]), "r"(r[21]), "r"(r[22]), "r"(r[23]), "r"(r[24]), "r"(r[25]), "r"(r[26]),
+          "r"(r[27]), "r"(r[28]), "r"(r[29]), "r"(r[30]), "r"(r[31])
+        : "memory");
+}
+__device__ __forceinline__ void tmem_st_wait() { asm volatile("tcgen05.wait::st.sync.aligned;" ::: "memory"); }
 
 __device__ __forceinline__ uint64_t make_kmajor_sw128_desc(uint32_t smem_addr) {
     uint64_t d = 0;
diff --git a/speechbrain_b200/csrc/engine.cu b/speechbrain_b200/csrc/engine.cu
--- a/speechbrain_b200/csrc/engine.cu
+++ b/speechbrain_b200/csrc/engine.cu
@@ -602,18 +602,31 @@
     if (feats != nullptr)
         RC(cnn_frontend_forward(feats, B, T0, c.n_mels, m->c1_w, m->c1_b, m->c1_g, m->c1_be, c.cnn_c1, m->c2_w, m->c2_b,
                                 m->c2_g, m->c2_be, c.cnn_c2, b.act1, nullptr, b.a_in, cnn_out_f, st));
+    const bool fuse_ln = c.num_encoder_layers > 0 && gemm_resid_ln_supported(d);
+    auto resid_ln = [&](GemmEpilogue e, const void* A, int K, const __half* W, const float* g, const float* be) -> int {
+        if (fuse_ln) {
+            e.mode = EPI_RESID_LN; e.ln_ga = g; e.ln_ba = be; e.ln_eps_a = 1e-5f; e.ln_out = b.h16;
+            return gemm_f16(A, K, W, K, e, M, d, K, st);
+        }
+        RC(gemm_f16(A, K, W, K, e, M, d, K, st));
+        return layernorm_rows(b.x, b.h16, true, g, be, M, d, 1e-5f, false, st);
+    };
     GemmEpilogue e;
-    e.mode = EPI_F32; e.bias = m->b_in; e.out = b.x; e.ldo = d;
-    RC(gemm_f16(b.a_in, c.input_size, m->w_in, c.input_size, e, M, d, c.input_size, st));
+    if (fuse_ln) {
+        e.bias = m->b_in; e.out = b.x; e.ldo = d;
+        RC(resid_ln(e, b.a_in, c.input_size, m->w_in, m->enc[0].ffn1_ln_g, m->enc[0].ffn1_ln_b));
+    } else {
+        e.mode = EPI_F32; e.bias = m->b_in; e.out = b.x; e.ldo = d;
+        RC(gemm_f16(b.a_in, c.input_size, m->w_in, c.input_size, e, M, d, c.input_size, st));
+    }
     const float att_scale = 1.0f / sqrtf((float)d);
     for (int l = 0; l < c.num_encoder_layers; ++l) {
         const EncLayerW& w = m->enc[l];
-        if (l == 0) RC(layernorm_rows(b.x, b.h16, true, w.ffn1_ln_g, w.ffn1_ln_b, M, d, 1e-5f, false, st));
+        if (l == 0 && !fuse_ln) RC(layernorm_rows(b.x, b.h16, true, w.ffn1_ln_g, w.ffn1_ln_b, M, d, 1e-5f, false, st));
         e = GemmEpilogue(); e.mode = EPI_F16; e.act = ACT_SILU; e.bias = w.ffn1_b1; e.out = b.f16; e.ldo = F;
         RC(gemm_f16(b.h16, d, w.ffn1_w1, d, e, M, F, d, st));
         e = GemmEpilogue(); e.mode = EPI_RESID; e.bias = w.ffn1_b2; e.out = b.x; e.resid = b.x; e.ldo = d; e.alpha = 0.5f;
-        RC(gemm_f16(b.f16, F, w.ffn1_w2, F, e, M, d, F, st));
-        RC(layernorm_rows(b.x, b.h16, true, w.norm1_g, w.norm1_b, M, d, 1e-5f, false, st));
+        RC(resid_ln(e, b.f16, F, w.ffn1_w2, w.norm1_g, w.norm1_b));
         e = GemmEpilogue(); e.out = b.qkv16; e.ldo = 3 * d;
         if (c.attention_type == SBK_ATT_ROPE) {
             e.mode = EPI_ROPE; e.alpha = att_scale; e.T = T; e.rope_cos = m->rope_cos; e.rope_sin = m->rope_sin; e.head_dim = dh;
@@ -628,18 +641,29 @@
         RC(encoder_attention(b.qkv16, 3 * d, B, T, H, dh, enc_len, c.attention_type == SBK_ATT_RELPOS, w.pos_u, w.pos_v,
                              b.P16, d, att_scale, b.att16, d, st, m->dyn_chunk, m->dyn_left));
         e = GemmEpilogue(); e.mode = EPI_RESID; e.bias = w.bo; e.out = b.x; e.resid = b.x; e.ldo = d; e.alpha = 1.0f;
-        RC(gemm_f16(b.att16, d, w.wo, d, e, M, d, d, st));
-        RC(layernorm_rows(b.x, b.h16, true, w.conv_ln_g, w.conv_ln_b, M, d, 1e-5f, false, st));
+        RC(resid_ln(e, b.att16, d, w.wo, w.conv_ln_g, w.conv_ln_b));
         e = GemmEpilogue(); e.mode = EPI_GLU; e.bias = w.bpw1; e.out = b.glu; e.ldo = d;
         RC(gemm_f16(b.h16, d, w.wpw1, d, e, M, 2 * d, d, st));
         RC(dwconv_ln_swish(b.glu, B, T, d, c.kernel_size, w.wdw, w.bdw, w.aconv_ln_g, w.aconv_ln_b, 1e-5f, b.h16, st, m->dyn_chunk));
         e = GemmEpilogue(); e.mode = EPI_RESID; e.bias = w.bpw2; e.out = b.x; e.resid = b.x; e.ldo = d; e.alpha = 1.0f;
         e.row_lens = enc_len; e.T = T;
-        RC(gemm_f16(b.h16, d, w.wpw2, d, e, M, d, d, st));
-        RC(layernorm_rows(b.x, b.h16, true, w.ffn2_ln_g, w.ffn2_ln_b, M, d, 1e-5f, false, st));
+        RC(resid_ln(e, b.h16, d, w.wpw2, w.ffn2_ln_g, w.ffn2_ln_b));
         e = GemmEpilogue(); e.mode = EPI_F16; e.act = ACT_SILU; e.bias = w.ffn2_b1; e.out = b.f16; e.ldo = F;
         RC(gemm_f16(b.h16, d, w.ffn2_w1, d, e, M, F, d, st));
         e = GemmEpilogue(); e.mode = EPI_RESID; e.bias = w.ffn2_b2; e.out = b.x; e.resid = b.x; e.ldo = d; e.alpha = 0.5f;
+        if (fuse_ln) {
+            const bool last = l + 1 == c.num_encoder_layers;
+            e.mode = EPI_RESID_LN; e.ln_ga = w.norm2_g; e.ln_ba = w.norm2_b; e.ln_eps_a = 1e-5f;
+            if (!last) {
+                e.ln_gb = m->enc[l + 1].ffn1_ln_g; e.ln_bb = m->enc[l + 1].ffn1_ln_b; e.ln_eps_b = 1e-5f;
+                e.ln_store_y = 1; e.ln_out = b.h16;
+            } else {
+                e.ln_gb = m->enc_norm_g; e.ln_bb = m->enc_norm_b; e.ln_eps_b = 1e-6f;
+                e.ln_out = enc_out; e.ln_out_f32 = 1;
+            }
+            RC(gemm_f16(b.f16, F, w.ffn2_w2, F, e, M, d, F, st));
+            continue;
+        }
         RC(gemm_f16(b.f16, F, w.ffn2_w2, F, e, M, d, F, st));
         if (l + 1 < c.num_encoder_layers) {
             const EncLayerW& nx = m->enc[l + 1];
@@ -1263,6 +1287,25 @@
     return gemm_f16(A_dev, K, W_dev, K, e, M, N, K, static_cast<cudaStream_t>(stream));
 }
 
+int sbk_gemm_f16_resid_ln_test(const void* A_dev, const void* W_dev, const float* bias_dev, float* x_dev, int has_resid,
+                               float alpha, const int* row_lens_dev, int T, const float* ga, const float* ba, float eps_a,
+                               const float* gb, const float* bb, float eps_b, int store_y, void* ln_out_dev, int ln_out_f32,
+                               int M, int N, int K, void* stream) {
+    GemmEpilogue e;
+    e.mode = EPI_RESID_LN;
+    e.bias = bias_dev;
+    e.out = x_dev;
+    e.resid = has_resid ? x_dev : nullptr;
+    e.alpha = alpha;
+    e.row_lens = row_lens_dev;
+    e.T = T;
+    e.ldo = N;
+    e.ln_ga = ga; e.ln_ba = ba; e.ln_eps_a = eps_a;
+    e.ln_gb = gb; e.ln_bb = bb; e.ln_eps_b = eps_b;
+    e.ln_store_y = store_y; e.ln_out = ln_out_dev; e.ln_out_f32 = ln_out_f32;
+    return gemm_f16(A_dev, K, W_dev, K, e, M, N, K, static_cast<cudaStream_t>(stream));
+}
+
 int sbk_asr_create(const sbk_asr_config* cfg, const sbk_tensor* weights, int n_weights, sbk_asr** out) {
     return asr_create(cfg, weights, n_weights, reinterpret_cast<AsrModel**>(out));
 }
diff --git a/speechbrain_b200/csrc/gemm_epilogue.cuh b/speechbrain_b200/csrc/gemm_epilogue.cuh
--- a/speechbrain_b200/csrc/gemm_epilogue.cuh
+++ b/speechbrain_b200/csrc/gemm_epilogue.cuh
@@ -177,7 +177,9 @@
 constexpr int EPI_STG_BYTES = 32 * EPI_STG_PITCH;
 
 template <int MODE>
-__host__ __device__ constexpr int epi_stg_pitch() { return (MODE == EPI_F32 || MODE == EPI_RESID || MODE == EPI_ROPE) ? EPI_STG_PITCH : 80; }
+__host__ __device__ constexpr int epi_stg_pitch() {
+    return (MODE == EPI_F32 || MODE == EPI_RESID || MODE == EPI_ROPE || MODE == EPI_RESID_LN) ? EPI_STG_PITCH : 80;
+}
 
 __device__ __forceinline__ void epilogue_resid_prefetch(const GemmEpilogue& e, float4 (&res)[8], int row_base, int col0, int M,
                                                         int lane) {
@@ -185,7 +187,7 @@
 #pragma unroll
     for (int i = 0; i < 8; ++i) {
         const int row = row_base + i * 4 + rsub;
-        res[i] = row < M ? __ldcg(reinterpret_cast<const float4*>(e.resid + static_cast<size_t>(row) * e.ldo + col0 + seg * 4))
+        res[i] = row < M && e.resid != nullptr ? __ldcg(reinterpret_cast<const float4*>(e.resid + static_cast<size_t>(row) * e.ldo + col0 + seg * 4))
                          : make_float4(0.f, 0.f, 0.f, 0.f);
     }
 }
@@ -361,4 +363,80 @@
     __syncwarp();
 }
 
-}
+
+__device__ __forceinline__ void resid_ln_x_chunk(const GemmEpilogue& e, uint32_t (&acc)[32], uint8_t* stg, int row_base,
+                                                  int col0, int M, int lane, float4 (&res)[8], int next_col0,
+                                                  const float* sbias, float alpha, bool store) {
+    const uint32_t stg_s = smem_u32(stg);
+    const uint32_t my = stg_s + lane * EPI_STG_PITCH;
+#pragma unroll
+    for (int j = 0; j < 32; j += 4) {
+        const float4 b = *reinterpret_cast<const float4*>(sbias + j);
+        sts128(my + j * 4, f4_as_u4(make_float4(alpha * (__uint_as_float(acc[j]) + b.x), alpha * (__uint_as_float(acc[j + 1]) + b.y),
+                                                alpha * (__uint_as_float(acc[j + 2]) + b.z), alpha * (__uint_as_float(acc[j + 3]) + b.w))));
+    }
+    __syncwarp();
+    const int seg = lane & 7, rsub = lane >> 3;
+    float* outp = reinterpret_cast<float*>(e.out);
+#pragma unroll
+    for (int i = 0; i < 8; ++i) {
+        const int r = i * 4 + rsub;
+        const int row = row_base + r;
+        const uint32_t a = stg_s + r * EPI_STG_PITCH + seg * 16;
+        float4 val = u4_as_f4(lds128(a));
+        val.x += res[i].x; val.y += res[i].y; val.z += res[i].z; val.w += res[i].w;
+        if (store && row < M) *reinterpret_cast<float4*>(outp + static_cast<size_t>(row) * e.ldo + col0 + seg * 4) = val;
+        sts128(a, f4_as_u4(val));
+    }
+    if (next_col0 >= 0) epilogue_resid_prefetch(e, res, row_base, next_col0, M, lane);
+    __syncwarp();
+#pragma unroll
+    for (int j = 0; j < 32; j += 4) {
+        const uint4 u = lds128(my + j * 4);
+        acc[j] = u.x; acc[j + 1] = u.y; acc[j + 2] = u.z; acc[j + 3] = u.w;
+    }
+    __syncwarp();
+}
+
+__device__ __forceinline__ void ln_store_chunk(const float (&v)[32], uint8_t* stg, void* out, bool out_f32, int ldo,
+                                               int row_base, int col0, int M, int lane) {
+    const uint32_t stg_s = smem_u32(stg);
+    const uint32_t my = stg_s + lane * EPI_STG_PITCH;
+    if (out_f32) {
+#pragma unroll
+        for (int j = 0; j < 32; j += 4) sts128(my + j * 4, f4_as_u4(make_float4(v[j], v[j + 1], v[j + 2], v[j + 3])));
+        __syncwarp();
+        const int seg = lane & 7, rsub = lane >> 3;
+        float* outp = reinterpret_cast<float*>(out);
+#pragma unroll
+        for (int i = 0; i < 8; ++i) {
+            const int row = row_base + i * 4 + rsub;
+            if (row < M)
+                *reinterpret_cast<uint4*>(outp + static_cast<size_t>(row) * ldo + col0 + seg * 4) =
+                    lds128(stg_s + (i * 4 + rsub) * EPI_STG_PITCH + seg * 16);
+        }
+    } else {
+#pragma unroll
+        for (int j = 0; j < 32; j += 8) {
+            __half2 h0 = floats2half2_sat(v[j], v[j + 1]), h1 = floats2half2_sat(v[j + 2], v[j + 3]);
+            __half2 h2 = floats2half2_sat(v[j + 4], v[j + 5]), h3 = floats2half2_sat(v[j + 6], v[j + 7]);
+            uint4 u;
+            u.x = *reinterpret_cast<uint32_t*>(&h0); u.y = *reinterpret_cast<uint32_t*>(&h1);
+            u.z = *reinterpret_cast<uint32_t*>(&h2); u.w = *reinterpret_cast<uint32_t*>(&h3);
+            sts128(my + j * 2, u);
+        }
+        __syncwarp();
+        const int seg = lane & 3, rsub = lane >> 2;
+        __half* outp = reinterpret_cast<__half*>(out);
+#pragma unroll
+        for (int i = 0; i < 4; ++i) {
+            const int row = row_base + i * 8 + rsub;
+            if (row < M)
+                *reinterpret_cast<uint4*>(outp + static_cast<size_t>(row) * ldo + col0 + seg * 8) =
+                    lds128(stg_s + (i * 8 + rsub) * EPI_STG_PITCH + seg * 16);
+        }
+    }
+    __syncwarp();
+}
+
+}
diff --git a/speechbrain_b200/csrc/gemm_tc.cu b/speechbrain_b200/csrc/gemm_tc.cu
--- a/speechbrain_b200/csrc/gemm_tc.cu
+++ b/speechbrain_b200/csrc/gemm_tc.cu
@@ -239,6 +239,8 @@
     if (epi.mode == EPI_GLU || epi.mode == EPI_ROPE)
         SBK_REQUIRE(N % 32 == 0, "gemm_f16: GLU/RoPE epilogues need N %% 32 == 0");
     if (epi.mode == EPI_ROPE) SBK_REQUIRE(epi.head_dim % 32 == 0, "gemm_f16: RoPE epilogue needs head_dim %% 32 == 0");
+    if (epi.mode == EPI_RESID_LN)
+        SBK_REQUIRE(gemm_resid_ln_supported(N), "gemm_f16: residual + LayerNorm epilogue not available for N=%d", N);
     if (N % 256 == 0 && getenv("SBK_GEMM_V1") == nullptr) return gemm_f16_2cta(A, lda, W, ldw, epi, M, N, K, stream);
     return launch_gemm<128, 3>(A, lda, W, ldw, epi, M, N, K, stream);
 }
diff --git a/speechbrain_b200/csrc/gemm_tc2.cu b/speechbrain_b200/csrc/gemm_tc2.cu
--- a/speechbrain_b200/csrc/gemm_tc2.cu
+++ b/speechbrain_b200/csrc/gemm_tc2.cu
@@ -14,21 +14,31 @@
 constexpr int G2_BK = 64;
 constexpr int G2_STAGES = 5;
 template <int MODE>
-constexpr int g2_epi_warps() { return (MODE == EPI_F32 || MODE == EPI_RESID || MODE == EPI_ROPE) ? 8 : 16; }
+constexpr int g2_epi_warps() {
+    return (MODE == EPI_F32 || MODE == EPI_RESID || MODE == EPI_ROPE || MODE == EPI_RESID_LN) ? 8 : 16;
+}
 constexpr int G2_A_BYTES = G2_BM * G2_BK * 2;
+constexpr int G2_W_BOX = 128;
 template <int BN, int ST>
 struct G2Cfg {
-    static constexpr int B_BYTES = (BN / 2) * G2_BK * 2;
+    static constexpr int NH = BN / 256;
+    static constexpr int B_BYTES = G2_W_BOX * G2_BK * 2;
     static constexpr int STAGE_BYTES = G2_A_BYTES + B_BYTES;
     static constexpr int BAR_OFFSET = ST * STAGE_BYTES;
     static constexpr int STG_OFFSET = BAR_OFFSET + 256;
+    static constexpr int NBUF = 512 / BN;
+    static_assert(BN == 256 || BN == 512, "tile width");
     static_assert(STAGE_BYTES % 1024 == 0, "128B-swizzled stages must stay 1 KB aligned");
     static_assert((2 * ST + 4) * 8 + 4 <= 256, "barrier block");
 };
 template <int MODE, int EW, int BN, int ST>
 constexpr int g2_bias_offset() { return G2Cfg<BN, ST>::STG_OFFSET + EW * 32 * epi_stg_pitch<MODE>(); }
+template <int MODE, int EW, int BN>
+constexpr int g2_ln_bytes() { return MODE == EPI_RESID_LN ? 4 * BN * 4 + 4 * G2_BM * 4 + G2_BM * 17 * 4 : 0; }
 template <int MODE, int EW, int BN, int ST>
-constexpr int g2_smem() { return g2_bias_offset<MODE, EW, BN, ST>() + BN * 4 + 1024; }
+constexpr int g2_smem() { return g2_bias_offset<MODE, EW, BN, ST>() + BN * 4 + g2_ln_bytes<MODE, EW, BN>() + 1024; }
+static_assert(g2_smem<EPI_RESID_LN, 8, 512, G2_STAGES>() <= 232448, "BN = 512 shared memory");
+static_assert(g2_smem<EPI_RESID_LN, 8, 256, G2_STAGES>() <= 232448, "BN = 256 LN shared memory");
 
 __device__ __forceinline__ uint32_t cluster_ctarank() {
     uint32_t r;
@@ -147,8 +157,9 @@
             for (int tile = pair; tile < total_tiles; tile += num_pairs) {
                 const int mt = tile / n_tiles, nt = tile - mt * n_tiles;
                 const int m_row = mt * 2 * G2_BM + static_cast<int>(rank) * G2_BM;
-                const int n_row = nt * BN + static_cast<int>(rank) * (BN / 2);
-                for (int kb = 0; kb < num_kb; ++kb, ++it) {
+                const int n_row = nt * BN + static_cast<int>(rank) * G2_W_BOX;
+                for (int hk = 0; hk < C::NH * num_kb; ++hk, ++it) {
+                    const int h = hk / num_kb, kb = hk - h * num_kb;
                     const int s = it % ST;
                     const uint32_t ph = (it / ST) & 1;
                     mbar_wait_b(&empty_bar[s], ph ^ 1, 1);
@@ -160,7 +171,7 @@
                     } else {
                         tma_load_2d_2sm(a_dst, &tmap_a, &full_bar[s], kb * G2_BK, m_row);
                     }
-                    tma_load_2d_2sm(a_dst + G2_A_BYTES, &tmap_b, &full_bar[s], kb * G2_BK, n_row);
+                    tma_load_2d_2sm(a_dst + G2_A_BYTES, &tmap_b, &full_bar[s], kb * G2_BK, n_row + 256 * h);
                     if (leader) mbar_arrive_expect_tx(&full_bar[s], 2 * C::STAGE_BYTES);
                     else mbar_arrive_remote(&full_bar[s], lead_rank);
                 }
@@ -168,29 +179,31 @@
         }
     } else if (warp == 1) {
         if (leader && lane == 0) {
-            const uint32_t idesc = make_idesc_f16(2 * G2_BM, BN, 0);
+            const uint32_t idesc = make_idesc_f16(2 * G2_BM, 256, 0);
             int it = 0, local_tile = 0;
             for (int tile = pair; tile < total_tiles; tile += num_pairs, ++local_tile) {
-                const int buf = local_tile & 1;
-                const uint32_t acc_ph = (local_tile >> 1) & 1;
+                const int buf = local_tile % C::NBUF;
+                const uint32_t acc_ph = (local_tile / C::NBUF) & 1;
                 mbar_wait_b(&tmem_empty_bar[buf], acc_ph ^ 1, 2);
                 tc_fence_after();
-                const uint32_t d_addr = tmem_base + buf * BN;
-                for (int kb = 0; kb < num_kb; ++kb, ++it) {
-                    const int s = it % ST;
-                    const uint32_t ph = (it / ST) & 1;
-                    mbar_wait_b(&full_bar[s], ph, 3);
-                    tc_fence_after();
-                    const uint32_t a_addr = smem_u32(smem + s * C::STAGE_BYTES);
-                    const uint64_t da = make_kmajor_sw128_desc(a_addr);
-                    const uint64_t db = make_kmajor_sw128_desc(a_addr + G2_A_BYTES);
-#pragma unroll
-                    for (int k = 0; k < G2_BK / 16; ++k)
-                        umma_f16_2sm(d_addr, da + 2 * k, db + 2 * k, idesc, (kb | k) != 0 ? 1u : 0u);
-                    if (mc) umma_commit_mask(&empty_bar[s], 0xF);
-                    else umma_commit_2sm(&empty_bar[s], lead_rank);
-                }
-                umma_commit_2sm(&tmem_full_bar[buf], lead_rank);
+                for (int h = 0; h < C::NH; ++h) {
+                    const uint32_t d_addr = tmem_base + buf * BN + 256 * h;
+                    for (int kb = 0; kb < num_kb; ++kb, ++it) {
+                        const int s = it % ST;
+                        const uint32_t ph = (it / ST) & 1;
+                        mbar_wait_b(&full_bar[s], ph, 3);
+                        tc_fence_after();
+                        const uint32_t a_addr = smem_u32(smem + s * C::STAGE_BYTES);
+                        const uint64_t da = make_kmajor_sw128_desc(a_addr);
+                        const uint64_t db = make_kmajor_sw128_desc(a_addr + G2_A_BYTES);
+#pragma unroll
+                        for (int k = 0; k < G2_BK / 16; ++k)
+                            umma_f16_2sm(d_addr, da + 2 * k, db + 2 * k, idesc, (kb | k) != 0 ? 1u : 0u);
+                        if (mc) umma_commit_mask(&empty_bar[s], 0xF);
+                        else umma_commit_2sm(&empty_bar[s], lead_rank);
+                    }
+                    umma_commit_2sm(&tmem_full_bar[buf + h], lead_rank);
+                }
             }
         }
     } else {
@@ -200,15 +213,29 @@
         constexpr int CHUNKS = PART_COLS / 32;
         static_assert(CHUNKS % 2 == 0, "epilogue double buffer needs an even chunk count");
         uint8_t* stg = smem + C::STG_OFFSET + (warp - 2) * 32 * PITCH;
+        if constexpr (MODE == EPI_RESID_LN) {
+            float* sln = reinterpret_cast<float*>(smem + C::STG_OFFSET + EW * 32 * PITCH) + BN;
+            for (int j = (warp - 2) * 32 + lane; j < BN; j += 32 * EW) {
+                sln[j] = __ldg(epi.ln_ga + j);
+                sln[BN + j] = __ldg(epi.ln_ba + j);
+                if (epi.ln_gb != nullptr) {
+                    sln[2 * BN + j] = __ldg(epi.ln_gb + j);
+                    sln[3 * BN + j] = __ldg(epi.ln_bb + j);
+                }
+            }
+        }
         int local_tile = 0;
         for (int tile = pair; tile < total_tiles; tile += num_pairs, ++local_tile) {
             const int mt = tile / n_tiles, nt = tile - mt * n_tiles;
-            const int buf = local_tile & 1;
-            const uint32_t acc_ph = (local_tile >> 1) & 1;
+            const int buf = local_tile % C::NBUF;
+            const uint32_t acc_ph = (local_tile / C::NBUF) & 1;
             const int row_base = mt * 2 * G2_BM + static_cast<int>(rank) * G2_BM + q * 32;
             const int n0 = nt * BN + part * PART_COLS;
             constexpr int BIAS_OFF = C::STG_OFFSET + EW * 32 * PITCH;
             float* sbias_tile = reinterpret_cast<float*>(smem + BIAS_OFF);
+            float* sln = sbias_tile + BN;
+            float* sred = sln + 4 * BN;
+            float* sxch = sred + 4 * G2_BM;
             {
                 const int e_tid = (warp - 2) * 32 + lane;
                 for (int j = e_tid; j < BN; j += 32 * EW) sbias_tile[j] = epi.bias ? __ldg(epi.bias + nt * BN + j) : 0.0f;
@@ -217,15 +244,125 @@
             const float* sb = sbias_tile + part * PART_COLS;
             float4 res[2][8];
             float4 rcs[4], rsn[4];
-            if constexpr (MODE == EPI_RESID) {
+            if constexpr (MODE == EPI_RESID || MODE == EPI_RESID_LN) {
                 epilogue_resid_prefetch(epi, res[0], row_base, n0, M, lane);
                 epilogue_resid_prefetch(epi, res[1], row_base, n0 + 32, M, lane);
             }
             if constexpr (MODE == EPI_ROPE) epilogue_rope_prefetch(epi, rcs, rsn, row_base, n0, lane);
-            mbar_wait_b(&tmem_full_bar[buf], acc_ph, 4);
+            mbar_wait_b(&tmem_full_bar[buf + part * PART_COLS / 256], acc_ph, 4);
             tc_fence_after();
             const uint32_t t0 = tmem_base + (static_cast<uint32_t>(q * 32) << 16) + buf * BN + part * PART_COLS;
-            if constexpr (MODE == EPI_RESID) {
+            if constexpr (MODE == EPI_RESID_LN) {
+                static_assert(PARTS == 2 && BN % 128 == 0, "row statistics assume two warps per lane quarter");
+                constexpr int NI = BN / 128;
+                const uint32_t trow = tmem_base + (static_cast<uint32_t>(q * 32) << 16) + buf * BN;
+                const int my_row = row_base + lane, r128 = q * 32 + lane;
+                float alpha = epi.alpha;
+                if (epi.row_lens != nullptr && my_row < M) {
+                    const int b = my_row / epi.T, t = my_row - b * epi.T;
+                    if (t >= epi.row_lens[b]) alpha = 0.0f;
+                }
+                const bool chained = epi.ln_gb != nullptr;
+                uint32_t acc1[32];
+                auto row_stat = [&](bool sq, float mean, int slot, bool tmem_written) -> float {
+                    if (tmem_written) {
+                        tc_fence_before();
+                        asm volatile("bar.sync 1, %0;" ::"n"(32 * EW) : "memory");
+                        tc_fence_after();
+                    }
+                    float sl[16];
+#pragma unroll
+                    for (int L = 0; L < 16; ++L) sl[L] = 0.0f;
+#pragma unroll
+                    for (int i = 0; i < NI; ++i) {
+#pragma unroll
+                        for (int c2 = 0; c2 < 2; ++c2) {
+                            tmem_ld_32x32(trow + (i * 4 + 2 * part + c2) * 32, acc1);
+                            tmem_ld_wait();
+#pragma unroll
+                            for (int g = 0; g < 8; ++g) {
+                                const float x0 = __uint_as_float(acc1[4 * g]), x1 = __uint_as_float(acc1[4 * g + 1]);
+                                const float x2 = __uint_as_float(acc1[4 * g + 2]), x3 = __uint_as_float(acc1[4 * g + 3]);
+                                float& a = sl[8 * c2 + g];
+                                if (!sq) {
+                                    a += (x0 + x1) + (x2 + x3);
+                                } else {
+                                    float d = x0 - mean; a += d * d;
+                                    d = x1 - mean; a += d * d;
+                                    d = x2 - mean; a += d * d;
+                                    d = x3 - mean; a += d * d;
+                                }
+                            }
+                        }
+                    }
+                    float* xch = sxch + r128 * 17;
+                    float* red = sred + slot * G2_BM;
+                    if (part == 0) {
+#pragma unroll
+                        for (int L = 0; L < 16; ++L) xch[L] = sl[L];
+                        asm volatile("bar.sync 1, %0;" ::"n"(32 * EW) : "memory");
+                        asm volatile("bar.sync 1, %0;" ::"n"(32 * EW) : "memory");
+                        return red[r128];
+                    }
+                    asm volatile("bar.sync 1, %0;" ::"n"(32 * EW) : "memory");
+#pragma unroll
+                    for (int L = 0; L < 16; ++L) sl[L] = xch[L] + sl[L];
+#pragma unroll
+                    for (int w = 8; w >= 1; w >>= 1)
+#pragma unroll
+                        for (int L = 0; L < w; ++L) sl[L] = sl[L] + sl[L + w];
+                    red[r128] = sl[0];
+                    asm volatile("bar.sync 1, %0;" ::"n"(32 * EW) : "memory");
+                    return sl[0];
+                };
+#pragma unroll 1
+                for (int c = 0; c < CHUNKS; c += 2) {
+                    tmem_ld_32x32(t0 + c * 32, acc1);
+                    tmem_ld_wait();
+                    resid_ln_x_chunk(epi, acc1, stg, row_base, n0 + c * 32, M, lane, res[0], c + 2 < CHUNKS ? n0 + (c + 2) * 32 : -1,
+                                     sb + c * 32, alpha, !(chained && epi.ln_store_y));
+                    tmem_st_32x32(t0 + c * 32, acc1);
+                    tmem_ld_32x32(t0 + (c + 1) * 32, acc1);
+                    tmem_ld_wait();
+                    resid_ln_x_chunk(epi, acc1, stg, row_base, n0 + (c + 1) * 32, M, lane, res[1],
+                                     c + 3 < CHUNKS ? n0 + (c + 3) * 32 : -1, sb + (c + 1) * 32, alpha, !(chained && epi.ln_store_y));
+                    tmem_st_32x32(t0 + (c + 1) * 32, acc1);
+                }
+                tmem_st_wait();
+#pragma unroll 1
+                for (int ln = 0; ln < (chained ? 2 : 1); ++ln) {
+                    const float* g = sln + 2 * BN * ln + part * PART_COLS;
+                    const float* bt = g + BN;
+                    const float mean = row_stat(false, 0.0f, 2 * ln, true) / BN;
+                    const float rstd =
+                        rsqrtf(row_stat(true, mean, 2 * ln + 1, false) / BN + (ln == 0 ? epi.ln_eps_a : epi.ln_eps_b));
+                    const bool last = ln == (chained ? 1 : 0);
+#pragma unroll 1
+                    for (int c = 0; c < CHUNKS; ++c) {
+                        tmem_ld_32x32(t0 + c * 32, acc1);
+                        tmem_ld_wait();
+                        float y[32];
+#pragma unroll
+                        for (int j = 0; j < 32; j += 4) {
+                            const float4 gg = *reinterpret_cast<const float4*>(g + c * 32 + j);
+                            const float4 bb = *reinterpret_cast<const float4*>(bt + c * 32 + j);
+                            y[j] = (__uint_as_float(acc1[j]) - mean) * rstd * gg.x + bb.x;
+                            y[j + 1] = (__uint_as_float(acc1[j + 1]) - mean) * rstd * gg.y + bb.y;
+                            y[j + 2] = (__uint_as_float(acc1[j + 2]) - mean) * rstd * gg.z + bb.z;
+                            y[j + 3] = (__uint_as_float(acc1[j + 3]) - mean) * rstd * gg.w + bb.w;
+                        }
+                        if (last) {
+                            ln_store_chunk(y, stg, epi.ln_out, epi.ln_out_f32 != 0, epi.ldo, row_base, n0 + c * 32, M, lane);
+                        } else {
+                            if (epi.ln_store_y) ln_store_chunk(y, stg, epi.out, true, epi.ldo, row_base, n0 + c * 32, M, lane);
+#pragma unroll
+                            for (int j = 0; j < 32; ++j) acc1[j] = __float_as_uint(y[j]);
+                            tmem_st_32x32(t0 + c * 32, acc1);
+                        }
+                    }
+                    tmem_st_wait();
+                }
+            } else if constexpr (MODE == EPI_RESID) {
                 uint32_t acc1[32];
 #pragma unroll 1
                 for (int c = 0; c < CHUNKS; c += 2) {
@@ -266,15 +403,18 @@
     if (warp == 1) tmem_dealloc_2sm(tmem_base, 512);
 }
 
+bool gemm_resid_ln_supported(int N) { return (N == 256 || N == 512) && getenv("SBK_GEMM_V1") == nullptr; }
+
 int gemm_f16_2cta(const void* A, int lda, const void* W, int ldw, const GemmEpilogue& epi, int M, int N, int K,
                   cudaStream_t stream) {
     CUtensorMap ta, tb;
     int rc = make_tmap_2d_f16(&ta, A, M, K, lda, G2_BM, G2_BK);
     if (rc) return rc;
-    static const bool bn128_env = getenv("SBK_GEMM_BN128") != nullptr;
-    const bool bn128 = bn128_env && (epi.mode == EPI_RESID || epi.mode == EPI_F32) && N % 128 == 0 && N <= 1024;
-    const int bn = bn128 ? 128 : G2_BN;
-    rc = make_tmap_2d_f16(&tb, W, N, K, ldw, bn / 2, G2_BK);
+    if (epi.mode == EPI_RESID_LN)
+        SBK_REQUIRE(gemm_resid_ln_supported(N) && epi.ln_ga && epi.ln_ba && epi.ln_out && epi.out,
+                    "gemm_f16_2cta: EPI_RESID_LN needs N = 256 or 512 and LayerNorm operands (N=%d)", N);
+    const int bn = epi.mode == EPI_RESID_LN ? N : G2_BN;
+    rc = make_tmap_2d_f16(&tb, W, N, K, ldw, G2_W_BOX, G2_BK);
     if (rc) return rc;
     void (*kern)(const CUtensorMap, const CUtensorMap, const CUtensorMap, const GemmEpilogue, int, int, int, int) = nullptr;
     int smem = 0, threads = 0;
@@ -285,11 +425,12 @@
         smem = g2_smem<MODE, EW, G2_BN, G2_STAGES>();                             \
         threads = 64 + 32 * EW;                                                   \
     } while (0)
-#define G2_PICK_BN128(MODE)                                                       \
+#define G2_PICK_LN(BN, ST)                                                        \
     do {                                                                          \
-        kern = gemm_tc2_kernel<MODE, ACT_NONE, 8, 128, 7>;                        \
-        smem = g2_smem<MODE, 8, 128, 7>();                                        \
-        threads = 64 + 32 * 8;                                                    \
+        constexpr int EW = g2_epi_warps<EPI_RESID_LN>();                          \
+        kern = gemm_tc2_kernel<EPI_RESID_LN, ACT_NONE, EW, BN, ST>;               \
+        smem = g2_smem<EPI_RESID_LN, EW, BN, ST>();                               \
+        threads = 64 + 32 * EW;                                                   \
     } while (0)
     static const bool fast_act = getenv("SBK_SILU_EXACT") == nullptr;
     switch (epi.mode) {
@@ -300,13 +441,11 @@
             else if (epi.act == ACT_NONE) G2_PICK(EPI_F16, ACT_NONE);
             else { set_error("gemm_f16_2cta: activation %d not built", epi.act); return SBK_ERR_ARG; }
             break;
-        case EPI_F32:
-            if (bn128) G2_PICK_BN128(EPI_F32);
-            else G2_PICK(EPI_F32, ACT_NONE);
-            break;
-        case EPI_RESID:
-            if (bn128) G2_PICK_BN128(EPI_RESID);
-            else G2_PICK(EPI_RESID, ACT_NONE);
+        case EPI_F32: G2_PICK(EPI_F32, ACT_NONE); break;
+        case EPI_RESID: G2_PICK(EPI_RESID, ACT_NONE); break;
+        case EPI_RESID_LN:
+            if (N == 512) G2_PICK_LN(512, G2_STAGES);
+            else G2_PICK_LN(256, G2_STAGES);
             break;
         case EPI_GLU:
             if (fast_act) G2_PICK(EPI_GLU, ACT_SILU_FAST);
@@ -316,7 +455,7 @@
         default: set_error("gemm_f16_2cta: bad epilogue mode %d", epi.mode); return SBK_ERR_ARG;
     }
 #undef G2_PICK
-#undef G2_PICK_BN128
+#undef G2_PICK_LN
     SBK_CUDA_CHECK(cudaFuncSetAttribute(kern, cudaFuncAttributeMaxDynamicSharedMemorySize, smem));
     static int num_sms = 0;
     if (num_sms == 0) {
diff --git a/speechbrain_b200/csrc/sbk_internal.h b/speechbrain_b200/csrc/sbk_internal.h
--- a/speechbrain_b200/csrc/sbk_internal.h
+++ b/speechbrain_b200/csrc/sbk_internal.h
@@ -7,7 +7,7 @@
 
 namespace sbk {
 
-enum GemmEpiMode { EPI_F16 = 0, EPI_F32 = 1, EPI_RESID = 2, EPI_GLU = 3, EPI_ROPE = 4, EPI_QKV_CACHE = 5 };
+enum GemmEpiMode { EPI_F16 = 0, EPI_F32 = 1, EPI_RESID = 2, EPI_GLU = 3, EPI_ROPE = 4, EPI_QKV_CACHE = 5, EPI_RESID_LN = 6 };
 enum GemmAct { ACT_NONE = 0, ACT_SILU = 1, ACT_GELU = 2, ACT_RELU = 3, ACT_SILU_FAST = 4  };
 
 struct GemmEpilogue {
@@ -25,6 +25,9 @@
     int head_dim = 64;
     __half* kcache = nullptr; __half* vcache = nullptr; const int* step_ptr = nullptr; int S_max = 0; int qkv_d = 0;
     int kv_heads = 0; size_t kv_part_stride = 0;
+    const float* ln_ga = nullptr; const float* ln_ba = nullptr; float ln_eps_a = 1e-5f;
+    const float* ln_gb = nullptr; const float* ln_bb = nullptr; float ln_eps_b = 1e-5f;
+    void* ln_out = nullptr; int ln_out_f32 = 0; int ln_store_y = 0;
 };
 
 int gemm_f16(const void* A, int lda, const void* W, int ldw, const GemmEpilogue& epi, int M, int N, int K,
@@ -33,6 +36,7 @@
                    cudaStream_t stream);
 int gemm_f16_2cta(const void* A, int lda, const void* W, int ldw, const GemmEpilogue& epi, int M, int N, int K,
                   cudaStream_t stream);
+bool gemm_resid_ln_supported(int N);
 
 
 const char* last_error();
```
